# askerlee/segtran

Hardware: AMD Instinct MI355X
Metric: train-step images/sec (cfg2, re-associated op order) (higher is better)
Workload: dtype f32; 1 GPU; REFUGE fundus 2D, segtran eff-b4, translayers 3, layercompress 1,1,2,2, 512x512, bs 6/GPU; global_batch=6, per_gpu_batch=6, parallelism=dp1, step=fwd+BCE/Dice+bwd+allreduce+clip+BertAdam, op_order=re-associated, ranks=1

## Files before the change

include/segx.h:

```cpp
#ifndef SEGX_H
#define SEGX_H
#include <stdint.h>
#ifdef __cplusplus
extern "C" {
#endif

int segx_version(void);
int segx_last_error(char* buf, int buflen);

enum { SEGX_EPI_NONE = 0, SEGX_EPI_GELU = 1 ,
       SEGX_EPI_SWISH = 2 ,
       SEGX_EPI_RELU = 3  };
enum { SEGX_BIAS_NONE = 0, SEGX_BIAS_N = 1 , SEGX_BIAS_M = 2  };
enum { SEGX_ENGINE_F32 = 0, SEGX_ENGINE_BF16X6 = 1 };
enum { SEGX_ENGINE_SEL_DEFAULT = 0, SEGX_ENGINE_SEL_F32 = 1, SEGX_ENGINE_SEL_BF16X6 = 2 };
enum { SEGX_TILE_AUTO = 0, SEGX_TILE_128x128 = 1, SEGX_TILE_64x64 = 2, SEGX_TILE_128x32 = 3, SEGX_TILE_32x128 = 4, SEGX_TILE_64x128 = 5,
       SEGX_TILE_256x128 = 6, SEGX_TILE_WS128x128 = 7, SEGX_TILE_WS128x256 = 8, SEGX_TILE_WS64x256 = 9,
       SEGX_TILE_WS96x256 = 10, SEGX_TILE_WS256x96 = 11,
       SEGX_TILE_SKINNY_NT = 12   };
typedef struct {
    int32_t M, N, K, nb0, nb1;
    int64_t a_b0, a_b1, a_m, a_k;
    int64_t b_b0, b_b1, b_n, b_k;
    int64_t c_b0, c_b1, c_m;
    float alpha;
    int32_t epilogue, bias_mode;
    int64_t bias_b1;
    const float* bias;
    float* aux;
    float* gmax;
    float dropout_p;
    uint64_t seed, offset;
    int32_t splitk;
    float* workspace;
    int32_t tile;
    int64_t bias_b0;
    int32_t batch_reduce;
    int32_t engine;
    const void* b_planes;
    int64_t bp_b0, bp_b1;
    const float* resid;
} segx_gemm_desc;
int segx_gemm_f32(const float* A, const float* B, float* C, const segx_gemm_desc* d, void* stream);
int segx_gemm_plan(const float* A, const float* B, const segx_gemm_desc* d, int* tile, int* splitk);
int segx_gemm_plan_model(const float* A, const float* B, const segx_gemm_desc* d, int* tile, int* splitk);
int segx_gemm_route(const float* A, const float* B, const segx_gemm_desc* d, int32_t* out);
int64_t segx_x6_presplit_elems(int rows, int K, int nb0, int nb1);
int segx_x6_presplit(const float* W, int rows, int K, int64_t s_row, int64_t s_k, int nb0, int nb1, int64_t s_b0, int64_t s_b1, void* planes, void* stream);


int segx_softmax_fwd(const float* S, float* P, float* Pdrop, int64_t rows, int L, float clip, const float* gmax,
                     float p, uint64_t seed, uint64_t offset, void* stream);
int segx_softmax_bwd(const float* P, const float* dPdrop, const float* S , float* dS,
                     int64_t rows, int L, float clip, const float* gmax, float p, uint64_t seed, uint64_t offset, void* stream);
int segx_posbias_fwd(const float* S, float* out, const float* table, int64_t nmat, int N, const int* geom, float weight, float clip,
                     const float* gmax, void* stream);
int segx_posbias_bwd(const float* dOut, const float* S, float* dS, float* dtable, int64_t nmat, int N, const int* geom, float weight,
                     float clip, void* stream);
int segx_layernorm_fwd(const float* X, const float* w, const float* b, float* Y, float* mean, float* rstd,
                       int64_t rows, int C, float eps, void* stream);
int segx_layernorm_bwd(const float* dY, const float* X, const float* w, const float* mean, const float* rstd, float* dX,
                       int64_t rows, int C, void* stream);
int64_t segx_colreduce_ws_floats(int64_t rows, int64_t C, int nout);
int segx_colsum(const float* X, float* out, float* ws, int64_t rows, int64_t C, void* stream);
int segx_ln_param_grad(const float* dY, const float* X, const float* mean, const float* rstd, float* dw, float* db,
                       float* ws, int64_t rows, int C, void* stream);
int segx_sum(const float* x, int64_t n, float* out, float* ws , float scale, void* stream);
int segx_rowsum(const float* X, float* out, int64_t R, int64_t S, void* stream);
int segx_prenorm_fwd(const float* X, const float* w1, const float* b1, const float* pos, int64_t pos_ld, float pos_weight,
                     const float* mask, float* Y, float* stats, int64_t B, int N, int C, float eps,
                     float p, uint64_t seed, uint64_t offset, void* stream);
int segx_prenorm_bwd(const float* dY, const float* X, const float* w1, const float* b1, const float* pos, int64_t pos_ld,
                     float pos_weight, const float* mask, const float* stats, float* dX, float* dU, int64_t B, int N, int C,
                     float p, uint64_t seed, uint64_t offset, void* stream);
int64_t segx_prenorm_bwd_all_ws_floats(int N, int C);
int segx_prenorm_bwd_all(const float* dY, const float* X, const float* w1, const float* b1, const float* pos, int64_t pos_ld, float pos_weight,
                         const float* mask, const float* stats, float* dX, float* dsum, float* dw, float* db, float* ws, int B, int N, int C,
                         float p, uint64_t seed, uint64_t offset, void* stream);
int segx_posembed_fwd(const float* posn, const float* Wp, const float* bp, float* out, float* stats, int64_t N, int C, int pd,
                      float eps, void* stream);
int segx_posembed_bwd(const float* dOut, const float* posn, const float* Wp, const float* bp, const float* stats, float* dZ,
                      int64_t N, int C, int pd, void* stream);
int segx_modes_aggr_fwd(const float* Z, const float* lnw, const float* lnb, const float* wa, const float* ba, float* Y, float* stats,
                        int Mo, int64_t R, int F, float eps, float p, uint64_t seed, uint64_t offset, void* stream);
int segx_modes_aggr_bwd(const float* dY, const float* Z, const float* lnw, const float* lnb, const float* wa, const float* stats,
                        float* dZ, float* dscore, int Mo, int64_t R, int F, float p, uint64_t seed, uint64_t offset, void* stream);
int segx_modes_aggr_param_grad(const float* dY, const float* Z, const float* lnw, const float* lnb, const float* wa,
                               const float* stats, const float* dscore, float* dlnw, float* dlnb, float* dwa, float* ws,
                               int Mo, int64_t R, int F, float p, uint64_t seed, uint64_t offset, void* stream);
int64_t segx_modes_aggr_bwd_all_ws_floats(int Mo, int64_t R, int F);
int segx_modes_aggr_bwd_all(const float* dY, const float* Z, const float* lnw, const float* lnb, const float* wa, const float* stats,
                            float* dZ, float* dscore, float* dlnw, float* dlnb, float* dwa, float* ws, int Mo, int64_t R, int F,
                            float p, uint64_t seed, uint64_t offset, void* stream);
int segx_gelu_bwd(const float* dH, const float* T, float* dT, int64_t n, float p, uint64_t seed, uint64_t offset, void* stream);
int64_t segx_gelu_bwd_colsum_ws_floats(int64_t rows, int N);
int segx_gelu_bwd_colsum(const float* dH, const float* T, float* dT, float* colsum, float* ws, int64_t rows, int N, float p, uint64_t seed, uint64_t offset,
                         void* stream);

int64_t segx_loss_ws_floats(int B, int C);
int segx_seg_loss_fwd(const float* logits, const float* mask, const float* pos_weight, const float* class_w, float* out,
                      float* ws, int B, int C, int64_t S, float dice_w, void* stream);
int segx_seg_loss_bwd(const float* logits, const float* mask, const float* pos_weight, const float* class_w, const float* ws,
                      const float* grad_out, float* dlogits, int B, int C, int64_t S, float dice_w, void* stream);
int segx_mt_bertadam_step(void* const* params, const void* const* grads, void* const* m, void* const* v, const int64_t* sizes,
                          const int* chunk_tensor, const int64_t* chunk_off, const int* chunk_first, const int* active,
                          const float* lr, const float* wd, int ntensors, int nchunks, int chunk,
                          float max_global_norm, float max_tensor_norm, float sched, double b1, double b2, float eps,
                          float* ws, void* stream);

int segx_mt_gather(const void* const* src, void* const* dst, const int64_t* sizes, const int* chunk_tensor, const int64_t* chunk_off,
                   int chunk_begin, int nchunks, int chunk, void* stream);

int64_t segx_bn_ws_floats(int B, int C, int64_t S);
int segx_bn_act_bwd_reduce(const float* dY, const float* X, const float* mean, const float* var, const float* w, const float* b,
                           float* dw, float* db, float* ws, int B, int C, int64_t S, float eps, int act,
                           const float* gate, const float* dpool, float inv_S, float dc_p, uint64_t seed, uint64_t offset, void* stream);
int segx_bn_act_bwd_apply(const float* dY, const float* X, const float* mean, const float* var, const float* w, const float* b,
                          const float* sum_dw, const float* sum_db, float* dX, int B, int C, int64_t S, float eps, int act,
                          float inv_n, const float* gate, const float* dpool, float inv_S, float dc_p, uint64_t seed, uint64_t offset, void* stream);
int64_t segx_plane_chunks(int64_t S);
int64_t segx_bn_pool_chunks(int B, int64_t S, int auto_stats);
int64_t segx_bn_parts_floats(int B, int C, int64_t S);
int segx_bn_stats_local(const float* X, float* part, float* ws, int B, int C, int64_t S, void* stream);
int segx_bn_act_fwd2(const float* X, const float* parts, int nparts, float* mean, float* var, float* run_mean, float* run_var, float momentum,
                     const float* w, const float* b, float* Y, float* psum, const float* resid, float dc_p, uint64_t seed, uint64_t offset,
                     int B, int C, int64_t S, float eps, int act, int64_t parts_floats, int64_t y_bs, void* stream);
int segx_team_status(int clear);
int segx_team_cap(void);
int segx_occupy(int wgs, int heavy, float ms, float* sink, void* stream);
int segx_bn_act_bwd2(const float* dY, const float* X, const float* mean, const float* var, const float* w, const float* b,
                     float* dX, float* dw, float* db, float* ws, int B, int C, int64_t S, float eps, int act, int training,
                     const float* gate, const float* dpool, float inv_S, float dc_p, uint64_t seed, uint64_t offset, int64_t dy_bs, int64_t ws_floats, void* stream);
int segx_se_fwd2(const float* psum, int nch, float inv_S, const float* W1, const float* b1, const float* W2, const float* b2, const float* Wproj,
                 float* p, float* hpre, float* gate, float* Wb, int B, int C, int Cs, int M, void* stream);
int64_t segx_se_ws2_floats(int B, int C, int Cs);
int segx_se_bwd2(const float* dWb, const float* Wproj, const float* dgate, const float* gate, const float* hpre, const float* p, const float* W1,
                 const float* W2, float inv_S, float* dpool, float* dW1, float* db1, float* dW2, float* db2, float* dWproj, float* ws,
                 int B, int C, int Cs, int M, void* stream);
int segx_dwconv2d_fwd(const float* X, const float* W, float* Y, int B, int C, int H, int Wd, int OH, int OW, int k, int stride,
                      int pad_t, int pad_l, void* stream);
int64_t segx_dwconv2d_pool_chunks(int OH, int OW);
int segx_dwconv2d_bias_act_pool(const float* X, const float* W, const float* bias, float* Y, float* psum, int B, int C, int H, int Wd, int OH, int OW,
                                int k, int stride, int pad_t, int pad_l, int act, void* stream);
int segx_dwconv2d_bwd_data(const float* dY, const float* W, float* dX, int B, int C, int H, int Wd, int OH, int OW, int k,
                           int stride, int pad_t, int pad_l, void* stream);
int64_t segx_dwconv2d_wgrad_rows(int OH, int OW);
int64_t segx_dwconv2d_bwd_fused_rows(int H, int Wd, int OH, int OW, int k, int stride, int pad_t, int pad_l);
int segx_dwconv2d_bwd_fused(const float* dY, const float* X, const float* W, float* dX, float* part, int B, int C, int H, int Wd, int OH, int OW,
                            int k, int stride, int pad_t, int pad_l, void* stream);
int segx_mbconv_mid_ok(int B, int C, int H, int W, int k);
int segx_mbconv_mid_fwd(const float* E, const float* w0, const float* b0, float* run_mean0, float* run_var0, const float* Wdw, const float* w1, const float* b1,
                        float* run_mean1, float* run_var1, float* D, float* Y, float* psum, float* mean0, float* var0, float* mean1, float* var1,
                        float momentum0, float eps0, float momentum1, float eps1, int B, int C, int H, int W, int k, void* stream);
int segx_mbconv_mid_bwd(const float* dY, const float* dpool, const float* D, const float* E, const float* mean0, const float* var0, const float* mean1,
                        const float* var1, const float* w0, const float* b0, const float* w1, const float* b1, const float* Wdw,
                        float* dE, float* dw0, float* db0, float* dw1, float* db1, float* dWdw, float inv_S, float eps0, float eps1,
                        int B, int C, int H, int W, int k, void* stream);
int segx_bn_dw_s2_ok(int B, int C, int H, int W, int k, int stride, int pad_t, int pad_l);
int64_t segx_bn_dw_s2_ws_floats(int B, int C, int H, int W, int backward);
int64_t segx_bn_dw_s2_rows(int B, int H, int W);
int segx_bn_dw_s2_fwd(const float* E, const float* w0, const float* b0, float* run_mean, float* run_var, const float* Wdw, float* D, float* mean, float* var,
                      float* ws, float momentum, float eps, int B, int C, int H, int W, int k, int pad_t, int pad_l, int64_t ws_floats, void* stream);
int segx_bn_dw_s2_bwd(const float* dD, const float* E, const float* mean, const float* var, const float* w0, const float* b0, const float* Wdw,
                      float* dE, float* dw0, float* db0, float* part, float* ws, float eps, int B, int C, int H, int W, int k, int pad_t, int pad_l,
                      int64_t part_rows, int64_t ws_floats, void* stream);
int segx_dwconv2d_bwd_weight_direct(const float* dY, const float* X, float* dW, int B, int C, int H, int Wd, int OH, int OW, int k,
                                    int stride, int pad_t, int pad_l, void* stream);
int segx_dwconv2d_bwd_weight(const float* dY, const float* X, float* part, int B, int C, int H, int Wd, int OH, int OW, int k,
                             int stride, int pad_t, int pad_l, void* stream);
int segx_plane_scale(const float* X, const float* gate, float* Y, int64_t planes, int64_t S, void* stream);
int segx_plane_bias_add(const float* X, const float* bias, float* Y, int64_t planes, int C, int64_t S, void* stream);
int segx_plane_dot(const float* A, const float* Bm, float* out, int64_t planes, int64_t S, void* stream);

int segx_add_relu_fwd(const float* Z, const float* R, const float* bias, float* Y, int64_t planes, int C, int64_t S, void* stream);
int segx_add_relu_bwd(const float* dY, const float* Y, float* dZ, int64_t planes, int64_t S, void* stream);

int64_t segx_gn_ws_floats(int B, int C, int G);
int segx_groupnorm_fwd(const float* X, const float* w, const float* b, float* Y, float* mean, float* rstd, float* ws,
                       int B, int C, int G, int64_t S, float eps, void* stream);
int segx_groupnorm_bwd(const float* dY, const float* X, const float* w, const float* mean, const float* rstd, float* dX,
                       float* dw, float* db, float* ws, int B, int C, int G, int64_t S, float* plane_dx_sums, void* stream);
int64_t segx_interp_gn_nparts(int64_t float4_per_plane, int cpg);
int segx_interp_linear_fwd_axis2_gn(const float* in, const float* base, float* out, int64_t outer, int n1_in, int n1_out, int n2_in, int n2_out,
                                    int64_t inner, int cpg, float* parts, int nparts, void* stream);
int segx_groupnorm_fwd_parts(const float* X, const float* parts, int nparts, const float* w, const float* b, float* Y, float* mean, float* rstd,
                             int B, int C, int G, int64_t S, float eps, void* stream);
int segx_groupnorm_stats_parts(const float* parts, int nparts, float* mean, float* rstd, int BG, float eps, void* stream);
int segx_gn_fold_bwd_proj(const float* dOut, const float* Wb, int NC, const float* X, const float* mean, const float* rstd, const float* A, const float* Bc,
                          float* dX, float* plane_sums, float* ws, int B, int C, int G, int64_t S, void* stream);
int segx_gn_fold_bwd(const float* Gd, const float* X, const float* mean, const float* rstd, const float* A, const float* Bc, float* dX, float* plane_sums,
                     float* ws, int B, int C, int G, int64_t S, void* stream);
int segx_avgpool2_fwd(const float* X, float* Y, int64_t planes, int H, int W, void* stream);
int segx_avgpool2_bwd(const float* dY, float* dX, int64_t planes, int H, int W, void* stream);
int segx_transpose(const float* X, float* Y, int64_t batch, int R, int C, void* stream);
int segx_dropout(const float* x, float* y, int64_t n, float p, uint64_t seed, uint64_t offset, void* stream);
int segx_set_rng_base(const uint64_t* base);
int segx_rng_advance(uint64_t* base, uint64_t span, void* stream);

enum {
    SEGX_KNOB_INTERP_VARIANT = 1,
    SEGX_KNOB_CONV_SMALL_POLICY = 2,
    SEGX_KNOB_BN_PATH = 3,
    SEGX_KNOB_ENGINE = 4,
    SEGX_KNOB_X6_LAUNCHES = 5,
    SEGX_KNOB_X6_VARIANT = 6,
    SEGX_KNOB_CONV_X6_WGRAD_ALL = 7,
    SEGX_KNOB_DW_STRIP_OUTPUTS = 8,
    SEGX_KNOB_WS_GRID = 9,
    SEGX_KNOB_TEAM_SPIN = 12,
    SEGX_KNOB_TEAM_DROP = 13,
    SEGX_KNOB_POOL_SLAB = 14,
    SEGX_KNOB_POOL_DSLIDE = 15,
    SEGX_KNOB_CONV_HALO = 16,
    SEGX_KNOB_CONV_HALO_MIN_TILES = 17,
    SEGX_KNOB_SKINNY_NT = 18,
    SEGX_KNOB_TILE_WALK = 19
};
#define SEGX_KNOB_X6_TERMS 20
int segx_tune(int knob, int value);
int segx_tune_get(int knob);
int segx_x3_launches(void);
int segx_interp_linear_fwd_axis2(const float* in, const float* base, float* out, int64_t outer, int n1_in, int n1_out, int n2_in, int n2_out,
                                 int64_t inner, void* stream);
int segx_interp_linear_bwd_axis2(const float* dout, float* din, int64_t outer, int n1_out, int n1_in, int n2_out, int n2_in, int64_t inner, void* stream);
int segx_interp_linear_fwd(const float* in, const float* base, float* out, int64_t planes, int d, int h, int w, int D, int H, int W,
                           void* stream);
int segx_interp_linear_fwd_axis(const float* in, const float* base, float* out, int64_t outer, int n_in, int n_out, int64_t inner,
                                float src_scale, void* stream);
int segx_resized_crop3d(const float* X, float* Y, int64_t planes, const int* geom, void* stream);
int segx_interp_linear_bwd(const float* dout, float* din, int64_t planes, int d, int h, int w, int D, int H, int W, void* stream);
int segx_axis_gather(const float* X, float* Y, int64_t planes, const int* geom, void* stream);
int segx_pixel_shuffle2(const float* X, float* Y, int64_t planes, int h, int w, int inverse, void* stream);
int segx_add_noise(const float* X, const float* noise, float* Y, int64_t n, float mu, float sigma, int nonzero_only, uint64_t seed, uint64_t offset,
                   void* stream);
int segx_resize2d(const float* X, float* Y, int64_t planes, int h, int w, int H, int W, int mode, int quantize, void* stream);
int segx_color_blend(const float* X, float* Y, int B, int64_t HW, int mode, const float* factor, const float* pivot, int quantize, void* stream);
int64_t segx_gray_mean_ws_floats(int B, int64_t HW);
int segx_gray_mean(const float* X, float* mean, float* ws, int B, int64_t HW, int quantize, void* stream);
int segx_normalize(const float* X, float* Y, int B, int C, int64_t HW, float scale, const float* mean, const float* std, void* stream);

int segx_interp_linear_bwd_axis(const float* dout, float* din, int64_t outer, int n_out, int n_in, int64_t inner, float src_scale,
                                void* stream);

int64_t segx_conv3d_splitk(int B, int Cout, const int* geom, int wgrad);
int segx_conv3d_route(int B, int Cout, const int* geom, int wgrad, int splitk, int aligned, int packed, int32_t* out);
int segx_conv3d_fwd_terms(int B, int Cout, const int* geom, int splitk, int aligned, int packed);
int segx_conv3d_fwd(const float* X, const float* W , float* Y, int B, int Cout, const int* geom, int splitk,
                    float* workspace, void* stream);
int segx_conv3d_pack_weights(const float* W, float* Wp, int O, int C, int KV, int mode, void* stream);
int segx_conv3d_fwd_packed(const float* X, const float* Wp, float* Y, int B, int Cout, const int* geom, int splitk, float* workspace,
                           void* stream);
int segx_conv3d_flip_weights(const float* W, float* Wt, int Cout, int Cin, int KV, void* stream);
int segx_conv3d_bwd_weight(const float* dY, const float* X, float* dWb, int B, int Cout, const int* geom, int splitk,
                           float* workspace, void* stream);
int segx_conv3d_bwd_weight_packed(const float* dY, const float* X, float* dWb, int B, int Cout, const int* geom, int splitk,
                                  float* workspace, void* stream);
int segx_conv3d_unpack_wgrad(const float* dWp, float* dW, int Cout, int Cin, int KV, void* stream);
int segx_conv3d_fwd_packed_bs(const float* X, const float* Wp, float* Y, int B, int Cout, const int* geom, int splitk, float* workspace,
                              int64_t x_bstride, int64_t y_bstride, void* stream);
int segx_conv3d_fwd_bias_act(const float* X, const float* W, const float* bias, float* Y, int B, int Cout, const int* geom, int splitk, float* workspace,
                             int packed, int64_t x_bstride, int64_t y_bstride, int act, void* stream);
int segx_bias_map_relu(float* Y, const float* map, int B, int64_t n, void* stream);
int segx_conv3d_bwd_weight_packed_bs(const float* dY, const float* X, float* dWb, int B, int Cout, const int* geom, int splitk, float* workspace,
                                     int64_t dy_bstride, int64_t x_bstride, void* stream);
int segx_conv3d_halo_ok(int B, int Cout, const int* geom);
int64_t segx_conv3d_halo_wq_floats(int O, int C);
int segx_conv3d_halo_pack(const float* W, void* Wq, int O, int C, int mode, void* stream);
int segx_conv3d_halo_fwd(const float* X, const void* Wq, float* Y, int B, int Cout, const int* geom, int64_t x_bstride, int64_t y_bstride, int mtile, void* stream);
int segx_conv3d_halo_bias_act_fwd(const float* X, const void* Wq, const float* bias, float* Y, int B, int Cout, const int* geom, int64_t x_bstride, int64_t y_bstride,
                                  int mtile, int act, void* stream);
int segx_conv3d_halo_wgrad_ok(int B, int Cout, const int* geom);
int64_t segx_conv3d_halo_wgrad_ws_floats(int B, int Cout, const int* geom);
int segx_conv3d_halo_wgrad(const float* dY, const float* X, float* dW, float* ws, int B, int Cout, const int* geom, int64_t dy_bstride, int64_t x_bstride, void* stream);
int segx_conv3d_bwd_data_direct(const float* dY, const float* W, float* dX, float* wt_ws , int B, int Cout,
                                const int* geom, void* stream);
int segx_stem_compose_fwd(const float* Ws, const float* Wb, const float* bb, float* Wc, int O, int C3, int Cb, int Cc, int T, void* stream);
int segx_stem_compose_bwd(const float* dWc, const float* Ws, const float* Wb, const float* bb, float* dWs, float* dWb, float* dbb,
                          int O, int C3, int Cb, int Cc, int T, void* stream);
int segx_bridge_input(const float* X, float* Y, int B, int Cb, int Cc, int H, int W, int D, void* stream);
int segx_stem_s2d_input(const float* X, float* Y, int B, int Cb, int H, int W, int D, int U, void* stream);
int segx_conv2d_stem_fwd(const float* X, const float* W, float* Y, int B, int Cin, int Cout, int H, int Wd, int OH, int OW, int K, int stride, int pt, int pl,
                         void* stream);
int segx_conv2d_stem_bias_act_fwd(const float* X, const float* W, const float* bias, float* Y, int B, int Cin, int Cout, int H, int Wd, int OH, int OW, int K,
                                  int stride, int pt, int pl, int act, void* stream);
int segx_conv2d_stem_im2col(const float* X, float* Xcol, int B, int Cin, int H, int Wd, int OH, int OW, int K, int stride, int pt, int pl, int rows, void* stream);
int segx_bridge_mask(const float* X, const float* Wb, const float* bb, float* out, int B, int Cb, int C3, int H, int W, int D, int kd, int kh, int kw, void* stream);
int segx_nonzero_mask(const float* X, float* out, int B, int C, int D, int H, int W, int kd, int kh, int kw, void* stream);
int segx_label_nhot(const void* labels, float* out, int B, int Cin, int64_t S, int mode, void* stream);
int segx_maxpool3d_fwd(const float* X, float* Y, int* arg, int64_t planes, const int* geom, void* stream);
int segx_maxpool3d_bwd(const float* dY, const int* arg, float* dX, int64_t planes, const int* geom, const float* addend, void* stream);

int segx_window_accum(const float* scores, float* acc, float* cnt, int B, int C, const int* geom, void* stream);
#define SEGX_MAX_CLASSES 16
int segx_harden_segmap(const float* acc, const float* cnt, float* soft, float* hard, int B, int C, int64_t S, int mode, float T,
                       void* stream);
int segx_window_gather(const float* image, const int* origins, const int* origins_host, float* out, int nwin, int B, int C, const int* geom,
                       void* stream);
int segx_window_merge(const float* scores, const int* origins, const int* origins_host, float* soft, float* hard, int nwin, int B, int C,
                      const int* geom, int mode, float T, void* stream);
int64_t segx_dice_ws_floats(int64_t planes, int64_t S);
int segx_dice_sums(const float* pred, const float* gt, float* part, int64_t planes, int64_t S, void* stream);

#define SEGX_EDT_INF 0x40000000
#define SEGX_EDT_MAX_EXTENT 256
int segx_surface_border(const float* mask, uint8_t* border, int64_t planes, int D, int H, int W, int nd, void* stream);
int segx_edt_sq(const uint8_t* border, int32_t* d2, int64_t planes, int D, int H, int W, void* stream);
int segx_surface_hist(const uint8_t* border_from, const int32_t* d2_to, int32_t* hist, int64_t planes, int D, int H, int W, int nbins, void* stream);
#define SEGX_CASE_TAIL_THREADS 256
#define SEGX_CASE_TAIL_MAX_BLOCKS 2048
int segx_brats_case_tail(const float* soft, const float* hard, const int32_t* gt, int32_t* counts, uint8_t* labels, int64_t S, void* stream);

int segx_index_onehot(const void* labels, int label_bytes, float* out, int64_t B, int C, int64_t S, void* stream);
int segx_onehot_colormap(const float* nhot, const uint8_t* colormap, uint8_t* out, int64_t B, int C, int64_t S, void* stream);
int segx_onehot_case_tail(const float* soft, const uint8_t* gt, const uint8_t* colormap, int32_t* counts, uint8_t* labels, uint8_t* rgb, int B, int C, int64_t S,
                          float T, void* stream);
int segx_nhot_case_tail(const float* soft, const void* gt, int gt_map, int gt_channels, const int32_t* values, int32_t* counts, int32_t* ext, uint8_t* labels,
                        float* hard, int B, int C, int h, int w, int H, int W, float T, void* stream);

// ... 14 lines not shown
```

segtran_amd/csrc/backbone.hip:

```cpp
#include "common.h"
#include <mutex>
#include <unordered_map>

namespace segx {


__device__ __forceinline__ float drop_connect_scale(float p, uint64_t seed, uint64_t offset, const uint64_t* __restrict__ rbase, int sample) {
    if (!(p > 0.f)) return 1.0f;
    return dropout_scale(seed, 0, offset + (rbase ? *rbase : 0) + (uint64_t)sample, p, 1.0f / (1.0f - p));
}
__device__ __forceinline__ void bn_fold_sums(const float* __restrict__ ws, int c, int nparts, float& a, float& q) {
    const int lane = threadIdx.x & 63;
    const float2* p = reinterpret_cast<const float2*>(ws) + (int64_t)c * nparts;
    a = 0.f; q = 0.f;
    for (int i = lane; i < nparts; i += 64) { const float2 v = p[i]; a += v.x; q += v.y; }
    a = wave_sum(a); q = wave_sum(q);
}

constexpr int BN_SLABS = 8;
static inline int bn_slabs(int64_t S) { const int64_t n = S / 8192; return (int)(n < 1 ? 1 : n > BN_SLABS ? BN_SLABS : n); }

__global__ __launch_bounds__(256) void bn_act_bwd_stage1(const float* __restrict__ dY, const float* __restrict__ X, const float* __restrict__ mean,
                                                         const float* __restrict__ var, const float* __restrict__ w, const float* __restrict__ b,
                                                         float* __restrict__ ws, int C, int64_t S, float eps, int act,
// ... 471 lines not shown
        g.mean[c] = mean; g.var[c] = var;
        if (g.run_mean && st.n == st.n) {
            g.run_mean[c] = (1.0f - g.momentum) * g.run_mean[c] + g.momentum * mean;
            g.run_var[c] = (1.0f - g.momentum) * g.run_var[c] + g.momentum * (st.m2 / fmaxf(st.n - 1.0f, 1.0f));
        }
    }
    const float sc = rsqrtf(var + g.eps) * g.w[c], sh = g.b[c] - mean * sc;
    const bool resid = RESID < 0 ? g.resid != nullptr : RESID != 0;
    const float dcs = drop_connect_scale(g.dc_p, g.seed, g.offset, g.rbase, b);
    const ws_gptr_w yb = ws_uniform_base_w(g.Y + (int64_t)b * g.y_bs + (int64_t)c * S);
    const ws_gptr rb = ws_uniform_base((resid ? g.resid : g.X) + plane);
    float acc = 0.f;
    constexpr int G = 4;
    int tl2 = tl;
    SEGX_PIN(tl2);
    auto offs = [&](int k) { const int j = j0 + tl2 + 256 * k; return 16u * (unsigned)(j < S4 ? j : S4 - 1); };
#pragma unroll
    for (int k0 = 0; k0 < KP; k0 += G) {
        f32x4 rv[G];
        if (resid) {
#pragma unroll
            for (int e = 0; e < G; ++e) rv[e] = ws_load<f32x4>(rb, offs(k0 + e));
        }
#pragma unroll
        for (int e = 0; e < G; ++e) {
            const int k = k0 + e;
            f32x4 o;
            o.x = act_fwd_c<ACT>(v[k].x * sc + sh, act); o.y = act_fwd_c<ACT>(v[k].y * sc + sh, act);
            o.z = act_fwd_c<ACT>(v[k].z * sc + sh, act); o.w = act_fwd_c<ACT>(v[k].w * sc + sh, act);
            if (resid) { o.x = o.x * dcs + rv[e].x; o.y = o.y * dcs + rv[e].y; o.z = o.z * dcs + rv[e].z; o.w = o.w * dcs + rv[e].w; }
            if (j0 + tl2 + 256 * k < S4) {
                ws_store<f32x4>(yb, offs(k), o);
                if (POOL) acc += (o.x + o.y) + (o.z + o.w);
            }
        }
        __builtin_amdgcn_sched_barrier(0);
    }
    if (POOL) {
        acc = block_sum<4>(acc, red);
        if (tl == 0) g.psum[((int64_t)b * C + c) * t.cpp + ch] = acc;
    }
}
template <int KP, int ACT>
__global__ __launch_bounds__(256) SEGX_MIN_WAVES_PER_SIMD(KP <= 4 ? 4 : KP <= 8 ? 3 : 2) void bn_act_bwd_team_kernel(BnBwdArgs g, BnTeam t) {
    __shared__ float red[4];
    const int TS = t.B * t.cpp, tl = threadIdx.x;
    const int c = blockIdx.x / TS, r = blockIdx.x - c * TS, b = r / t.cpp, ch = r - b * t.cpp;
    const int C = g.C, S4 = (int)(g.S >> 2), j0 = ch * 256 * KP, act = g.act;
    const int64_t S = g.S;
    unsigned off[KP];
#pragma unroll
    for (int k = 0; k < KP; ++k) { const int j = j0 + tl + 256 * k; off[k] = 16u * (unsigned)(j < S4 ? j : S4 - 1); }
    f32x4 h[KP], d[KP];
    const ws_gptr xb = ws_uniform_base(g.X + ((int64_t)b * C + c) * S), gb = ws_uniform_base(g.dY + (int64_t)b * g.dy_bs + (int64_t)c * S);
#pragma unroll
    for (int k = 0; k < KP; ++k) { h[k] = ws_load<f32x4>(xb, off[k]); d[k] = ws_load<f32x4>(gb, off[k]); }
    __builtin_amdgcn_sched_barrier(0);
    const float rstd = rsqrtf(g.var[c] + g.eps), m = g.mean[c], wc = g.w[c], bc_ = g.b[c];
    const int pl = b * C + c;
    const float gt = (g.gate ? g.gate[pl] : 1.0f) * drop_connect_scale(g.dc_p, g.seed, g.offset, g.rbase, b), dp = g.dpool ? g.dpool[pl] * g.inv_S : 0.f;
    float a = 0.f, q = 0.f;
#pragma unroll
    for (int k = 0; k < KP; ++k) {
        const bool ok = j0 + tl + 256 * k < S4;
        const f32x4 xv = h[k], gv = d[k];
        f32x4 hh, dd;
        hh.x = (xv.x - m) * rstd; hh.y = (xv.y - m) * rstd; hh.z = (xv.z - m) * rstd; hh.w = (xv.w - m) * rstd;
        dd.x = (gv.x * gt + dp) * act_grad_c<ACT>(hh.x * wc + bc_, act); dd.y = (gv.y * gt + dp) * act_grad_c<ACT>(hh.y * wc + bc_, act);
        dd.z = (gv.z * gt + dp) * act_grad_c<ACT>(hh.z * wc + bc_, act); dd.w = (gv.w * gt + dp) * act_grad_c<ACT>(hh.w * wc + bc_, act);
        if (!ok) { dd = f32x4{0.f, 0.f, 0.f, 0.f}; hh = dd; }
        h[k] = hh; d[k] = dd;
        a += (dd.x + dd.y) + (dd.z + dd.w); q += (dd.x * hh.x + dd.y * hh.y) + (dd.z * hh.z + dd.w * hh.w);
    }
    a = block_sum<4>(a, red); q = block_sum<4>(q, red);
    const TeamBufs tb{t.slots + (int64_t)c * TS * TEAM_SLOT, t.mbox + (int64_t)c * TS * TEAM_MBOX, t.tag_lo, t.tag_hi, t.err, t.spin};
    if (tl == 0) { float* pp = tb.slots + r * TEAM_SLOT; team_store(pp, a); team_store(pp + 1, q); }
    float res[3];
    team_exchange(tb, r, TS, res, [](const float* parts, int members, float (&o)[3]) {
        const int lane = threadIdx.x & 63;
        const bool h0 = lane < members, h1 = lane + 64 < members;
        const float a0 = team_load(parts + TEAM_SLOT * (h0 ? lane : 0)), q0 = team_load(parts + TEAM_SLOT * (h0 ? lane : 0) + 1);
        const float a1 = team_load(parts + TEAM_SLOT * (h1 ? lane + 64 : 0)), q1 = team_load(parts + TEAM_SLOT * (h1 ? lane + 64 : 0) + 1);
        float A = (h0 ? a0 : 0.f) + (h1 ? a1 : 0.f), Q = (h0 ? q0 : 0.f) + (h1 ? q1 : 0.f);
#pragma unroll
        for (int o2 = 1; o2 < 64; o2 <<= 1) { A += __shfl_xor(A, o2); Q += __shfl_xor(Q, o2); }
        o[0] = A; o[1] = Q; o[2] = 0.f;
    });
    const float A = res[0], Q = res[1];
    if (r == 0 && tl == 0) { g.db[c] = A; g.dw[c] = Q; }
    const float inv_n = 1.0f / ((float)t.B * (float)S), k1 = A * inv_n, k2 = Q * inv_n, sc = wc * rstd;
    const ws_gptr_w ob = ws_uniform_base_w(g.dX + ((int64_t)b * C + c) * S);
#pragma unroll
    for (int k = 0; k < KP; ++k) {
        if (j0 + tl + 256 * k < S4) {
            f32x4 o;
            o.x = sc * (d[k].x - k1 - h[k].x * k2); o.y = sc * (d[k].y - k1 - h[k].y * k2);
            o.z = sc * (d[k].z - k1 - h[k].z * k2); o.w = sc * (d[k].w - k1 - h[k].w * k2);
            ws_store<f32x4>(ob, off[k], o);
        }
    }
}
static inline int bn_res_form(int B, int64_t S, bool backward) {
    if ((S & 3) || B < 1 || B > 8 || S > 8192) return 0;
    const int S4 = (int)(S >> 2);
    const int kw = (S4 + 63) / 64, kb = (S4 + 255) / 256;
    const int capw = backward ? 1 : 2, capb = backward ? 2 : 4;
    if (kw <= capw) return 64 * 16 + (kw <= 1 ? 1 : 2);
    if (kb <= capb) return 256 * 16 + (kb <= 1 ? 1 : kb <= 2 ? 2 : 4);
    return 0;
}
static inline bool bn_bwd_plane_team(int B, int64_t S) { return (S & 3) == 0 && S > 2048 && S <= 4096 && B >= 1 && B <= 6; }

static inline int bn_team_chunks(int64_t S, int kp) { return (int)((S / 4 + 256 * kp - 1) / (256 * kp)); }
static inline int bn_team_kp_small(int64_t S) { return S <= 4096 ? 4 : S <= 8192 ? 8 : 16; }
static inline int bn_team_kp(int B, int64_t S, bool backward) {
    if ((S & 3) || B < 1 || S < 16384) return 0;
    const int cap = team_cap();
    if (backward) return (int64_t)bn_team_chunks(S, 16) * B <= cap ? 16 : 0;
    if ((int64_t)bn_team_chunks(S, 16) * B <= (cap < 32 ? cap : 32)) return 16;
    return (int64_t)bn_team_chunks(S, 32) * B <= (cap < 64 ? cap : 64) ? 32 : 0;
}
static inline int bn_auto_form(int B, int64_t S, bool backward, int* kp = nullptr) {
    const int path = kget(knobs().bn_path);
    int k = 16;
    int form = 0;
    if (path == 2 && (S & 3) == 0 && B <= 128 && S >= 4 && (int64_t)bn_team_chunks(S, 16) * B <= team_cap()) { form = 1; k = bn_team_kp_small(S); }
    else if (bn_res_form(B, S, backward)) form = 2;
    else if (backward && path != 1 && bn_bwd_plane_team(B, S) && B <= team_cap()) { form = 1; k = bn_team_kp_small(S); }
    else if (path != 1 && (k = bn_team_kp(B, S, backward)) != 0) form = 1;
    if (kp) *kp = form == 1 ? k : 0;
    return form;
}
template <int KP>
static int bn_team_launch_fwd(const BnFwdArgs& g, const BnTeam& t, dim3 grid, hipStream_t stream, bool pool) {
    const bool resid = g.resid != nullptr;
#define SEGX_BN_TF(P, A, R) do { if (int rc = team_occupancy_ok((const void*)bn_act_fwd_team_kernel<KP, P, A, R>, "segx_bn_act_fwd2/team")) return rc; \
                                 hipLaunchKernelGGL((bn_act_fwd_team_kernel<KP, P, A, R>), grid, dim3(256), 0, stream, g, t); } while (0)
    if (pool) { if (!resid && g.act == ACT_SWISH) SEGX_BN_TF(true, ACT_SWISH, 0); else SEGX_BN_TF(true, -1, -1); }
    else if (!resid && g.act == ACT_SWISH) SEGX_BN_TF(false, ACT_SWISH, 0);
    else if (g.act == ACT_NONE) { if (resid) SEGX_BN_TF(false, ACT_NONE, 1); else SEGX_BN_TF(false, ACT_NONE, 0); }
    else if (!resid && g.act == ACT_RELU) SEGX_BN_TF(false, ACT_RELU, 0);
    else SEGX_BN_TF(false, -1, -1);
#undef SEGX_BN_TF
    return check_launch("segx_bn_act_fwd2/team");
}
template <int KP>
static int bn_team_launch_bwd(const BnBwdArgs& g, const BnTeam& t, dim3 grid, hipStream_t stream) {
#define SEGX_BN_TB(A) do { if (int rc = team_occupancy_ok((const void*)bn_act_bwd_team_kernel<KP, A>, "segx_bn_act_bwd2/team")) return rc; \
                           hipLaunchKernelGGL((bn_act_bwd_team_kernel<KP, A>), grid, dim3(256), 0, stream, g, t); } while (0)
    if (g.act == ACT_SWISH) SEGX_BN_TB(ACT_SWISH); else if (g.act == ACT_NONE) SEGX_BN_TB(ACT_NONE); else if (g.act == ACT_RELU) SEGX_BN_TB(ACT_RELU); else SEGX_BN_TB(-1);
#undef SEGX_BN_TB
    return check_launch("segx_bn_act_bwd2/team");
}
constexpr int S2_BAND = 4;
constexpr int S2_IMG = 1440;
constexpr int S2_GIMG = 1600;
struct BnDwS2Args {
    const float* E; const float* w; const float* b; const float* Wdw; float* mean; float* var;
    float* D; float* run_mean; float* run_var; float momentum;
    const float* dD; float* dE; float* dw; float* db; float* part;
    float eps; int C, H, W4, pt;
};
template <int KP, int K, int PL>
__global__ __launch_bounds__(256) SEGX_MIN_WAVES_PER_SIMD(KP <= 16 ? 3 : 2) void bn_dw_s2_fwd_team_kernel(BnDwS2Args g, BnTeam t) {
    static_assert(KP % S2_BAND == 0 && PL <= 4 && 4 + 3 * 2 + K - 1 - PL < 16, "window does not fit the four float4 read per row");
    constexpr int NB = KP / S2_BAND;
    __shared__ float red[4];
    __shared__ f32x4 img[NB > 1 ? 2 : 1][S2_IMG];
    const int TS = t.B * t.cpp, tl = threadIdx.x;
    const int c = blockIdx.x / TS, r = blockIdx.x - c * TS, b = r / t.cpp, ch = r - b * t.cpp;
    const int C = g.C, W4 = g.W4, S4 = g.H * W4, j0 = ch * 256 * KP;
    const int64_t S = 4 * (int64_t)S4, plane = ((int64_t)b * C + c) * S;
    auto offk = [&](int k) { const int j = j0 + tl + 256 * k; return 16u * (unsigned)(j < S4 ? j : S4 - 1); };
    f32x4 v[KP];
    const ws_gptr xb = ws_uniform_base(g.E + plane);
#pragma unroll
    for (int k = 0; k < KP; ++k) v[k] = ws_load<f32x4>(xb, offk(k));
    const int rpk = 256 / W4, tr = tl / W4, tc = tl - tr * W4, HT = g.pt, LS = W4 + 1, IR = S2_BAND * rpk + K - 2;
    f32x4 hv[2]; bool hok[2];
#pragma unroll
    for (int q = 0; q < 2; ++q) {
        const int hr = tr + q * rpk;
        const int jh = (hr < HT ? j0 - (HT - hr) * W4 : j0 + 256 * KP + (hr - HT) * W4) + tc;
        hok[q] = hr < K - 2 && jh >= 0 && jh < S4;
        hv[q] = ws_load<f32x4>(xb, 16u * (unsigned)(hok[q] ? jh : 0));
    }
    __builtin_amdgcn_sched_barrier(0);
    for (int i = tl; i <= IR; i += 256) {
        img[0][i * LS] = f32x4{0.f, 0.f, 0.f, 0.f};
        if (NB > 1) img[NB > 1 ? 1 : 0][i * LS] = f32x4{0.f, 0.f, 0.f, 0.f};
    }
    float w[K * K];
#pragma unroll
    for (int i = 0; i < K * K; ++i) w[i] = g.Wdw[(int64_t)c * K * K + i];
    float s = 0.f;
#pragma unroll
    for (int k = 0; k < KP; ++k) {
        if (!(j0 + tl + 256 * k < S4)) v[k] = f32x4{0.f, 0.f, 0.f, 0.f};
        s += (v[k].x + v[k].y) + (v[k].z + v[k].w);
    }
    const int left4 = S4 - j0;
    const float n = 4.0f * (float)(left4 < 256 * KP ? left4 : 256 * KP);
    const float m = block_sum<4>(s, red) / n;
    float q = 0.f;
#pragma unroll
    for (int k = 0; k < KP; ++k) {
        const float d0 = v[k].x - m, d1 = v[k].y - m, d2 = v[k].z - m, d3 = v[k].w - m;
        q += (j0 + tl + 256 * k < S4) ? (d0 * d0 + d1 * d1) + (d2 * d2 + d3 * d3) : 0.f;
    }
    q = block_sum<4>(q, red);
    const TeamBufs tb{t.slots + (int64_t)c * TS * TEAM_SLOT, t.mbox + (int64_t)c * TS * TEAM_MBOX, t.tag_lo, t.tag_hi, t.err, t.spin};
    if (tl == 0) { float* pp = tb.slots + r * TEAM_SLOT; team_store(pp, n); team_store(pp + 1, m); team_store(pp + 2, q); }
    float res[3];
    team_exchange(tb, r, TS, res, [](const float* slots, int members, float (&o)[3]) { const BnPart f = bn_fold_team(slots, members); o[0] = f.n; o[1] = f.mean; o[2] = f.m2; });
    BnPart st; st.n = res[0]; st.mean = res[1]; st.m2 = res[2];
    const float mean = st.mean, var = st.n != st.n ? st.n : st.n > 0.f ? fmaxf(st.m2 / st.n, 0.f) : 0.f;
    if (r == 0 && tl == 0) {
        g.mean[c] = mean; g.var[c] = var;
        if (g.run_mean && st.n == st.n) {
            g.run_mean[c] = (1.0f - g.momentum) * g.run_mean[c] + g.momentum * mean;
            g.run_var[c] = (1.0f - g.momentum) * g.run_var[c] + g.momentum * (st.m2 / fmaxf(st.n - 1.0f, 1.0f));
        }
    }
    const float sc = rsqrtf(var + g.eps) * g.w[c], sh = g.b[c] - mean * sc;
    auto act4 = [&](const f32x4& x, bool ok) {
        f32x4 o;
        o.x = act_fwd_c<ACT_SWISH>(x.x * sc + sh, ACT_SWISH); o.y = act_fwd_c<ACT_SWISH>(x.y * sc + sh, ACT_SWISH);
        o.z = act_fwd_c<ACT_SWISH>(x.z * sc + sh, ACT_SWISH); o.w = act_fwd_c<ACT_SWISH>(x.w * sc + sh, ACT_SWISH);
        return ok ? o : f32x4{0.f, 0.f, 0.f, 0.f};
    };
    const int OW4 = W4 >> 1, orow = tl / OW4, oc = tl - orow * OW4, D4 = S4 >> 2;
    const int rpos = (2 * orow) * LS + 2 * oc + 1;
    const ws_gptr_w db_ = ws_uniform_base_w(g.D + ((int64_t)b * C + c) * (S >> 2));
#pragma unroll
    for (int bd = 0; bd < NB; ++bd) {
        constexpr int KB = S2_BAND;
        const int k0 = bd * KB;
        f32x4* im = img[bd & (NB > 1 ? 1 : 0)];
#pragma unroll
        for (int kk = k0 - 1; kk <= k0 + KB; ++kk) {
            if (kk < 0 || kk >= KP) continue;
            const int ir = tr + (kk - k0) * rpk + HT;
            if (kk < k0 ? ir >= 0 : kk < k0 + KB || ir < IR) im[ir * LS + 1 + tc] = act4(v[kk], j0 + tl + 256 * kk < S4);
        }
        if (bd == 0 || bd == NB - 1) {
#pragma unroll
            for (int q2 = 0; q2 < 2; ++q2) {
                const int hr = tr + q2 * rpk;
                if (hr < K - 2 && (hr < HT ? bd == 0 : bd == NB - 1)) im[(hr < HT ? hr : KB * rpk + hr) * LS + 1 + tc] = act4(hv[q2], hok[q2]);
            }
        }
        __syncthreads();
        float acc[4] = {0.f, 0.f, 0.f, 0.f};
#pragma unroll
        for (int ky = 0; ky < K; ++ky) {
            const f32x4* p = im + rpos + ky * LS;
            const f32x4 e0 = p[-1], e1 = p[0], e2 = p[1], e3 = p[2];
            const float e[16] = {e0.x, e0.y, e0.z, e0.w, e1.x, e1.y, e1.z, e1.w, e2.x, e2.y, e2.z, e2.w, e3.x, e3.y, e3.z, e3.w};
#pragma unroll
            for (int j = 0; j < 4; ++j)
#pragma unroll
                for (int kx = 0; kx < K; ++kx) acc[j] += w[ky * K + kx] * e[4 + j * 2 + kx - PL];
#pragma unroll
            for (int j = 0; j < 4; ++j) SEGX_PIN(acc[j]);
        }
        const int dj = ((j0 + 256 * k0) >> 2) + tl;
        if (dj < D4) ws_store<f32x4>(db_, 16u * (unsigned)dj, f32x4{acc[0], acc[1], acc[2], acc[3]});
        __builtin_amdgcn_sched_barrier(0);
    }
}
template <int KP, int K, int PL>
__global__ __launch_bounds__(256) SEGX_MIN_WAVES_PER_SIMD(2) void bn_dw_s2_bwd_team_kernel(BnDwS2Args g, BnTeam t) {
    constexpr int A = (K + 1) / 2, KK = K * K, NGV = KP / 4 + 1;
    __shared__ float red[4];
    __shared__ double wred[4][KK];
    __shared__ f32x4 gim[S2_GIMG];
    const int TS = t.B * t.cpp, tl = threadIdx.x;
    const int c = blockIdx.x / TS, r = blockIdx.x - c * TS, b = r / t.cpp, ch = r - b * t.cpp;
    const int C = g.C, W4 = g.W4, S4 = g.H * W4, j0 = ch * 256 * KP, pt = g.pt;
    const int64_t S = 4 * (int64_t)S4, plane = ((int64_t)b * C + c) * S;
    auto offk = [&](int k) { const int j = j0 + tl + 256 * k; return 16u * (unsigned)(j < S4 ? j : S4 - 1); };
    f32x4 h[KP], d[KP];
    const ws_gptr xb = ws_uniform_base(g.E + plane);
#pragma unroll
    for (int k = 0; k < KP; ++k) h[k] = ws_load<f32x4>(xb, offk(k));
    const int rpk = 256 / W4, tr = tl / W4, tc = tl - tr * W4, OW4 = W4 >> 1, OH = g.H >> 1, GS = OW4 + 1, NG = KP * (rpk >> 1) + A;
    const int gpr = 256 / OW4, gr = tl / OW4, gc = tl - gr * OW4, oy_lo = ((j0 / W4) >> 1) + (pt >> 1) - (A - 1);
    {
        const ws_gptr gb = ws_uniform_base(g.dD + ((int64_t)b * C + c) * (S >> 2));
        f32x4 gv[NGV];
#pragma unroll
        for (int i = 0; i < NGV; ++i) {
            const int oy = oy_lo + gr + i * gpr;
            gv[i] = ws_load<f32x4>(gb, 16u * (unsigned)(gr + i * gpr < NG && oy >= 0 && oy < OH ? oy * OW4 + gc : 0));
        }
        for (int i = tl; i <= NG; i += 256) gim[i * GS] = f32x4{0.f, 0.f, 0.f, 0.f};
#pragma unroll
        for (int i = 0; i < NGV; ++i) {
            const int gi = gr + i * gpr, oy = oy_lo + gi;
            if (gi < NG) gim[gi * GS + 1 + gc] = oy >= 0 && oy < OH ? gv[i] : f32x4{0.f, 0.f, 0.f, 0.f};
        }
    }
    __syncthreads();
    __builtin_amdgcn_sched_barrier(0);
    const float rstd = rsqrtf(g.var[c] + g.eps), m = g.mean[c], wc = g.w[c], bc_ = g.b[c], sc = rstd * wc, sh = bc_ - m * sc;
    const int py = (tr + pt) & 1;
    float wsel[A][K], dwa[A][K];
#pragma unroll
    for (int a = 0; a < A; ++a)
#pragma unroll
        for (int kx = 0; kx < K; ++kx) {
            const float we = g.Wdw[(int64_t)c * KK + (2 * a) * K + kx], wo = 2 * a + 1 < K ? g.Wdw[(int64_t)c * KK + (2 * a + 1) * K + kx] : 0.f;
            wsel[a][kx] = py ? wo : we; dwa[a][kx] = 0.f;
        }
    const float* gf = reinterpret_cast<const float*>(gim) + (((tr + pt) >> 1) - (pt >> 1) + A - 1) * (4 * GS) + 2 * tc + 2;
    float sa = 0.f, sq = 0.f;
#pragma unroll
    for (int k = 0; k < KP; ++k) {
        const bool ok = j0 + tl + 256 * k < S4;
        const f32x4 xv = h[k];
        const float u[4] = {xv.x * sc + sh, xv.y * sc + sh, xv.z * sc + sh, xv.w * sc + sh};
        float ep[4], de[4] = {0.f, 0.f, 0.f, 0.f};
#pragma unroll
        for (int i = 0; i < 4; ++i) ep[i] = ok ? act_fwd_c<ACT_SWISH>(u[i], ACT_SWISH) : 0.f;
#pragma unroll
        for (int a = A - 1; a >= 0; --a) {
            const float* gp = gf + (k * (rpk >> 1) - a) * (4 * GS);
            const float2 g0 = *reinterpret_cast<const float2*>(gp), g1 = *reinterpret_cast<const float2*>(gp + 2), g2 = *reinterpret_cast<const float2*>(gp + 4);
            const float G[6] = {g0.x, g0.y, g1.x, g1.y, g2.x, g2.y};
#pragma unroll
            for (int i = 0; i < 4; ++i)
#pragma unroll
                for (int kx = 0; kx < K; ++kx) {
                    if ((i + PL - kx) & 1) continue;
                    const int nn = (i + PL - kx + 4) / 2;
                    de[i] = __builtin_fmaf(wsel[a][kx], G[nn], de[i]); dwa[a][kx] = __builtin_fmaf(ep[i], G[nn], dwa[a][kx]);
                    SEGX_PIN(de[i]); SEGX_PIN(dwa[a][kx]);
                }
            __builtin_amdgcn_sched_barrier(0);
        }
        f32x4 hh, dd;
        hh.x = (xv.x - m) * rstd; hh.y = (xv.y - m) * rstd; hh.z = (xv.z - m) * rstd; hh.w = (xv.w - m) * rstd;
        dd.x = de[0] * act_grad_c<ACT_SWISH>(hh.x * wc + bc_, ACT_SWISH); dd.y = de[1] * act_grad_c<ACT_SWISH>(hh.y * wc + bc_, ACT_SWISH);
        dd.z = de[2] * act_grad_c<ACT_SWISH>(hh.z * wc + bc_, ACT_SWISH); dd.w = de[3] * act_grad_c<ACT_SWISH>(hh.w * wc + bc_, ACT_SWISH);
        if (!ok) { dd = f32x4{0.f, 0.f, 0.f, 0.f}; hh = dd; }
        h[k] = hh; d[k] = dd;
        sa += (dd.x + dd.y) + (dd.z + dd.w); sq += (dd.x * hh.x + dd.y * hh.y) + (dd.z * hh.z + dd.w * hh.w);
    }
    sa = block_sum<4>(sa, red); sq = block_sum<4>(sq, red);
    const TeamBufs tb{t.slots + (int64_t)c * TS * TEAM_SLOT, t.mbox + (int64_t)c * TS * TEAM_MBOX, t.tag_lo, t.tag_hi, t.err, t.spin};
    if (tl == 0) { float* pp = tb.slots + r * TEAM_SLOT; team_store(pp, sa); team_store(pp + 1, sq); }
    float res[3];
    team_exchange(tb, r, TS, res, [](const float* parts, int members, float (&o)[3]) {
        const int lane = threadIdx.x & 63;
        const bool h0 = lane < members, h1 = lane + 64 < members;
        const float a0 = team_load(parts + TEAM_SLOT * (h0 ? lane : 0)), q0 = team_load(parts + TEAM_SLOT * (h0 ? lane : 0) + 1);
        const float a1 = team_load(parts + TEAM_SLOT * (h1 ? lane + 64 : 0)), q1 = team_load(parts + TEAM_SLOT * (h1 ? lane + 64 : 0) + 1);
        float As = (h0 ? a0 : 0.f) + (h1 ? a1 : 0.f), Qs = (h0 ? q0 : 0.f) + (h1 ? q1 : 0.f);
#pragma unroll
        for (int o2 = 1; o2 < 64; o2 <<= 1) { As += __shfl_xor(As, o2); Qs += __shfl_xor(Qs, o2); }
        o[0] = As; o[1] = Qs; o[2] = 0.f;
    });
    const float As = res[0], Qs = res[1];
    if (r == 0 && tl == 0) { g.db[c] = As; g.dw[c] = Qs; }
    const float inv_n = 1.0f / ((float)t.B * (float)S), k1 = As * inv_n, k2 = Qs * inv_n;
    const ws_gptr_w ob = ws_uniform_base_w(g.dE + plane);
    int tl2 = tl;
    SEGX_PIN(tl2);
#pragma unroll
    for (int k = 0; k < KP; ++k) {
        const int j = j0 + tl2 + 256 * k;
        if (j < S4) {
            f32x4 o;
            o.x = sc * (d[k].x - k1 - h[k].x * k2); o.y = sc * (d[k].y - k1 - h[k].y * k2);
            o.z = sc * (d[k].z - k1 - h[k].z * k2); o.w = sc * (d[k].w - k1 - h[k].w * k2);
            ws_store<f32x4>(ob, 16u * (unsigned)j, o);
        }
    }
#pragma unroll
    for (int a = 0; a < A; ++a)
#pragma unroll
        for (int p = 0; p < 2; ++p) {
            if (2 * a + p >= K) continue;
#pragma unroll
            for (int kx = 0; kx < K; ++kx) {
                const double sw = wave_sum_d(py == p ? (double)dwa[a][kx] : 0.0);
                if ((tl & 63) == 0) wred[tl >> 6][(2 * a + p) * K + kx] = sw;
            }
        }
    __syncthreads();
    if (tl < KK) g.part[((int64_t)r * C + c) * KK + tl] = (float)((wred[0][tl] + wred[1][tl]) + (wred[2][tl] + wred[3][tl]));
}
static inline bool s2_pow2(int v) { return v > 0 && (v & (v - 1)) == 0; }
static inline int s2_kp(int B, int64_t S, bool backward) {
    int kp = 0;
    if (B < 1 || S < 4 || bn_auto_form(B, S, backward, &kp) != 1) return 0;
    return kp == 4 || kp == 16 || (kp == 32 && !backward) ? kp : 0;
}
static inline bool s2_serves(int B, int C, int H, int W, int k, int stride, int pt, int pl) {
    if (!(stride == 2 && (k == 3 || k == 5) && B >= 1 && C >= 1 && H >= 2 && (H & 1) == 0 && W >= 16 && W <= 512 && s2_pow2(W))) return false;
    if (!(pt == pl && pt >= (k - 2) / 2 && pt <= k / 2)) return false;
    const int64_t S = (int64_t)H * W;
    if (S > (int64_t)1 << 26 || (int64_t)B * C > 65535) return false;
    const int kf = s2_kp(B, S, false), kb = s2_kp(B, S, true);
    if (!kf || !kb || (1024 * kf) % (2 * W) || (1024 * kb) % (2 * W)) return false;
    const int W4 = W / 4, rpk = 256 / W4;
    return (S2_BAND * rpk + k - 2) * (W4 + 1) + 1 <= S2_IMG && (kb * (rpk / 2) + (k + 1) / 2) * (W4 / 2 + 1) + 1 <= S2_GIMG;
}
template <int KP, int K>
static int s2_launch_fwd(const BnDwS2Args& g, const BnTeam& t, dim3 grid, hipStream_t stream, int pl) {
#define SEGX_S2F(P) do { if (int rc = team_occupancy_ok((const void*)bn_dw_s2_fwd_team_kernel<KP, K, P>, "segx_bn_dw_s2_fwd")) return rc; \
                         hipLaunchKernelGGL((bn_dw_s2_fwd_team_kernel<KP, K, P>), grid, dim3(256), 0, stream, g, t); } while (0)
    if (pl == (K - 2) / 2) SEGX_S2F((K - 2) / 2); else SEGX_S2F(K / 2);
#undef SEGX_S2F
    return check_launch("segx_bn_dw_s2_fwd");
}
template <int KP, int K>
static int s2_launch_bwd(const BnDwS2Args& g, const BnTeam& t, dim3 grid, hipStream_t stream, int pl) {
#define SEGX_S2B(P) do { if (int rc = team_occupancy_ok((const void*)bn_dw_s2_bwd_team_kernel<KP, K, P>, "segx_bn_dw_s2_bwd")) return rc; \
                         hipLaunchKernelGGL((bn_dw_s2_bwd_team_kernel<KP, K, P>), grid, dim3(256), 0, stream, g, t); } while (0)
    if (pl == (K - 2) / 2) SEGX_S2B((K - 2) / 2); else SEGX_S2B(K / 2);
#undef SEGX_S2B
    return check_launch("segx_bn_dw_s2_bwd");
}
template <int T, int K, int BM>
static void bn_res_launch_fwd(const BnFwdArgs& g, int B, dim3 grid, hipStream_t stream, bool pool) {
    const bool resid = g.resid != nullptr;
#define SEGX_BN_F(P, A, R) hipLaunchKernelGGL((bn_act_fwd_res_kernel<T, K, BM, P, A, R>), grid, dim3(256), 0, stream, g, B)
    if (pool) { if (!resid && g.act == ACT_SWISH) SEGX_BN_F(true, ACT_SWISH, 0); else SEGX_BN_F(true, -1, -1); }
    else if (!resid && g.act == ACT_SWISH) SEGX_BN_F(false, ACT_SWISH, 0);
    else if (g.act == ACT_NONE) { if (resid) SEGX_BN_F(false, ACT_NONE, 1); else SEGX_BN_F(false, ACT_NONE, 0); }
    else if (!resid && g.act == ACT_RELU) SEGX_BN_F(false, ACT_RELU, 0);
    else SEGX_BN_F(false, -1, -1);
#undef SEGX_BN_F
}
template <int T, int K, int BM>
static void bn_res_launch_bwd(const BnBwdArgs& g, int B, dim3 grid, hipStream_t stream) {
#define SEGX_BN_B(A) hipLaunchKernelGGL((bn_act_bwd_res_kernel<T, K, BM, A>), grid, dim3(256), 0, stream, g, B)
    if (g.act == ACT_SWISH) SEGX_BN_B(ACT_SWISH); else if (g.act == ACT_NONE) SEGX_BN_B(ACT_NONE); else if (g.act == ACT_RELU) SEGX_BN_B(ACT_RELU); else SEGX_BN_B(-1);
#undef SEGX_BN_B
}

constexpr int DW_TY = 8;
struct DwTile { int ox, oy0; bool live; };
__device__ __forceinline__ DwTile dw_tile(int tile, int tiles_x, int txw_log2, int OH, int OW) {
    const int txw = 1 << txw_log2, rg = threadIdx.x >> txw_log2, nrg = 256 >> txw_log2;
    const int tyi = tile / tiles_x, txi = tile - tyi * tiles_x;
    DwTile t;
    t.ox = txi * txw + (threadIdx.x & (txw - 1));
    t.oy0 = (tyi * nrg + rg) * DW_TY;
    t.live = t.ox < OW && t.oy0 < OH;
    return t;
}
template <int K, int ST, bool FLIP>
__global__ __launch_bounds__(256) void dwconv_rows_kernel(const float* __restrict__ X, const float* __restrict__ Wt, float* __restrict__ Y,
                                                          int C, int H, int W, int OH, int OW, int pt, int pl, int tiles_x, int txw_log2) {
    const int bc = blockIdx.y, c = bc % C;
    const DwTile t = dw_tile(blockIdx.x, tiles_x, txw_log2, OH, OW);
    if (!t.live) return;
    const float* x = X + (int64_t)bc * H * W;
    float w[K * K];
#pragma unroll
    for (int i = 0; i < K * K; ++i) w[i] = Wt[(int64_t)c * K * K + (FLIP ? K * K - 1 - i : i)];
    float acc[DW_TY];
#pragma unroll
    for (int i = 0; i < DW_TY; ++i) acc[i] = 0.f;
    const int ix0 = t.ox * ST - pl, iy0 = t.oy0 * ST - pt;
    constexpr int NR = (DW_TY - 1) * ST + K;
#pragma unroll
    for (int r = 0; r < NR; ++r) {
        const int iy = iy0 + r;
        const bool rowok = iy >= 0 && iy < H;
        const float* xr = x + (int64_t)min(max(iy, 0), H - 1) * W;
        float v[K];
#pragma unroll
        for (int kx = 0; kx < K; ++kx) {
            const int ix = ix0 + kx;
            const float q = xr[min(max(ix, 0), W - 1)];
            v[kx] = (rowok && ix >= 0 && ix < W) ? q : 0.f;
        }
#pragma unroll
        for (int ky = 0; ky < K; ++ky) {
            if ((r - ky) < 0 || (r - ky) % ST != 0 || (r - ky) / ST >= DW_TY) continue;
#pragma unroll
            for (int kx = 0; kx < K; ++kx) acc[(r - ky) / ST] += w[ky * K + kx] * v[kx];
            SEGX_PIN(acc[(r - ky) / ST]);
        }
    }
    float* y = Y + (int64_t)bc * OH * OW + t.ox;
#pragma unroll
    for (int i = 0; i < DW_TY; ++i) if (t.oy0 + i < OH) y[(int64_t)(t.oy0 + i) * OW] = acc[i];
}
constexpr int DW4_TY = 8, DW4_AHEAD = 2;
template <int K, int ST> struct Dw4 { static constexpr int NV = ST == 1 ? 3 : 4; };
template <int NV>
__device__ __forceinline__ void dw4_load_row(float (&e)[4 * NV], const float* __restrict__ xr, const int (&xo)[NV], const bool (&okv)[NV], bool rowok) {
#pragma unroll
    for (int i = 0; i < NV; ++i) {
        const float4 q = *reinterpret_cast<const float4*>(xr + xo[i]);
        const bool ok = rowok && okv[i];
        e[4 * i] = ok ? q.x : 0.f; e[4 * i + 1] = ok ? q.y : 0.f; e[4 * i + 2] = ok ? q.z : 0.f; e[4 * i + 3] = ok ? q.w : 0.f;
    }
}
template <int K, int ST, int PL, bool FLIP>
__global__ __launch_bounds__(256) SEGX_MIN_WAVES_PER_SIMD(4) void dwconv_rows4_kernel(const float* __restrict__ X, const float* __restrict__ Wt, float* __restrict__ Y,
                                                           int C, int H, int W, int OH, int OW, int pt, int tiles_x, int tiles_y, int tpr_log2,
                                                           int64_t ngroups) {
    constexpr int NV = Dw4<K, ST>::NV;
    static_assert(PL <= 4 && 4 + 3 * ST + K - 1 - PL < 4 * NV, "window does not fit the loaded float4s");
    const int64_t gid = ((int64_t)xcd_block(blockIdx.x, gridDim.x) * 256 + threadIdx.x) >> tpr_log2;
    if (gid >= ngroups) return;
    const int gpp = tiles_x * tiles_y;
    const int64_t plane = gid / gpp;
    const int rem = (int)(gid - plane * gpp), tyi = rem / tiles_x, txi = rem - tyi * tiles_x;
    const int ox = ((txi << tpr_log2) + (threadIdx.x & ((1 << tpr_log2) - 1))) * 4, oy0 = tyi * DW4_TY;
    if (ox >= OW) return;
    const int c = (int)(plane % C);
    const float* x = X + plane * H * W;
    float w[K * K];
#pragma unroll
    for (int i = 0; i < K * K; ++i) w[i] = Wt[(int64_t)c * K * K + (FLIP ? K * K - 1 - i : i)];
    float acc[DW4_TY][4];
#pragma unroll
    for (int i = 0; i < DW4_TY; ++i) { acc[i][0] = 0.f; acc[i][1] = 0.f; acc[i][2] = 0.f; acc[i][3] = 0.f; }
    int xo[NV]; bool okv[NV];
#pragma unroll
    for (int i = 0; i < NV; ++i) { const int col = ox * ST - 4 + 4 * i; okv[i] = col >= 0 && col < W; xo[i] = min(max(col, 0), W - 4); }
    const int iy0 = oy0 * ST - pt;
    constexpr int NR = (DW4_TY - 1) * ST + K;
    float e[DW4_AHEAD + 1][4 * NV];
#pragma unroll
    for (int r = 0; r < DW4_AHEAD && r < NR; ++r)
        dw4_load_row<NV>(e[r], x + (int64_t)min(max(iy0 + r, 0), H - 1) * W, xo, okv, iy0 + r >= 0 && iy0 + r < H);
#pragma unroll
    for (int r = 0; r < NR; ++r) {
        if (r + DW4_AHEAD < NR) {
            const int iy = iy0 + r + DW4_AHEAD;
            dw4_load_row<NV>(e[(r + DW4_AHEAD) % (DW4_AHEAD + 1)], x + (int64_t)min(max(iy, 0), H - 1) * W, xo, okv, iy >= 0 && iy < H);
        }
        __builtin_amdgcn_sched_barrier(0);
#pragma unroll
        for (int ky = 0; ky < K; ++ky) {
            if ((r - ky) < 0 || (r - ky) % ST != 0 || (r - ky) / ST >= DW4_TY) continue;
#pragma unroll
            for (int j = 0; j < 4; ++j)
#pragma unroll
                for (int kx = 0; kx < K; ++kx)
                    acc[(r - ky) / ST][j] += w[ky * K + kx] * e[r % (DW4_AHEAD + 1)][4 + j * ST + kx - PL];
#pragma unroll
            for (int j = 0; j < 4; ++j) SEGX_PIN(acc[(r - ky) / ST][j]);
        }
        __builtin_amdgcn_sched_barrier(0);
    }
    float* y = Y + plane * OH * OW + ox;
#pragma unroll
    for (int i = 0; i < DW4_TY; ++i)
        if (oy0 + i < OH) *reinterpret_cast<float4*>(y + (int64_t)(oy0 + i) * OW) = make_float4(acc[i][0], acc[i][1], acc[i][2], acc[i][3]);
}
template <int K, int ST, int PL>
__global__ __launch_bounds__(256) SEGX_MIN_WAVES_PER_SIMD(4) void dwconv_rows4_bias_act_pool_kernel(const float* __restrict__ X, const float* __restrict__ Wt, const float* __restrict__ bias,
                                                           float* __restrict__ Y, float* __restrict__ psum, int C, int H, int W, int OH, int OW, int pt, int tiles_x, int tiles_y,
                                                           int tpr_log2, int64_t ngroups, int act) {
    constexpr int NV = Dw4<K, ST>::NV;
    static_assert(PL <= 4 && 4 + 3 * ST + K - 1 - PL < 4 * NV, "window does not fit the loaded float4s");
    const int64_t gid_raw = ((int64_t)xcd_block(blockIdx.x, gridDim.x) * 256 + threadIdx.x) >> tpr_log2;
    const bool glive = gid_raw < ngroups;
    const int64_t gid = glive ? gid_raw : ngroups - 1;
    const int gpp = tiles_x * tiles_y;
    const int64_t plane = gid / gpp;
    const int rem = (int)(gid - plane * gpp), tyi = rem / tiles_x, txi = rem - tyi * tiles_x;
    const int ox_raw = ((txi << tpr_log2) + (threadIdx.x & ((1 << tpr_log2) - 1))) * 4, oy0 = tyi * DW4_TY;
    const bool live = glive && ox_raw < OW;
    const int ox = ox_raw < OW ? ox_raw : OW - 4;
    const int c = (int)(plane % C);
    const float* x = X + plane * H * W;
    float w[K * K];
// ... 818 lines not shown
    const int rows = (64 >> g.tpr_log2) * segx::DWG_TY, ntiles = g.tiles_x * ((OH + rows - 1) / rows);
    const int64_t nwork = (int64_t)B * C * strips;
    const int64_t nblocks = (nwork + 3) / 4;
#define SEGX_DW4(KK, SS, PP)                                                                                                        \
    if (k == KK && stride == SS && pl == PP) {                                                                                       \
        hipLaunchKernelGGL((segx::dwconv_wgrad4_kernel<KK, SS, PP>), dim3((unsigned)nblocks), dim3(256), 0, stream, dY, X, part, C,  \
                           H, Wd, OH, OW, pt, g.tiles_x, ntiles, g.tpr_log2, strips, nwork);                                         \
        return true;                                                                                                                 \
    }
    SEGX_DW4(3, 1, 1) SEGX_DW4(5, 1, 2) SEGX_DW4(3, 2, 0) SEGX_DW4(3, 2, 1) SEGX_DW4(5, 2, 1) SEGX_DW4(5, 2, 2)
#undef SEGX_DW4
    return false;
}
}

extern "C" int segx_dwconv2d_fwd(const float* X, const float* W, float* Y, int B, int C, int H, int Wd, int OH, int OW, int k, int stride,
                                 int pad_t, int pad_l, void* stream_) {
    SEGX_STREAM; SEGX_REQUIRE(X && W && Y && B > 0 && C > 0 && H > 0 && Wd > 0 && OH > 0 && OW > 0 && (int64_t)B * C <= 65535, "segx_dwconv2d_fwd: bad args");
    if (dw4_ok(X, Y, Wd, OW) && dw4_rows_launch<false>(stream, X, W, Y, B * C, C, H, Wd, OH, OW, k, stride, pad_t, pad_l))
        return check_launch("segx_dwconv2d_fwd");
    const DwGrid g = dw_grid(OH, OW);
    dim3 grid(g.tiles_x * g.tiles_y, B * C);
    SEGX_DW_ROWS_DISPATCH(false, X, W, Y, C, H, Wd, OH, OW, pad_t, pad_l, g.tiles_x, g.txw_log2);
    return check_launch("segx_dwconv2d_fwd");
}
extern "C" int64_t segx_dwconv2d_pool_chunks(int OH, int OW) {
    if (OH <= 0 || OW <= 0) return 0;
    return (int64_t)dw4_grid(OW).tiles_x * ((OH + segx::DW4_TY - 1) / segx::DW4_TY);
}
extern "C" int segx_dwconv2d_bias_act_pool(const float* X, const float* W, const float* bias, float* Y, float* psum, int B, int C, int H, int Wd, int OH, int OW,
                                           int k, int stride, int pad_t, int pad_l, int act, void* stream_) {
    SEGX_STREAM; SEGX_REQUIRE(X && W && bias && Y && B > 0 && C > 0 && H > 0 && Wd > 0 && OH > 0 && OW > 0 && (int64_t)B * C <= 65535 && (act == 0 || act == 1) && pad_t >= 0 && pad_l >= 0,
                              "segx_dwconv2d_bias_act_pool: bad args");
    SEGX_REQUIRE((int64_t)(OH - 1) * stride - pad_t < H && (int64_t)(OW - 1) * stride - pad_l < Wd, "segx_dwconv2d_bias_act_pool: output %d x %d does not fit input %d x %d", OH, OW, H, Wd);
    const Dw4Grid g = dw4_grid(OW);
    const int tiles_y = (OH + segx::DW4_TY - 1) / segx::DW4_TY, planes = B * C;
    if (dw4_ok(X, Y, Wd, OW)) {
        const int64_t ngroups = (int64_t)planes * g.tiles_x * tiles_y;
        const int64_t nblocks = ((ngroups << g.tpr_log2) + 255) / 256;
        if (nblocks <= 2147483647LL) {
#define SEGX_DW4P(KK, SS, PP)                                                                                                                          \
            if (k == KK && stride == SS && pad_l == PP) {                                                                                               \
                hipLaunchKernelGGL((segx::dwconv_rows4_bias_act_pool_kernel<KK, SS, PP>), dim3((unsigned)nblocks), dim3(256), 0, stream, X, W, bias, Y, \
                                   psum, C, H, Wd, OH, OW, pad_t, g.tiles_x, tiles_y, g.tpr_log2, ngroups, act);                                        \
                return check_launch("segx_dwconv2d_bias_act_pool");                                                                                     \
            }
            SEGX_DW4P(3, 1, 1) SEGX_DW4P(5, 1, 2) SEGX_DW4P(3, 2, 0) SEGX_DW4P(3, 2, 1) SEGX_DW4P(5, 2, 1) SEGX_DW4P(5, 2, 2)
#undef SEGX_DW4P
        }
    }
    const dim3 grid(g.tiles_x * tiles_y, planes);
    SEGX_DW_DISPATCH(segx::dwconv_bias_act_pool_kernel, X, W, bias, Y, psum, C, H, Wd, OH, OW, pad_t, pad_l, g.tiles_x, g.tpr_log2 + 2, act);
    return check_launch("segx_dwconv2d_bias_act_pool");
}
extern "C" int segx_dwconv2d_bwd_data(const float* dY, const float* W, float* dX, int B, int C, int H, int Wd, int OH, int OW, int k, int stride,
                                      int pad_t, int pad_l, void* stream_) {
    SEGX_STREAM; SEGX_REQUIRE(dY && W && dX && B > 0 && C > 0 && H > 0 && Wd > 0 && OH > 0 && OW > 0 && (int64_t)B * C <= 65535, "segx_dwconv2d_bwd_data: bad args");
    if (stride == 1) {
        if (dw4_ok(dY, dX, OW, Wd) && dw4_rows_launch<true>(stream, dY, W, dX, B * C, C, OH, OW, H, Wd, k, 1, k - 1 - pad_t, k - 1 - pad_l))
            return check_launch("segx_dwconv2d_bwd_data");
        const DwGrid g = dw_grid(H, Wd);
        dim3 grid(g.tiles_x * g.tiles_y, B * C);
        SEGX_DW_ROWS_DISPATCH(true, dY, W, dX, C, OH, OW, H, Wd, k - 1 - pad_t, k - 1 - pad_l, g.tiles_x, g.txw_log2);
        return check_launch("segx_dwconv2d_bwd_data");
    }
    if (stride == 2 && Wd % 8 == 0 && OW % 4 == 0 && pad_t == pad_l && ((reinterpret_cast<uintptr_t>(dY) | reinterpret_cast<uintptr_t>(dX)) & 15) == 0) {
        int l = 3;
        while (l < 6 && (8 << l) < Wd) ++l;
        const int tiles_x = (Wd + (8 << l) - 1) / (8 << l), tiles_y = (H + segx::DWB_TY - 1) / segx::DWB_TY;
        const int64_t ngroups = (int64_t)B * C * tiles_x * tiles_y, nblocks = ((ngroups << l) + 255) / 256;
#define SEGX_DWB(KK, PP)                                                                                                             \
        if (k == KK && pad_l == PP && nblocks <= 2147483647LL) {                                                                      \
            hipLaunchKernelGGL((segx::dwconv_bwd4s2_kernel<KK, PP, PP>), dim3((unsigned)nblocks), dim3(256), 0, stream, dY, W, dX, C, \
                               H, Wd, OH, OW, tiles_x, tiles_y, l, ngroups);                                                          \
            return check_launch("segx_dwconv2d_bwd_data");                                                                            \
        }
        SEGX_DWB(3, 0) SEGX_DWB(3, 1) SEGX_DWB(5, 1) SEGX_DWB(5, 2)
#undef SEGX_DWB
    }
    const int tx = (Wd + 15) / 16, ty = (H + 15) / 16;
    dim3 grid(tx * ty, B * C);
    SEGX_DW_DISPATCH(dwconv_bwd_data_kernel, dY, W, dX, C, H, Wd, OH, OW, pad_t, pad_l, tx);
    return check_launch("segx_dwconv2d_bwd_data");
}
extern "C" int segx_dwconv2d_bwd_weight_direct(const float* dY, const float* X, float* dW, int B, int C, int H, int Wd, int OH, int OW,
                                               int k, int stride, int pad_t, int pad_l, void* stream_) {
    SEGX_STREAM; SEGX_REQUIRE(dY && X && dW && B > 0 && C > 0 && OH > 0 && OW > 0, "segx_dwconv2d_bwd_weight_direct: bad args");
    if (B > 8 || dw_wgrad_strips(OH, OW) != 1 || !dw4_ok(dY, X, Wd, OW)) return 0;
    const Dw4Grid g = dw4_grid(OW);
    const int rows = (64 >> g.tpr_log2) * segx::DWG_TY, ntiles = g.tiles_x * ((OH + rows - 1) / rows);
#define SEGX_DW4C(KK, SS, PP)                                                                                                       \
    if (k == KK && stride == SS && pad_l == PP) {                                                                                    \
        hipLaunchKernelGGL((segx::dwconv_wgrad4c_kernel<KK, SS, PP>), dim3(C), dim3(512), 0, stream, dY, X, dW, B, C, H, Wd, OH, OW,  \
                           pad_t, g.tiles_x, ntiles, g.tpr_log2);                                                                     \
        const int rc = check_launch("segx_dwconv2d_bwd_weight_direct");                                                               \
        return rc ? (rc > 0 ? -rc - 1000 : rc) : 1;                                                                                  \
    }
    SEGX_DW4C(3, 1, 1) SEGX_DW4C(5, 1, 2) SEGX_DW4C(3, 2, 0) SEGX_DW4C(3, 2, 1) SEGX_DW4C(5, 2, 1) SEGX_DW4C(5, 2, 2)
#undef SEGX_DW4C
    return 0;
}
static int dw_fused_strips(int H, int Wd, int OH, int OW, int k, int stride, int pad_t, int pad_l) {
    if (stride != 1 || (k != 3 && k != 5) || pad_t != (k - 1) / 2 || pad_l != (k - 1) / 2 || OH != H || OW != Wd || Wd % 4 != 0 || Wd < 4) return 0;
    const Dw4Grid g = dw4_grid(Wd);
    const int tiles_y = (H + segx::DW4_TY - 1) / segx::DW4_TY, gpp = g.tiles_x * tiles_y, gpw = 64 >> g.tpr_log2;
    return gpp % gpw == 0 ? gpp / gpw : 0;
}
extern "C" int64_t segx_dwconv2d_bwd_fused_rows(int H, int Wd, int OH, int OW, int k, int stride, int pad_t, int pad_l) {
    return dw_fused_strips(H, Wd, OH, OW, k, stride, pad_t, pad_l);
}
extern "C" int segx_dwconv2d_bwd_fused(const float* dY, const float* X, const float* W, float* dX, float* part , int B, int C, int H, int Wd,
                                       int OH, int OW, int k, int stride, int pad_t, int pad_l, void* stream_) {
    SEGX_STREAM; SEGX_REQUIRE(dY && X && W && dX && part && B > 0 && C > 0 && (int64_t)B * C <= 65535, "segx_dwconv2d_bwd_fused: bad args");
    const int strips = dw_fused_strips(H, Wd, OH, OW, k, stride, pad_t, pad_l);
    SEGX_REQUIRE(strips > 0 && ((reinterpret_cast<uintptr_t>(dY) | reinterpret_cast<uintptr_t>(X) | reinterpret_cast<uintptr_t>(dX)) & 15) == 0,
                 "segx_dwconv2d_bwd_fused: shape not served (segx_dwconv2d_bwd_fused_rows == 0) or unaligned tensors");
    const Dw4Grid g = dw4_grid(Wd);
    const int tiles_y = (H + segx::DW4_TY - 1) / segx::DW4_TY;
    const int64_t ngroups = (int64_t)B * C * g.tiles_x * tiles_y, nblocks = ((ngroups << g.tpr_log2) + 255) / 256;
    SEGX_REQUIRE(nblocks <= 2147483647LL, "segx_dwconv2d_bwd_fused: too many workgroups");
    if (k == 3) hipLaunchKernelGGL((segx::dwconv_bwd_s1_fused_kernel<3>), dim3((unsigned)nblocks), dim3(256), 0, stream, dY, X, W, dX, part, C, H, Wd, g.tiles_x, tiles_y, g.tpr_log2, ngroups, strips);
    else hipLaunchKernelGGL((segx::dwconv_bwd_s1_fused_kernel<5>), dim3((unsigned)nblocks), dim3(256), 0, stream, dY, X, W, dX, part, C, H, Wd, g.tiles_x, tiles_y, g.tpr_log2, ngroups, strips);
    return check_launch("segx_dwconv2d_bwd_fused");
}
extern "C" int64_t segx_dwconv2d_wgrad_rows(int OH, int OW) { return OH > 0 && OW > 0 ? dw_wgrad_strips(OH, OW) : 0; }
extern "C" int segx_dwconv2d_bwd_weight(const float* dY, const float* X, float* part , int B, int C, int H, int Wd, int OH, int OW,
                                        int k, int stride, int pad_t, int pad_l, void* stream_) {
    SEGX_STREAM; SEGX_REQUIRE(dY && X && part && B > 0 && C > 0 && OH > 0 && OW > 0 && (int64_t)B * C <= 65535, "segx_dwconv2d_bwd_weight: bad args");
    const int strips = dw_wgrad_strips(OH, OW);
    if (dw4_ok(dY, X, Wd, OW) && dw4_wgrad_launch(stream, dY, X, part, B, C, H, Wd, OH, OW, k, stride, pad_t, pad_l, strips))
        return check_launch("segx_dwconv2d_bwd_weight");
    const DwGrid g = dw_grid(OH, OW);
    dim3 grid(strips, B * C);
    SEGX_DW_DISPATCH(dwconv_wgrad_rows_kernel, dY, X, part, C, H, Wd, OH, OW, pad_t, pad_l, g.tiles_x, g.tiles_x * g.tiles_y, g.txw_log2);
    return check_launch("segx_dwconv2d_bwd_weight");
}
extern "C" int segx_plane_scale(const float* X, const float* gate, float* Y, int64_t planes, int64_t S, void* stream_) {
    SEGX_STREAM; SEGX_REQUIRE(X && gate && Y && planes > 0 && S > 0 && planes <= 65535, "segx_plane_scale: bad args");
    hipLaunchKernelGGL(plane_scale_kernel, dim3(plane_chunks(S, 8), (unsigned)planes), dim3(256), 0, stream, X, gate, Y, S);
    return check_launch("segx_plane_scale");
}
extern "C" int segx_plane_bias_add(const float* X, const float* bias, float* Y, int64_t planes, int C, int64_t S, void* stream_) {
    SEGX_STREAM; SEGX_REQUIRE(X && bias && Y && planes > 0 && C > 0 && S > 0 && planes <= 65535, "segx_plane_bias_add: bad args");
    hipLaunchKernelGGL(plane_bias_add_kernel, dim3(plane_chunks(S, 8), (unsigned)planes), dim3(256), 0, stream, X, bias, Y, C, S);
    return check_launch("segx_plane_bias_add");
}
extern "C" int segx_plane_dot(const float* A, const float* Bm, float* out, int64_t planes, int64_t S, void* stream_) {
    SEGX_STREAM; SEGX_REQUIRE(A && Bm && out && planes > 0 && S > 0 && planes < 2147483647LL, "segx_plane_dot: bad args");
    hipLaunchKernelGGL(plane_dot_kernel, dim3((unsigned)planes), dim3(256), 0, stream, A, Bm, out, S);
    return check_launch("segx_plane_dot");
}
extern "C" int segx_bn_dw_s2_ok(int B, int C, int H, int W, int k, int stride, int pad_t, int pad_l) { return s2_serves(B, C, H, W, k, stride, pad_t, pad_l) ? 1 : 0; }
extern "C" int64_t segx_bn_dw_s2_ws_floats(int B, int C, int H, int W, int backward) {
    const int kp = H > 0 && W > 0 ? s2_kp(B, (int64_t)H * W, backward != 0) : 0;
    return kp ? (int64_t)C * B * bn_team_chunks((int64_t)H * W, kp) * (TEAM_SLOT + TEAM_MBOX) : 0;
}
extern "C" int64_t segx_bn_dw_s2_rows(int B, int H, int W) {
    const int kp = H > 0 && W > 0 ? s2_kp(B, (int64_t)H * W, true) : 0;
    return kp ? (int64_t)B * bn_team_chunks((int64_t)H * W, kp) : 0;
}
static int s2_team(BnTeam& t, float* ws, int64_t ws_floats, int B, int C, int64_t S, int kp, const char* what) {
    t.B = B; t.cpp = bn_team_chunks(S, kp); t.slots = ws; t.mbox = ws + (int64_t)C * B * t.cpp * TEAM_SLOT;
    team_fill(t);
    SEGX_REQUIRE(B * t.cpp <= team_cap() && (int64_t)C * B * t.cpp < 2147483647LL, "%s: team of %d workgroups", what, B * t.cpp);
    const int64_t need = (int64_t)C * B * t.cpp * (TEAM_SLOT + TEAM_MBOX);
    SEGX_REQUIRE(ws_floats >= need, "%s: the scratch holds %lld floats, this call needs %lld (segx_bn_dw_s2_ws_floats under the current knob 3)", what, (long long)ws_floats, (long long)need);
    return 0;
}
extern "C" int segx_bn_dw_s2_fwd(const float* E, const float* w0, const float* b0, float* run_mean, float* run_var, const float* Wdw, float* D, float* mean, float* var,
                                 float* ws, float momentum, float eps, int B, int C, int H, int W, int k, int pad_t, int pad_l, int64_t ws_floats, void* stream_) {
    SEGX_STREAM; SEGX_REQUIRE(E && w0 && b0 && Wdw && D && mean && var && ws && (!run_mean == !run_var), "segx_bn_dw_s2_fwd: bad args");
    SEGX_REQUIRE(s2_serves(B, C, H, W, k, 2, pad_t, pad_l), "segx_bn_dw_s2_fwd: shape not served (segx_bn_dw_s2_ok == 0)");
    SEGX_REQUIRE(((reinterpret_cast<uintptr_t>(E) | reinterpret_cast<uintptr_t>(D)) & 15) == 0, "segx_bn_dw_s2_fwd: tensors must be 16-byte aligned");
    const int64_t S = (int64_t)H * W;
    const int kp = s2_kp(B, S, false);
    BnTeam t;
    if (int rc = s2_team(t, ws, ws_floats, B, C, S, kp, "segx_bn_dw_s2_fwd")) return rc;
    BnDwS2Args g; memset(&g, 0, sizeof(g));
    g.E = E; g.w = w0; g.b = b0; g.Wdw = Wdw; g.mean = mean; g.var = var; g.D = D; g.run_mean = run_mean; g.run_var = run_var; g.momentum = momentum;
    g.eps = eps; g.C = C; g.H = H; g.W4 = W / 4; g.pt = pad_t;
    const dim3 tg = team_grid((int64_t)C * B * t.cpp);
#define SEGX_S2(KP) (k == 3 ? s2_launch_fwd<KP, 3>(g, t, tg, stream, pad_l) : s2_launch_fwd<KP, 5>(g, t, tg, stream, pad_l))
    return kp == 4 ? SEGX_S2(4) : kp == 16 ? SEGX_S2(16) : SEGX_S2(32);
#undef SEGX_S2
}
extern "C" int segx_bn_dw_s2_bwd(const float* dD, const float* E, const float* mean, const float* var, const float* w0, const float* b0, const float* Wdw,
                                 float* dE, float* dw0, float* db0, float* part, float* ws, float eps, int B, int C, int H, int W, int k, int pad_t, int pad_l,
                                 int64_t part_rows, int64_t ws_floats, void* stream_) {
    SEGX_STREAM; SEGX_REQUIRE(dD && E && mean && var && w0 && b0 && Wdw && dE && dw0 && db0 && part && ws, "segx_bn_dw_s2_bwd: bad args");
    SEGX_REQUIRE(s2_serves(B, C, H, W, k, 2, pad_t, pad_l), "segx_bn_dw_s2_bwd: shape not served (segx_bn_dw_s2_ok == 0)");
    SEGX_REQUIRE(((reinterpret_cast<uintptr_t>(E) | reinterpret_cast<uintptr_t>(dD) | reinterpret_cast<uintptr_t>(dE)) & 15) == 0, "segx_bn_dw_s2_bwd: tensors must be 16-byte aligned");
    const int64_t S = (int64_t)H * W;
    const int kp = s2_kp(B, S, true);
    BnTeam t;
    if (int rc = s2_team(t, ws, ws_floats, B, C, S, kp, "segx_bn_dw_s2_bwd")) return rc;
    SEGX_REQUIRE(part_rows >= (int64_t)B * t.cpp, "segx_bn_dw_s2_bwd: the filter-gradient partials hold %lld rows, this call writes %d (segx_bn_dw_s2_rows under the current knob 3)",
                 (long long)part_rows, B * t.cpp);
    BnDwS2Args g; memset(&g, 0, sizeof(g));
    g.E = E; g.w = w0; g.b = b0; g.Wdw = Wdw; g.mean = const_cast<float*>(mean); g.var = const_cast<float*>(var); g.dD = dD; g.dE = dE; g.dw = dw0; g.db = db0; g.part = part;
    g.eps = eps; g.C = C; g.H = H; g.W4 = W / 4; g.pt = pad_t;
    const dim3 tg = team_grid((int64_t)C * B * t.cpp);
#define SEGX_S2(KP) (k == 3 ? s2_launch_bwd<KP, 3>(g, t, tg, stream, pad_l) : s2_launch_bwd<KP, 5>(g, t, tg, stream, pad_l))
    return kp == 4 ? SEGX_S2(4) : SEGX_S2(16);
#undef SEGX_S2
}
```

segtran_amd/efficientnet/model.py:

```python
import math
import torch
from torch import nn
from torch.nn import functional as F

from .. import functional as SF
from ..fold import FoldableBackbone, fold_conv_bn, pair_sources

BN_MOM, BN_EPS = 1 - 0.99, 1e-3

_BASE = [(1, 3, 1, 1, 32, 16, 0.25), (2, 3, 2, 6, 16, 24, 0.25), (2, 5, 2, 6, 24, 40, 0.25), (3, 3, 2, 6, 40, 80, 0.25),
         (3, 5, 1, 6, 80, 112, 0.25), (4, 5, 2, 6, 112, 192, 0.25), (1, 3, 1, 6, 192, 320, 0.25)]
_PARAMS = {'efficientnet-b0': (1.0, 1.0, 224, 0.2), 'efficientnet-b1': (1.0, 1.1, 240, 0.2),
           'efficientnet-b2': (1.1, 1.2, 260, 0.3), 'efficientnet-b3': (1.2, 1.4, 300, 0.3),
           'efficientnet-b4': (1.4, 1.8, 380, 0.4), 'efficientnet-b5': (1.6, 2.2, 456, 0.4),
           'efficientnet-b6': (1.8, 2.6, 528, 0.5), 'efficientnet-b7': (2.0, 3.1, 600, 0.5)}


def round_filters(filters, width, divisor=8):
    filters *= width
    new = max(divisor, int(filters + divisor / 2) // divisor * divisor)
    if new < 0.9 * filters:
        new += divisor
    return int(new)


def round_repeats(repeats, depth):
    return int(math.ceil(depth * repeats))


class Conv2dStaticSamePadding(nn.Conv2d):

    def __init__(self, in_channels, out_channels, kernel_size, stride=1, image_size=None, **kwargs):
        super().__init__(in_channels, out_channels, kernel_size, stride, **kwargs)
        ih = iw = image_size
        kh, kw = self.weight.shape[-2:]
        sh, sw = self.stride
        oh, ow = math.ceil(ih / sh), math.ceil(iw / sw)
        ph = max((oh - 1) * sh + (kh - 1) * self.dilation[0] + 1 - ih, 0)
        pw = max((ow - 1) * sw + (kw - 1) * self.dilation[1] + 1 - iw, 0)
        self.static_pad = (pw // 2, pw - pw // 2, ph // 2, ph - ph // 2)
        self.pointwise = (kh == 1 and kw == 1 and sh == 1 and sw == 1 and self.groups == 1)

    def forward(self, x, pass_input=False):
        if self.pointwise:
            return SF.conv1x1(x, self.weight, self.bias, pass_input=pass_input)
        if self.groups == self.in_channels and self.groups == self.out_channels and self.bias is None:
            return SF.dwconv2d(x, self.weight, self.stride[0], self.static_pad)
        assert self.groups == 1 and self.bias is None and self.dilation == (1, 1)
        return SF.conv2d_dense(x, self.weight, self.stride[0], self.static_pad)


def swish(x):
    return x * torch.sigmoid(x)


def drop_connect(x, p, training):
    if not training:
        return x
    keep = 1 - p
    r = keep + torch.rand([x.shape[0], 1, 1, 1], dtype=x.dtype, device=x.device)
    return x / keep * torch.floor(r)


class MBConvBlock(nn.Module):
    def __init__(self, k, s, e, cin, cout, se_ratio, image_size):
        super().__init__()
        self.stride, self.expand_ratio, self.input_filters, self.output_filters = s, e, cin, cout
        oup = cin * e
        if e != 1:
            self._expand_conv = Conv2dStaticSamePadding(cin, oup, 1, image_size=image_size, bias=False)
            self._bn0 = nn.BatchNorm2d(oup, momentum=BN_MOM, eps=BN_EPS)
        self._depthwise_conv = Conv2dStaticSamePadding(oup, oup, k, stride=s, image_size=image_size, groups=oup, bias=False)
        self._bn1 = nn.BatchNorm2d(oup, momentum=BN_MOM, eps=BN_EPS)
        nsq = max(1, int(cin * se_ratio))
        self._se_reduce = Conv2dStaticSamePadding(oup, nsq, 1, image_size=1)
        self._se_expand = Conv2dStaticSamePadding(nsq, oup, 1, image_size=1)
        self._project_conv = Conv2dStaticSamePadding(oup, cout, 1, image_size=math.ceil(image_size / s), bias=False)
        self._bn2 = nn.BatchNorm2d(cout, momentum=BN_MOM, eps=BN_EPS)

    gate_in_weights = True
    fused_middle = True

    fused_entry = True

    def _takes_fused_entry(self, x):
        if not (MBConvBlock.fused_entry and self.training and SF._bn_stats_sync is None and self.expand_ratio != 1):
            return False
        dw = self._depthwise_conv
        if not (self._bn0.training and dw.stride == (2, 2) and dw.kernel_size[0] == dw.kernel_size[1] and x.dim() == 4 and x.dtype == torch.float32):
            return False
        return SF.bn_dw_s2_ok((x.shape[0], dw.in_channels, x.shape[2], x.shape[3]), dw.kernel_size[0], 2, dw.static_pad)

    def _takes_fused_middle(self, x):
        if not (MBConvBlock.fused_middle and MBConvBlock.gate_in_weights and self.training and SF._bn_stats_sync is None and self.expand_ratio != 1):
            return False
        dw = self._depthwise_conv
        k = dw.kernel_size[0]
        if not (self._bn0.training and self._bn1.training and dw.stride == (1, 1) and dw.kernel_size == (k, k) and tuple(dw.static_pad) == (k // 2,) * 4):
            return False
        return x.dim() == 4 and x.dtype == torch.float32 and SF.mbconv_mid_ok((x.shape[0], dw.in_channels, x.shape[2], x.shape[3]), k)

    def folded_operands(self):
        f0 = fold_conv_bn(self._expand_conv.weight, self._bn0) if self.expand_ratio != 1 else None
        return f0, fold_conv_bn(self._depthwise_conv.weight, self._bn1), fold_conv_bn(self._project_conv.weight, self._bn2)

    def forward_folded(self, inputs, folded):
        f0, (w1, b1), (w2, b2) = folded
        x = inputs
        skip = self.stride == 1 and self.input_filters == self.output_filters
        if f0 is not None:
            x = SF.conv1x1(x, f0[0], f0[1], act=SF.ACT_SWISH)
        dw = self._depthwise_conv
        y, psum, nch = SF.dwconv2d_bias_act_pool(x, w1, b1, dw.stride[0], dw.static_pad, SF.ACT_SWISH)
        Wb = SF.se_gate_weights(y, psum, nch, self._se_reduce.weight, self._se_reduce.bias, self._se_expand.weight, self._se_expand.bias, w2)
        return SF.conv1x1_per_sample_bias(y, Wb, b2, resid=inputs if skip else None)

    def forward(self, inputs, drop_connect_rate=None):
        x = skip_in = inputs
        skip = self.stride == 1 and self.input_filters == self.output_filters
        fused = self._takes_fused_middle(x)
        entry = not fused and self._takes_fused_entry(x)
        if entry:
            dw = self._depthwise_conv
            d = SF.bn_act_dwconv_s2(self._expand_conv(x), self._bn0, dw.weight, dw.stride[0], dw.static_pad)
        elif self.expand_ratio != 1 and not fused:
            x = SF.bn_act(self._expand_conv(x), self._bn0, SF.ACT_SWISH)
        se = (self._se_reduce.weight, self._se_reduce.bias, self._se_expand.weight, self._se_expand.bias)
        rate = float(drop_connect_rate) if (skip and drop_connect_rate and self.training) else 0.0
        if fused:
            y, Wb = SF.mbconv_mid(self._expand_conv(x), self._bn0, self._depthwise_conv.weight, self._bn1, *se, self._project_conv.weight)
            x = SF.conv1x1_per_sample(y, Wb)
        elif MBConvBlock.gate_in_weights:
            y, Wb = SF.bn_act_gate_weights(d if entry else self._depthwise_conv(x), self._bn1, SF.ACT_SWISH, *se, self._project_conv.weight)
            x = SF.conv1x1_per_sample(y, Wb)
        else:
            x = self._project_conv(SF.bn_act_se(d if entry else self._depthwise_conv(x), self._bn1, SF.ACT_SWISH, *se))
        return SF.bn_act(x, self._bn2, SF.ACT_NONE, resid=skip_in if skip else None, drop_connect=rate)


class EfficientNet(FoldableBackbone, nn.Module):
    def __init__(self, model_name='efficientnet-b4', stem_stride=2, drop_connect_rate=0.2, num_classes=1000):
        super().__init__()
        width, depth, res, _ = _PARAMS[model_name]
        self.drop_connect_rate = drop_connect_rate
        self.stem_stride = stem_stride
        c0 = round_filters(32, width)
        self._conv_stem = Conv2dStaticSamePadding(3, c0, 3, stride=stem_stride, image_size=res, bias=False)
        self._bn0 = nn.BatchNorm2d(c0, momentum=BN_MOM, eps=BN_EPS)
        size = math.ceil(res / 2)
        self._blocks = nn.ModuleList([])
        self.endpoint_seg_indices = [0, 1, 2, 4]
        self.endpoint_blk_indices = []
        for i, (r, k, s, e, cin, cout, se) in enumerate(_BASE):
            cin, cout, r = round_filters(cin, width), round_filters(cout, width), round_repeats(r, depth)
            self._blocks.append(MBConvBlock(k, s, e, cin, cout, se, size))
            size = math.ceil(size / s)
            for _ in range(r - 1):
                self._blocks.append(MBConvBlock(k, 1, e, cout, cout, se, size))
            if i in self.endpoint_seg_indices:
                self.endpoint_blk_indices.append(len(self._blocks))
        chead = round_filters(1280, width)
        self._conv_head = Conv2dStaticSamePadding(cout, chead, 1, image_size=size, bias=False)
        self._bn1 = nn.BatchNorm2d(chead, momentum=BN_MOM, eps=BN_EPS)
        self._fc = nn.Linear(chead, num_classes)

    def _fold_build(self):
        pairs = [(self._conv_stem, self._bn0), (self._conv_head, self._bn1)] + \
                [(c, b) for blk in self._blocks for c, b in ((getattr(blk, '_expand_conv', None), getattr(blk, '_bn0', None)), (blk._depthwise_conv, blk._bn1),
                                                            (blk._project_conv, blk._bn2)) if c is not None]
        return (fold_conv_bn(self._conv_stem.weight, self._bn0), [blk.folded_operands() for blk in self._blocks],
                fold_conv_bn(self._conv_head.weight, self._bn1)), pair_sources(pairs)

    def _extract_endpoints_folded(self, inputs):
        (ws, bs), blocks, (wh, bh) = self._folded[:3]
        endpoints = {}
        with torch.no_grad():
            x = SF.conv2d_stem_bias_act(inputs, ws, bs, self._conv_stem.stride[0], self._conv_stem.static_pad, SF.ACT_SWISH)
            prev_x = x
            for idx, block in enumerate(self._blocks):
                x = block.forward_folded(x, blocks[idx])
                if idx in self.endpoint_blk_indices:
                    endpoints['reduction_%d' % (len(endpoints) + 1)] = prev_x
                prev_x = x
            endpoints['reduction_%d' % (len(endpoints) + 1)] = SF.conv1x1(x, wh, bh, act=SF.ACT_SWISH)
        return endpoints

    @classmethod
    def from_name(cls, model_name, stem_stride=2, **kw):
        return cls(model_name, stem_stride=stem_stride, **kw)

    @classmethod
    def from_pretrained(cls, model_name, weights_path=None, advprop=False, ignore_missing_keys=False, stem_stride=2, **kw):
        model = cls.from_name(model_name, stem_stride=stem_stride, **kw)
        load_pretrained_weights(model, model_name, weights_path=weights_path, load_fc=True, advprop=advprop,
                                ignore_missing_keys=ignore_missing_keys)
        return model

    def extract_endpoints(self, inputs):
        if self.batchnorm_folded:
            return self._extract_endpoints_folded(inputs)
        endpoints = {}
        x = SF.bn_act(self._conv_stem(inputs), self._bn0, SF.ACT_SWISH)
        prev_x = x
        nblk = len(self._blocks)
        for idx, block in enumerate(self._blocks):
            rate = self.drop_connect_rate * float(idx) / nblk if self.drop_connect_rate else None
            x = block(x, drop_connect_rate=rate)
            if idx in self.endpoint_blk_indices:
                endpoints['reduction_%d' % (len(endpoints) + 1)] = prev_x
            prev_x = x
        x = SF.bn_act(self._conv_head(x), self._bn1, SF.ACT_SWISH)
        endpoints['reduction_%d' % (len(endpoints) + 1)] = x
        return endpoints


PRETRAINED_FILES = {False: {'efficientnet-b0': 'efficientnet-b0-355c32eb.pth', 'efficientnet-b1': 'efficientnet-b1-f1951068.pth',
                            'efficientnet-b2': 'efficientnet-b2-8bb594d6.pth', 'efficientnet-b3': 'efficientnet-b3-5fb5a3c3.pth',
                            'efficientnet-b4': 'efficientnet-b4-6ed6700e.pth', 'efficientnet-b5': 'efficientnet-b5-b6417697.pth',
                            'efficientnet-b6': 'efficientnet-b6-c76e70fd.pth', 'efficientnet-b7': 'efficientnet-b7-dcc49843.pth'},
                    True: {'efficientnet-b0': 'adv-efficientnet-b0-b64d5a18.pth', 'efficientnet-b1': 'adv-efficientnet-b1-0f3ce85a.pth',
                           'efficientnet-b2': 'adv-efficientnet-b2-6e9d97e5.pth', 'efficientnet-b3': 'adv-efficientnet-b3-cdd7c0f4.pth',
                           'efficientnet-b4': 'adv-efficientnet-b4-44fb3a87.pth', 'efficientnet-b5': 'adv-efficientnet-b5-86493f6b.pth',
                           'efficientnet-b6': 'adv-efficientnet-b6-ac80338e.pth', 'efficientnet-b7': 'adv-efficientnet-b7-4652b6dd.pth',
                           'efficientnet-b8': 'adv-efficientnet-b8-22a8fe65.pth'}}


def pretrained_path(model_name, advprop=False):
    import os
    d = os.environ.get('SEGX_PRETRAINED_DIR')
    if not d:
        raise RuntimeError('pretrained %s weights: no network access here -- download %s and pass weights_path=..., or put it '
                           'under $SEGX_PRETRAINED_DIR (or build with use_pretrained=False)' % (model_name, PRETRAINED_FILES[advprop][model_name]))
    path = os.path.join(d, PRETRAINED_FILES[advprop][model_name])
    if not os.path.exists(path):
        raise RuntimeError('pretrained weights not found: ' + path)
    return path


def load_pretrained_weights(model, model_name, weights_path=None, load_fc=True, advprop=False, ignore_missing_keys=False):
    state_dict = torch.load(weights_path if isinstance(weights_path, str) else pretrained_path(model_name, advprop), map_location='cpu')
    if not load_fc:
        state_dict.pop('_fc.weight'); state_dict.pop('_fc.bias')
    ret = model.load_state_dict(state_dict, strict=False)
    if not ignore_missing_keys:
        expect = set() if load_fc else {'_fc.weight', '_fc.bias'}
        assert set(ret.missing_keys) == expect, 'Missing keys when loading pretrained weights: %s' % ret.missing_keys
    assert not ret.unexpected_keys, 'Unexpected keys when loading pretrained weights: %s' % ret.unexpected_keys
```

segtran_amd/functional.py:

```python
import math
import torch
import torch.nn.functional as F
from . import segx
from .segx import EPI_NONE, EPI_GELU, EPI_SWISH, EPI_RELU, BIAS_NONE, BIAS_N, BIAS_M

LN_EPS = 1e-12


_MRO = torch.autograd.Function.__mro__
_fast_apply = torch._C._FunctionBase in _MRO and not any('apply' in c.__dict__ for c in _MRO[1:_MRO.index(torch._C._FunctionBase)])


class _Fn(torch.autograd.Function):

    @classmethod
    def apply(cls, *args):
        if _fast_apply and not torch._C._are_functorch_transforms_active():
            return super(torch.autograd.Function, cls).apply(*args)
        return super().apply(*args)


def _live(t):
    return t.requires_grad and torch.is_grad_enabled()

# ... 940 lines not shown
        if ctx.needs_input_grad[0]:
            dx = torch.empty_like(x)
            L.dwconv2d_bwd_data(dy, w, dx, B, C, H, W, OH, OW, k, stride, pt, pl)
        if ctx.needs_input_grad[1]:
            dw = _empty(x, C * k * k)
            if not L.dwconv2d_bwd_weight_direct(dy, x, dw, B, C, H, W, OH, OW, k, stride, pt, pl):
                rows = B * L.dwconv2d_wgrad_rows(OH, OW)
                part = _empty(x, rows, C * k * k)
                L.dwconv2d_bwd_weight(dy, x, part, B, C, H, W, OH, OW, k, stride, pt, pl)
                L.colsum(part, dw, _empty(x, L.colreduce_ws(rows, C * k * k, 1)), rows, C * k * k)
            dw = dw.view_as(w)
        return dx, dw, None, None


def dwconv2d(x, w, stride, pad):
    return _DWConv.apply(x, w, int(stride), tuple(int(p) for p in pad))


def _se_excite(L, x, psum, nch, S, w1, b1, w2, b2, Wproj=None):
    B, C = x.shape[0], x.shape[1]
    Cs = w1.shape[0]
    W1, W2 = _c(w1.reshape(Cs, C)), _c(w2.reshape(C, Cs))
    p, hpre, gate = _empty(x, B, C), _empty(x, B, Cs), _empty(x, B, C)
    M = Wproj.shape[0] if Wproj is not None else 0
    Wb = _empty(x, B, M, C) if Wproj is not None else None
    L.se_fwd2(psum, nch, 1.0 / S, W1, b1, W2, b2, Wproj, p, hpre, gate, Wb, B, C, Cs, M)
    return p, hpre, gate, W1, W2, Wb


def _se_excite_backward(L, x, dWb, Wproj, dgate, gate, hpre, p, W1, W2, S):
    B, C = gate.shape
    Cs = hpre.shape[1]
    dpool = _empty(x, B * C)
    dW1, db1, dW2, db2 = _empty(x, Cs, C), _empty(x, Cs), _empty(x, C, Cs), _empty(x, C)
    dWproj = torch.empty_like(Wproj) if Wproj is not None else None
    M = Wproj.shape[0] if Wproj is not None else 0
    L.se_bwd2(dWb, Wproj, dgate, gate, hpre, p, W1, W2, 1.0 / S, dpool, dW1, db1, dW2, db2, dWproj, _empty(x, L.se_ws2(B, C, Cs)), B, C, Cs, M)
    return dpool, dW1, db1, dW2, db2, dWproj


class _BNActSE(_Fn):

    @staticmethod
    def forward(ctx, x, w, b, run_mean, run_var, training, momentum, eps, act, w1, b1, w2, b2):
        L = segx.lib()
        x = _c(x)
        B, C = x.shape[0], x.shape[1]
        S = x.numel() // (B * C)
        y, mean, var, n, psum, nch = _bn_forward(L, x, w, b, run_mean, run_var, training, momentum, eps, act, B, C, S, pool=True)
        p, hpre, gate, W1, W2, _ = _se_excite(L, x, psum, nch, S, w1, b1, w2, b2)
        z = torch.empty_like(x)
        L.plane_scale(y, gate, z, B * C, S)
        ctx.cfg = (B, C, S, eps, act, training, n)
        ctx.shapes = (tuple(w1.shape), tuple(w2.shape))
        ctx.save_for_backward(x, mean, var, w, b, y, p, hpre, gate, W1, W2)
        return z

    @staticmethod
    def backward(ctx, dz):
        L = segx.lib()
        x, mean, var, w, b, y, p, hpre, gate, W1, W2 = ctx.saved_tensors
        B, C, S = ctx.cfg[:3]
        w1s, w2s = ctx.shapes
        dz = _c(dz)
        dgate = _empty(x, B * C)
        L.plane_dot(dz, y, dgate, B * C, S)
        dpool, dW1, db1, dW2, db2, _ = _se_excite_backward(L, x, None, None, dgate, gate, hpre, p, W1, W2, S)
        dx, dw, db = _bn_act_backward(L, dz, x, mean, var, w, b, ctx.cfg, gate.reshape(-1), dpool, 1.0)
        return dx, dw, db, None, None, None, None, None, None, dW1.view(w1s), db1, dW2.view(w2s), db2


class _BNActGateW(_Fn):

    @staticmethod
    def forward(ctx, x, w, b, run_mean, run_var, training, momentum, eps, act, w1, b1, w2, b2, Wproj):
        L = segx.lib()
        x = _c(x)
        B, C = x.shape[0], x.shape[1]
        S = x.numel() // (B * C)
        Wp = _c(Wproj.reshape(Wproj.shape[0], C))
        y, mean, var, n, psum, nch = _bn_forward(L, x, w, b, run_mean, run_var, training, momentum, eps, act, B, C, S, pool=True)
        p, hpre, gate, W1, W2, Wb = _se_excite(L, x, psum, nch, S, w1, b1, w2, b2, Wp)
        ctx.cfg = (B, C, S, eps, act, training, n)
        ctx.shapes = (tuple(w1.shape), tuple(w2.shape), tuple(Wproj.shape))
        ctx.save_for_backward(x, mean, var, w, b, p, hpre, gate, W1, W2, Wp)
        return y, Wb

    @staticmethod
    def backward(ctx, dy, dWb):
        L = segx.lib()
        x, mean, var, w, b, p, hpre, gate, W1, W2, Wp = ctx.saved_tensors
        S = ctx.cfg[2]
        w1s, w2s, wps = ctx.shapes
        dWb = _c(dWb) if dWb is not None else torch.zeros(gate.shape[0], Wp.shape[0], Wp.shape[1], dtype=torch.float32, device=x.device)
        dpool, dW1, db1, dW2, db2, dWp = _se_excite_backward(L, x, dWb, Wp, None, gate, hpre, p, W1, W2, S)
        dx, dw, db = _bn_act_backward(L, _c(dy), x, mean, var, w, b, ctx.cfg, None, dpool, 1.0)
        return dx, dw, db, None, None, None, None, None, None, dW1.view(w1s), db1, dW2.view(w2s), db2, dWp.view(wps)


def bn_act_gate_weights(x, bn, act, w1, b1, w2, b2, proj_weight):
    _bn_tick(bn)
    return _BNActGateW.apply(x, bn.weight, bn.bias, bn.running_mean, bn.running_var, bn.training, float(bn.momentum), float(bn.eps), act, w1, b1, w2, b2,
                             proj_weight)


class _MBConvMid(_Fn):

    @staticmethod
    def forward(ctx, e, w0, b0, rm0, rv0, mom0, eps0, wdw, w1, b1, rm1, rv1, mom1, eps1, sw1, sb1, sw2, sb2, Wproj):
        L = segx.lib()
        e, wdw = _c(e), _c(wdw)
        if e.data_ptr() % 16:
            e = e.clone()
        B, C, H, W = e.shape
        k, S = wdw.shape[-1], H * W
        Wp = _c(Wproj.reshape(Wproj.shape[0], C))
        d, y = torch.empty_like(e), torch.empty_like(e)
        psum, stats = _empty(e, B * C), _empty(e, 4, C)
        L.mbconv_mid_fwd(e, w0, b0, rm0, rv0, wdw, w1, b1, rm1, rv1, d, y, psum, stats[0], stats[1], stats[2], stats[3], mom0, eps0, mom1, eps1, B, C, H, W, k)
        p, hpre, gate, W1, W2, Wb = _se_excite(L, y, psum, 1, S, sw1, sb1, sw2, sb2, Wp)
        ctx.cfg = (B, C, H, W, k, eps0, eps1)
        ctx.shapes = (tuple(sw1.shape), tuple(sw2.shape), tuple(Wproj.shape), tuple(wdw.shape))
        ctx.save_for_backward(e, d, stats, w0, b0, wdw, w1, b1, p, hpre, gate, W1, W2, Wp)
        return y, Wb

    @staticmethod
    def backward(ctx, dy, dWb):
        L = segx.lib()
        e, d, stats, w0, b0, wdw, w1, b1, p, hpre, gate, W1, W2, Wp = ctx.saved_tensors
        B, C, H, W, k, eps0, eps1 = ctx.cfg
        w1s, w2s, wps, wds = ctx.shapes
        dWb = _c(dWb) if dWb is not None else torch.zeros(B, Wp.shape[0], C, dtype=torch.float32, device=e.device)
        dy = _c(dy) if dy is not None else torch.zeros_like(e)
        if dy.data_ptr() % 16:
            dy = dy.clone()
        dpool, dW1, db1, dW2, db2, dWp = _se_excite_backward(L, e, dWb, Wp, None, gate, hpre, p, W1, W2, H * W)
        de, g, dwd = torch.empty_like(e), _empty(e, 4, C), _empty(e, C * k * k)
        L.mbconv_mid_bwd(dy, dpool, d, e, stats[0], stats[1], stats[2], stats[3], w0, b0, w1, b1, wdw, de, g[0], g[1], g[2], g[3], dwd, 1.0, eps0, eps1, B, C, H, W, k)
        return (de, g[0], g[1], None, None, None, None, dwd.view(wds), g[2], g[3], None, None, None, None,
                dW1.view(w1s), db1, dW2.view(w2s), db2, dWp.view(wps))


def mbconv_mid_ok(e_shape, k):
    return len(e_shape) == 4 and segx.lib().mbconv_mid_ok(e_shape[0], e_shape[1], e_shape[2], e_shape[3], int(k))


def mbconv_mid(e, bn0, dw_weight, bn1, w1, b1, w2, b2, proj_weight):
    _bn_tick(bn0)
    _bn_tick(bn1)
    return _MBConvMid.apply(e, bn0.weight, bn0.bias, bn0.running_mean, bn0.running_var, float(bn0.momentum), float(bn0.eps), dw_weight,
                            bn1.weight, bn1.bias, bn1.running_mean, bn1.running_var, float(bn1.momentum), float(bn1.eps), w1, b1, w2, b2, proj_weight)


class _BNActDWConvS2(_Fn):

    @staticmethod
    def forward(ctx, e, w0, b0, rm0, rv0, mom0, eps0, wdw, pt, pl):
        L = segx.lib()
        e, wdw = _c(e), _c(wdw)
        if e.data_ptr() % 16:
            e = e.clone()
        B, C, H, W = e.shape
        k = wdw.shape[-1]
        d, stats = _empty(e, B, C, H // 2, W // 2), _empty(e, 2, C)
        L.bn_dw_s2_fwd(e, w0, b0, rm0, rv0, wdw, d, stats[0], stats[1], _empty(e, L.bn_dw_s2_ws(B, C, H, W, False)), mom0, eps0, B, C, H, W, k, pt, pl)
        ctx.cfg = (B, C, H, W, k, pt, pl, eps0, tuple(wdw.shape))
        ctx.save_for_backward(e, stats, w0, b0, wdw)
        return d

    @staticmethod
    def backward(ctx, dd):
        L = segx.lib()
        e, stats, w0, b0, wdw = ctx.saved_tensors
        B, C, H, W, k, pt, pl, eps0, wds = ctx.cfg
        dd = _c(dd)
        if dd.data_ptr() % 16:
            dd = dd.clone()
        rows = L.bn_dw_s2_rows(B, H, W)
        de, g, part = torch.empty_like(e), _empty(e, 2, C), _empty(e, rows, C * k * k)
        L.bn_dw_s2_bwd(dd, e, stats[0], stats[1], w0, b0, wdw, de, g[0], g[1], part, _empty(e, L.bn_dw_s2_ws(B, C, H, W, True)), eps0, B, C, H, W, k, pt, pl)
        dwd = _empty(e, C * k * k)
        L.colsum(part, dwd, _empty(e, L.colreduce_ws(rows, C * k * k, 1)), rows, C * k * k)
        return de, g[0], g[1], None, None, None, None, dwd.view(wds), None, None


def bn_dw_s2_ok(e_shape, k, stride, pad):
    if len(e_shape) != 4:
        return False
    B, C, H, W = (int(v) for v in e_shape)
    pl, pr, pt, pb = (int(p) for p in pad)
    if int(stride) != 2 or H % 2 or W % 2 or (H + pt + pb - k) // 2 + 1 != H // 2 or (W + pl + pr - k) // 2 + 1 != W // 2:
        return False
    return segx.lib().bn_dw_s2_ok(B, C, H, W, int(k), int(stride), pt, pl)


def bn_act_dwconv_s2(e, bn0, dw_weight, stride, static_pad):
    assert int(stride) == 2
    _bn_tick(bn0)
    return _BNActDWConvS2.apply(e, bn0.weight, bn0.bias, bn0.running_mean, bn0.running_var, float(bn0.momentum), float(bn0.eps), dw_weight,
                                int(static_pad[2]), int(static_pad[0]))


def conv1x1_per_sample(x, Wb, bias=None):
    B, Cin = x.shape[0], x.shape[1]
    S = x.numel() // (B * Cin)
    Cout = Wb.shape[1]
    if bias is None:
        spec = GemmSpec(Cout, S, Cin, (Cout * Cin, 0, Cin, 1), (Cin * S, 0, 1, S), (Cout * S, 0, S), (B, Cout) + tuple(x.shape[2:]), nb=(B, 1))
        return bgemm(Wb, x, spec)
    spec = GemmSpec(Cout, S, Cin, (Cout * Cin, 0, Cin, 1), (Cin * S, 0, 1, S), (Cout * S, 0, S), (B, Cout) + tuple(x.shape[2:]), nb=(B, 1), bias_mode=BIAS_M, bias_b0=Cout)
    return bgemm(Wb, x, spec, bias=_c(bias))


def dwconv2d_bias_act_pool(x, w, bias, stride, pad, act=ACT_SWISH, pool=True):
    if act not in (ACT_NONE, ACT_SWISH):
        raise NotImplementedError('dwconv2d_bias_act_pool: act is ACT_NONE or ACT_SWISH')
    _no_grad_operands('dwconv2d_bias_act_pool', x, w, bias)
    L = segx.lib()
    x, w = _c(x), _c(w)
    B, C, H, W = x.shape
    k, stride = w.shape[-1], int(stride)
    pl, pr, pt, pb = (int(v) for v in pad)
    OH, OW = (H + pt + pb - k) // stride + 1, (W + pl + pr - k) // stride + 1
    y = _empty(x, B, C, OH, OW)
    nch = L.dwconv2d_pool_chunks(OH, OW) if pool else 0
    psum = _empty(x, B * C * nch) if pool else None
    L.dwconv2d_bias_act_pool(x, w, _c(bias), y, psum, B, C, H, W, OH, OW, k, stride, pt, pl, act)
    return y, psum, nch


def se_gate_weights(y, psum, nch, w1, b1, w2, b2, proj_weight):
    _no_grad_operands('se_gate_weights', psum, w1, b1, w2, b2, proj_weight)
    B, C = y.shape[0], y.shape[1]
    S = y.numel() // (B * C)
    return _se_excite(segx.lib(), y, psum, nch, S, w1, b1, w2, b2, _c(proj_weight.reshape(proj_weight.shape[0], C)))[5]


def conv1x1_per_sample_bias(x, Wb, bias, resid=None):
    _no_grad_operands('conv1x1_per_sample_bias', x, Wb, bias, resid)
    B, Cin = x.shape[0], x.shape[1]
    S = x.numel() // (B * Cin)
    Cout = Wb.shape[1]
    x, Wb = _c(x), _c(Wb)
    y = _empty(x, B, Cout, *x.shape[2:])
    kw = dict(resid=_c(resid)) if resid is not None else {}
    assert resid is None or resid.shape == y.shape
    _run_gemm(segx.lib(), Wb, x, y, Cout, S, Cin, (Cout * Cin, 0, Cin, 1), (Cin * S, 0, 1, S), (Cout * S, 0, S), (B, 1), 1.0, bias=_c(bias), bias_mode=BIAS_M, **kw)
    return y


def bn_act_se(x, bn, act, w1, b1, w2, b2):
    _bn_tick(bn)
    return _BNActSE.apply(x, bn.weight, bn.bias, bn.running_mean, bn.running_var, bn.training, float(bn.momentum), float(bn.eps), act, w1, b1, w2, b2)


class _GroupNorm(_Fn):
    @staticmethod
    def forward(ctx, x, w, b, G, eps):
        L = segx.lib()
        x = _c(x)
        B, C = x.shape[:2]
        S = x.numel() // (B * C)
        y = torch.empty_like(x)
        mean, rstd = _empty(x, B * G), _empty(x, B * G)
        L.groupnorm_fwd(x, w, b, y, mean, rstd, _empty(x, L.gn_ws(B, C, G)), B, C, G, S, eps)
        ctx.cfg = (B, C, G, S)
        ctx.save_for_backward(x, w, mean, rstd)
        return y

    @staticmethod
    def backward(ctx, dy):
        L = segx.lib()
        x, w, mean, rstd = ctx.saved_tensors
        B, C, G, S = ctx.cfg
        dx = torch.empty_like(x)
        dw, db = _empty(x, C), _empty(x, C)
        L.groupnorm_bwd(_c(dy), x, w, mean, rstd, dx, dw, db, _empty(x, L.gn_ws(B, C, G)), B, C, G, S)
        return dx, dw, db, None, None


def group_norm(x, gn):
    return _GroupNorm.apply(x, gn.weight, gn.bias, int(gn.num_groups), float(gn.eps))


def _dhw(shape):
    sp = tuple(int(v) for v in shape)
    return (1,) + sp if len(sp) == 2 else sp


def _corner_scale(n_in, n_out):
    return -((n_in - 1) / (n_out - 1)) if n_out > 1 and n_in > 1 else -1e-6


class _InterpAdd(_Fn):
    @staticmethod
    def forward(ctx, x, base, size, align_corners=False):
        L = segx.lib()
        x = _c(x)
        B, C = x.shape[:2]
        d, h, w = _dhw(x.shape[2:])
        D, H, W = _dhw(size)
        base = _c(base) if base is not None else None
        axes = [(ax, n_in, n_out) for ax, (n_in, n_out) in enumerate(((d, D), (h, H), (w, W))) if n_in != n_out]
        ctx.align = bool(align_corners)
        if d != D and h != H and not align_corners and W % 4 == 0:
            cur = x
            if w != W:
                cur = _empty(x, B * C * d * h * W)
                L.interp_fwd_axis(x, None, cur, B * C * d * h, w, W, 1, 0.0)
            out = _empty(x, B, C, *size)
            L.interp_fwd_axis2(cur, base, out, B * C, d, D, h, H, W)
        elif (D > 1 or align_corners) and axes:
            cur, dims = x, [d, h, w]
            for k, (ax, n_in, n_out) in enumerate(sorted(axes, reverse=True)):
                outer = B * C
                for a in range(ax):
                    outer *= dims[a]
                inner = 1
                for a in range(ax + 1, 3):
                    inner *= dims[a]
                last = k == len(axes) - 1
                nxt = _empty(x, B, C, *size) if last else _empty(x, outer * n_out * inner)
                L.interp_fwd_axis(cur, base if last else None, nxt, outer, n_in, n_out, inner, _corner_scale(n_in, n_out) if align_corners else 0.0)
                cur, dims[ax] = nxt, n_out
            out = cur
        elif align_corners:
            out = x.clone() if base is None else x + base
        else:
            out = _empty(x, B, C, *size)
            L.interp_fwd(x, base, out, B * C, d, h, w, D, H, W)
        ctx.cfg = (B * C, d, h, w, D, H, W, tuple(x.shape))
        return out

    @staticmethod
    def backward(ctx, dy):
        L = segx.lib()
        planes, d, h, w, D, H, W, xshape = ctx.cfg
        dy = _c(dy)
        dx = None
        if ctx.needs_input_grad[0] and d != D and h != H and not ctx.align and W % 4 == 0:
            dx = _interp_bwd_yz_x(L, dy, planes, d, h, w, D, H, W).view(xshape)
        if ctx.needs_input_grad[0] and dx is None:
            cur, dims = dy, [D, H, W]
            for ax, n_in in ((0, d), (1, h), (2, w)):
                if dims[ax] == n_in:
                    continue
                outer = planes
                for a in range(ax):
                    outer *= dims[a]
                inner = 1
                for a in range(ax + 1, 3):
                    inner *= dims[a]
                nxt = _empty(dy, outer * n_in * inner)
# ... 1308 lines not shown
```

segtran_amd/segx.py:

```python
import contextlib
import ctypes
import enum
import os
import torch

_HERE = os.path.dirname(os.path.abspath(__file__))
LIB_PATH = os.path.join(_HERE, 'lib', 'libsegx.so')

c_f = ctypes.c_float
c_i = ctypes.c_int32
c_l = ctypes.c_int64
c_u = ctypes.c_uint64
c_p = ctypes.c_void_p


class GemmDesc(ctypes.Structure):
    _fields_ = [('M', c_i), ('N', c_i), ('K', c_i), ('nb0', c_i), ('nb1', c_i),
                ('a_b0', c_l), ('a_b1', c_l), ('a_m', c_l), ('a_k', c_l),
                ('b_b0', c_l), ('b_b1', c_l), ('b_n', c_l), ('b_k', c_l),
                ('c_b0', c_l), ('c_b1', c_l), ('c_m', c_l),
                ('alpha', c_f), ('epilogue', c_i), ('bias_mode', c_i), ('bias_b1', c_l),
                ('bias', c_p), ('aux', c_p), ('gmax', c_p),
                ('dropout_p', c_f), ('seed', c_u), ('offset', c_u),
                ('splitk', c_i), ('workspace', c_p), ('tile', c_i), ('bias_b0', c_l), ('batch_reduce', c_i), ('engine', c_i),
# ... 210 lines not shown
                    raise AssertionError('tensors on different devices')
                assert a.is_contiguous(), name + ': non-contiguous tensor'
                conv.append(a.data_ptr())
            else:
                conv.append(a)
        rc = getattr(self.c, name)(*conv, self.stream(ref))
        if rc:
            self.check(rc, name)

    def colreduce_ws(self, rows, C, nout):
        return int(self.c.segx_colreduce_ws_floats(rows, C, nout))

    def softmax_fwd(self, S, P, Pdrop, rows, L, clip, gmax, p, seed, offset):
        self._call('segx_softmax_fwd', S, S, P, Pdrop, rows, L, clip, gmax, p, seed, offset)

    def softmax_bwd(self, P, dPd, S, dS, rows, L, clip, gmax, p, seed, offset):
        self._call('segx_softmax_bwd', P, P, dPd, S, dS, rows, L, clip, gmax, p, seed, offset)

    def posbias_fwd(self, S, out, table, nmat, N, geom, weight, clip, gmax):
        self._chk_t(S, out, table, gmax)
        rc = self.c.segx_posbias_fwd(_ptr(S), _ptr(out), _ptr(table), nmat, N, self._geom(geom), weight, clip, _ptr(gmax), self.stream(out))
        self.check(rc, 'segx_posbias_fwd')

    def posbias_bwd(self, dOut, S, dS, dtable, nmat, N, geom, weight, clip):
        self._chk_t(dOut, S, dS, dtable)
        rc = self.c.segx_posbias_bwd(_ptr(dOut), _ptr(S), _ptr(dS), _ptr(dtable), nmat, N, self._geom(geom), weight, clip, self.stream(dtable))
        self.check(rc, 'segx_posbias_bwd')

    def layernorm_fwd(self, X, w, b, Y, mean, rstd, rows, C, eps):
        self._call('segx_layernorm_fwd', X, X, w, b, Y, mean, rstd, rows, C, eps)

    def layernorm_bwd(self, dY, X, w, mean, rstd, dX, rows, C):
        self._call('segx_layernorm_bwd', X, dY, X, w, mean, rstd, dX, rows, C)

    def colsum(self, X, out, ws, rows, C):
        self._call('segx_colsum', X, X, out, ws, rows, C)

    def ln_param_grad(self, dY, X, mean, rstd, dw, db, ws, rows, C):
        self._call('segx_ln_param_grad', X, dY, X, mean, rstd, dw, db, ws, rows, C)

    def rowsum(self, X, out, R, S):
        self._call('segx_rowsum', X, X, out, R, S)

    def sum(self, x, n, out, ws, scale=1.0):
        self._call('segx_sum', x, x, n, out, ws, scale)

    def prenorm_fwd(self, X, w1, b1, pos, pos_ld, pw, mask, Y, stats, B, N, C, eps, p, seed, offset):
        self._call('segx_prenorm_fwd', X, X, w1, b1, pos, pos_ld, pw, mask, Y, stats, B, N, C, eps, p, seed, offset)

    def prenorm_bwd(self, dY, X, w1, b1, pos, pos_ld, pw, mask, stats, dX, dU, B, N, C, p, seed, offset):
        self._call('segx_prenorm_bwd', X, dY, X, w1, b1, pos, pos_ld, pw, mask, stats, dX, dU, B, N, C, p, seed, offset)

    def prenorm_bwd_all_ws(self, N, C):
        return int(self.c.segx_prenorm_bwd_all_ws_floats(N, C))

    def prenorm_bwd_all(self, dY, X, w1, b1, pos, pos_ld, pos_weight, mask, stats, dX, dsum, dw, db, ws, B, N, C, p, seed, offset):
        self._call('segx_prenorm_bwd_all', X, dY, X, w1, b1, pos, pos_ld, pos_weight, mask, stats, dX, dsum, dw, db, ws, B, N, C, p, seed, offset)

    def posembed_fwd(self, posn, Wp, bp, out, stats, N, C, pd, eps):
        self._call('segx_posembed_fwd', out, posn, Wp, bp, out, stats, N, C, pd, eps)

    def posembed_bwd(self, dOut, posn, Wp, bp, stats, dZ, N, C, pd):
        self._call('segx_posembed_bwd', dOut, dOut, posn, Wp, bp, stats, dZ, N, C, pd)

    def modes_aggr_fwd(self, Z, lnw, lnb, wa, ba, Y, stats, Mo, R, F, eps, p, seed, offset):
        self._call('segx_modes_aggr_fwd', Z, Z, lnw, lnb, wa, ba, Y, stats, Mo, R, F, eps, p, seed, offset)

    def modes_aggr_bwd(self, dY, Z, lnw, lnb, wa, stats, dZ, dscore, Mo, R, F, p, seed, offset):
        self._call('segx_modes_aggr_bwd', Z, dY, Z, lnw, lnb, wa, stats, dZ, dscore, Mo, R, F, p, seed, offset)

    def modes_aggr_param_grad(self, dY, Z, lnw, lnb, wa, stats, dscore, dlnw, dlnb, dwa, ws, Mo, R, F, p, seed, offset):
        self._call('segx_modes_aggr_param_grad', Z, dY, Z, lnw, lnb, wa, stats, dscore, dlnw, dlnb, dwa, ws, Mo, R, F,
                   p, seed, offset)

    def modes_aggr_bwd_all_ws(self, Mo, R, F):
        return int(self.c.segx_modes_aggr_bwd_all_ws_floats(Mo, R, F))

    def modes_aggr_bwd_all(self, dY, Z, lnw, lnb, wa, stats, dZ, dscore, dlnw, dlnb, dwa, ws, Mo, R, F, p, seed, offset):
        self._call('segx_modes_aggr_bwd_all', Z, dY, Z, lnw, lnb, wa, stats, dZ, dscore, dlnw, dlnb, dwa, ws, Mo, R, F, p, seed, offset)

    def gelu_bwd_colsum_ws(self, rows, N):
        return int(self.c.segx_gelu_bwd_colsum_ws_floats(rows, N))

    def gelu_bwd_colsum(self, dH, T, dT, colsum, ws, rows, N, p, seed, offset):
        self._call('segx_gelu_bwd_colsum', dH, dH, T, dT, colsum, ws, rows, N, p, seed, offset)

    def gelu_bwd(self, dH, T, dT, n, p, seed, offset):
        self._call('segx_gelu_bwd', T, dH, T, dT, n, p, seed, offset)

    def loss_ws(self, B, C):
        return int(self.c.segx_loss_ws_floats(B, C))

    def seg_loss_fwd(self, logits, mask, pw, cw, out, ws, B, C, S, dice_w):
        self._call('segx_seg_loss_fwd', logits, logits, mask, pw, cw, out, ws, B, C, S, dice_w)

    def seg_loss_bwd(self, logits, mask, pw, cw, ws, gout, dlogits, B, C, S, dice_w):
        self._call('segx_seg_loss_bwd', logits, logits, mask, pw, cw, ws, gout, dlogits, B, C, S, dice_w)

    def bn_ws(self, B, C, S=0):
        return int(self.c.segx_bn_ws_floats(B, C, S))

    def plane_chunks(self, S):
        return int(self.c.segx_plane_chunks(S))

    def bn_pool_chunks(self, B, S, auto_stats):
        return int(self.c.segx_bn_pool_chunks(B, S, 1 if auto_stats else 0))

    def bn_parts_floats(self, B, C, S=0):
        return int(self.c.segx_bn_parts_floats(B, C, S))

    def bn_stats_local(self, X, part, ws, B, C, S):
        self._call('segx_bn_stats_local', X, X, part, ws, B, C, S)

    def bn_act_fwd2(self, X, parts, nparts, mean, var, run_mean, run_var, momentum, w, b, Y, psum, resid, dc_p, seed, offset, B, C, S, eps, act, y_bs=0):
        if y_bs:
            self._chk_t(Y)
            assert Y.device == X.device and Y.dtype == torch.float32 and Y.stride(1) == S and Y.stride(0) == y_bs and Y[0].is_contiguous()
            Y = Y.data_ptr()
        self._call('segx_bn_act_fwd2', X, X, parts, nparts, mean, var, run_mean, run_var, momentum, w, b, Y, psum, resid, float(dc_p), seed, offset, B, C, S, eps, act,
                   0 if parts is None else parts.numel(), int(y_bs))

    def bn_act_bwd2(self, dY, X, mean, var, w, b, dX, dw, db, ws, B, C, S, eps, act, training, gate=None, dpool=None, inv_S=0.0, dc_p=0.0, seed=0, offset=0, dy_bs=0):
        self._chk_t(dY, X, mean, var, w, b, dX, dw, db, ws, gate, dpool)
        for t in (X, mean, var, w, b, dX, dw, db, ws):
            assert t.is_contiguous()
        assert dy_bs or dY.is_contiguous()
        rc = self.c.segx_bn_act_bwd2(_ptr(dY), _ptr(X), _ptr(mean), _ptr(var), _ptr(w), _ptr(b), _ptr(dX), _ptr(dw), _ptr(db), _ptr(ws), B, C, S, eps, act, training,
                                     _ptr(gate), _ptr(dpool), float(inv_S), float(dc_p), seed, offset, int(dy_bs), ws.numel(), self.stream(X))
        self.check(rc, 'segx_bn_act_bwd2')

    def se_fwd2(self, psum, nch, inv_S, W1, b1, W2, b2, Wproj, p, hpre, gate, Wb, B, C, Cs, M):
        self._call('segx_se_fwd2', gate, psum, nch, inv_S, W1, b1, W2, b2, Wproj, p, hpre, gate, Wb, B, C, Cs, M)

    def se_ws2(self, B, C, Cs):
        return int(self.c.segx_se_ws2_floats(B, C, Cs))

    def se_bwd2(self, dWb, Wproj, dgate, gate, hpre, p, W1, W2, inv_S, dpool, dW1, db1, dW2, db2, dWproj, ws, B, C, Cs, M):
        self._call('segx_se_bwd2', gate, dWb, Wproj, dgate, gate, hpre, p, W1, W2, inv_S, dpool, dW1, db1, dW2, db2, dWproj, ws, B, C, Cs, M)

    def bn_dw_s2_ok(self, B, C, H, W, k, stride, pt, pl):
        return bool(self.c.segx_bn_dw_s2_ok(B, C, H, W, k, stride, pt, pl))

    def bn_dw_s2_ws(self, B, C, H, W, backward):
        return int(self.c.segx_bn_dw_s2_ws_floats(B, C, H, W, 1 if backward else 0))

    def bn_dw_s2_rows(self, B, H, W):
        return int(self.c.segx_bn_dw_s2_rows(B, H, W))

    def bn_dw_s2_fwd(self, E, w0, b0, rm, rv, Wdw, D, mean, var, ws, mom, eps, B, C, H, W, k, pt, pl):
        self._call('segx_bn_dw_s2_fwd', E, E, w0, b0, rm, rv, Wdw, D, mean, var, ws, float(mom), float(eps), B, C, H, W, k, pt, pl, ws.numel())

    def bn_dw_s2_bwd(self, dD, E, mean, var, w0, b0, Wdw, dE, dw0, db0, part, ws, eps, B, C, H, W, k, pt, pl):
        self._call('segx_bn_dw_s2_bwd', dD, dD, E, mean, var, w0, b0, Wdw, dE, dw0, db0, part, ws, float(eps), B, C, H, W, k, pt, pl, part.shape[0], ws.numel())

    def mbconv_mid_ok(self, B, C, H, W, k):
        return bool(self.c.segx_mbconv_mid_ok(B, C, H, W, k))

    def mbconv_mid_fwd(self, E, w0, b0, rm0, rv0, Wdw, w1, b1, rm1, rv1, D, Y, psum, mean0, var0, mean1, var1, mom0, eps0, mom1, eps1, B, C, H, W, k):
        self._call('segx_mbconv_mid_fwd', E, E, w0, b0, rm0, rv0, Wdw, w1, b1, rm1, rv1, D, Y, psum, mean0, var0, mean1, var1, float(mom0), float(eps0), float(mom1), float(eps1),
                   B, C, H, W, k)

    def mbconv_mid_bwd(self, dY, dpool, D, E, mean0, var0, mean1, var1, w0, b0, w1, b1, Wdw, dE, dw0, db0, dw1, db1, dWdw, inv_S, eps0, eps1, B, C, H, W, k):
        self._call('segx_mbconv_mid_bwd', dY, dY, dpool, D, E, mean0, var0, mean1, var1, w0, b0, w1, b1, Wdw, dE, dw0, db0, dw1, db1, dWdw, float(inv_S), float(eps0), float(eps1),
                   B, C, H, W, k)

    def dwconv2d_fwd(self, X, W, Y, B, C, H, Wd, OH, OW, k, stride, pt, pl):
        self._call('segx_dwconv2d_fwd', X, X, W, Y, B, C, H, Wd, OH, OW, k, stride, pt, pl)

    def dwconv2d_pool_chunks(self, OH, OW):
        return int(self.c.segx_dwconv2d_pool_chunks(OH, OW))

    def dwconv2d_bias_act_pool(self, X, W, bias, Y, psum, B, C, H, Wd, OH, OW, k, stride, pt, pl, act):
        self._call('segx_dwconv2d_bias_act_pool', X, X, W, bias, Y, psum, B, C, H, Wd, OH, OW, k, stride, pt, pl, act)

    def dwconv2d_bwd_data(self, dY, W, dX, B, C, H, Wd, OH, OW, k, stride, pt, pl):
        self._call('segx_dwconv2d_bwd_data', dY, dY, W, dX, B, C, H, Wd, OH, OW, k, stride, pt, pl)

    def dwconv2d_bwd_weight_direct(self, dY, X, dW, B, C, H, Wd, OH, OW, k, stride, pt, pl):
        self._chk_t(dY, X, dW)
        rc = self.c.segx_dwconv2d_bwd_weight_direct(_ptr(dY), _ptr(X), _ptr(dW), B, C, H, Wd, OH, OW, k, stride, pt, pl, self.stream(X))
        if rc < 0:
            self.check(rc, 'segx_dwconv2d_bwd_weight_direct')
        return rc == 1

    def dwconv2d_bwd_fused_rows(self, H, W, OH, OW, k, stride, pad_t, pad_l):
        return int(self.c.segx_dwconv2d_bwd_fused_rows(H, W, OH, OW, k, stride, pad_t, pad_l))

    def dwconv2d_bwd_fused(self, dY, X, W, dX, part, B, C, H, Wd, OH, OW, k, stride, pad_t, pad_l):
        self._call('segx_dwconv2d_bwd_fused', dY, dY, X, W, dX, part, B, C, H, Wd, OH, OW, k, stride, pad_t, pad_l)

    def dwconv2d_wgrad_rows(self, OH, OW):
        return int(self.c.segx_dwconv2d_wgrad_rows(OH, OW))

    def dwconv2d_bwd_weight(self, dY, X, part, B, C, H, Wd, OH, OW, k, stride, pt, pl):
        self._call('segx_dwconv2d_bwd_weight', dY, dY, X, part, B, C, H, Wd, OH, OW, k, stride, pt, pl)

    def plane_scale(self, X, gate, Y, planes, S):
        self._call('segx_plane_scale', X, X, gate, Y, planes, S)

    def bn_act_bwd_reduce(self, dY, X, mean, var, w, b, dw, db, ws, B, C, S, eps, act, gate=None, dpool=None, inv_S=0.0, dc_p=0.0, seed=0, offset=0):
        self._call('segx_bn_act_bwd_reduce', X, dY, X, mean, var, w, b, dw, db, ws, B, C, S, eps, act, gate, dpool, float(inv_S), float(dc_p), seed, offset)

    def bn_act_bwd_apply(self, dY, X, mean, var, w, b, sdw, sdb, dX, B, C, S, eps, act, inv_n, gate=None, dpool=None, inv_S=0.0, dc_p=0.0, seed=0, offset=0):
        self._call('segx_bn_act_bwd_apply', X, dY, X, mean, var, w, b, sdw, sdb, dX, B, C, S, eps, act, inv_n, gate, dpool, float(inv_S), float(dc_p), seed, offset)

    def add_relu_fwd(self, Z, R, bias, Y, planes, C, S):
        self._call('segx_add_relu_fwd', Y, Z, R, bias, Y, planes, C, S)

    def add_relu_bwd(self, dY, Y, dZ, planes, S):
        self._call('segx_add_relu_bwd', dZ, dY, Y, dZ, planes, S)

    def plane_bias_add(self, X, bias, Y, planes, C, S):
        self._call('segx_plane_bias_add', X, X, bias, Y, planes, C, S)

    def plane_dot(self, A, B, out, planes, S):
        self._call('segx_plane_dot', A, A, B, out, planes, S)

    def interp_fwd_axis2(self, inp, base, out, outer, n1_in, n1_out, n2_in, n2_out, inner):
        self._call('segx_interp_linear_fwd_axis2', inp, inp, base, out, outer, n1_in, n1_out, n2_in, n2_out, inner)

    def interp_bwd_axis2(self, dout, din, outer, n1_out, n1_in, n2_out, n2_in, inner):
        self._call('segx_interp_linear_bwd_axis2', dout, dout, din, outer, n1_out, n1_in, n2_out, n2_in, inner)

    def gn_ws(self, B, C, G):
        return int(self.c.segx_gn_ws_floats(B, C, G))

    def groupnorm_fwd(self, X, w, b, Y, mean, rstd, ws, B, C, G, S, eps):
        self._call('segx_groupnorm_fwd', X, X, w, b, Y, mean, rstd, ws, B, C, G, S, eps)

    def groupnorm_bwd(self, dY, X, w, mean, rstd, dX, dw, db, ws, B, C, G, S, plane_dx_sums=None):
        self._call('segx_groupnorm_bwd', X, dY, X, w, mean, rstd, dX, dw, db, ws, B, C, G, S, plane_dx_sums)

    def interp_gn_nparts(self, per4, cpg):
        return int(self.c.segx_interp_gn_nparts(int(per4), int(cpg)))

    def interp_fwd_axis2_gn(self, x, base, out, outer, n1_in, n1_out, n2_in, n2_out, inner, cpg, parts, nparts):
        self._call('segx_interp_linear_fwd_axis2_gn', x, x, base, out, outer, n1_in, n1_out, n2_in, n2_out, inner, cpg, parts, nparts)

    def groupnorm_stats_parts(self, parts, nparts, mean, rstd, BG, eps):
        self._call('segx_groupnorm_stats_parts', parts, parts, nparts, mean, rstd, BG, eps)

    def gn_fold_bwd(self, Gd, X, mean, rstd, A, Bc, dX, plane_sums, ws, B, C, G, S):
        self._call('segx_gn_fold_bwd', X, Gd, X, mean, rstd, A, Bc, dX, plane_sums, ws, B, C, G, S)

    def gn_fold_bwd_proj(self, dOut, Wb, NC, X, mean, rstd, A, Bc, dX, plane_sums, ws, B, C, G, S):
        self._call('segx_gn_fold_bwd_proj', X, dOut, Wb, NC, X, mean, rstd, A, Bc, dX, plane_sums, ws, B, C, G, S)

    def bridge_mask(self, X, Wb, bb, out, B, Cb, C3, H, W, D, kd, kh, kw):
        self._call('segx_bridge_mask', X, X, Wb, bb, out, B, Cb, C3, H, W, D, kd, kh, kw)

    def groupnorm_fwd_parts(self, X, parts, nparts, w, b, Y, mean, rstd, B, C, G, S, eps):
        self._call('segx_groupnorm_fwd_parts', X, X, parts, nparts, w, b, Y, mean, rstd, B, C, G, S, eps)

    def interp_fwd(self, inp, base, out, planes, d, h, w, D, H, W):
        self._call('segx_interp_linear_fwd', inp, inp, base, out, planes, d, h, w, D, H, W)

    def interp_fwd_axis(self, inp, base, out, outer, n_in, n_out, inner, src_scale=0.0):
        self._call('segx_interp_linear_fwd_axis', inp, inp, base, out, outer, n_in, n_out, inner, float(src_scale))

    def resized_crop3d(self, X, Y, planes, geom):
        self._chk_t(X, Y)
        self.check(self.c.segx_resized_crop3d(_ptr(X), _ptr(Y), planes, self._geom(geom), self.stream(Y)), 'segx_resized_crop3d')

    def axis_gather(self, X, Y, planes, geom):
        self._chk_t(X, Y)
        self.check(self.c.segx_axis_gather(_ptr(X), _ptr(Y), planes, self._geom(geom), self.stream(Y)), 'segx_axis_gather')

    def pixel_shuffle2(self, X, Y, planes, h, w, inverse):
        self._call('segx_pixel_shuffle2', X, X, Y, planes, h, w, int(inverse))

    def add_noise(self, X, noise, Y, mu, sigma, nonzero_only, seed, offset):
        self._call('segx_add_noise', X, X, noise, Y, X.numel(), float(mu), float(sigma), int(nonzero_only), seed, offset)

    def resize2d(self, X, Y, planes, h, w, H, W, mode, quantize):
        self._call('segx_resize2d', X, X, Y, planes, h, w, H, W, mode, int(quantize))

    def color_blend(self, X, Y, B, HW, mode, factor, pivot, quantize):
        self._call('segx_color_blend', X, X, Y, B, HW, mode, factor, pivot, int(quantize))

    def gray_mean(self, X, mean, B, HW, quantize):
        ws = torch.empty(int(self.c.segx_gray_mean_ws_floats(B, HW)), dtype=torch.float32, device=X.device)
        self._call('segx_gray_mean', X, X, mean, ws, B, HW, int(quantize))

    def normalize(self, X, Y, B, C, HW, scale, mean, std):
        self._call('segx_normalize', X, X, Y, B, C, HW, float(scale), mean, std)

    def interp_bwd(self, dout, din, planes, d, h, w, D, H, W):
        self._call('segx_interp_linear_bwd', dout, dout, din, planes, d, h, w, D, H, W)

    @staticmethod
    def _geom(vals):
        return (ctypes.c_int32 * len(vals))(*[int(v) for v in vals])

    def _timed(self, ref, flops, tag, fn):
        if self.gemm_prof is not None and ref.is_cuda:
            e0, e1 = torch.cuda.Event(enable_timing=True), torch.cuda.Event(enable_timing=True)
            self.x6_launches()
            e0.record(); rc = fn(); e1.record()
            self.gemm_prof.append((e0, e1, flops, tag, self.x6_launches() > 0))
            return rc
        return fn()

    def avgpool2_fwd(self, X, Y, planes, H, W):
        self._call('segx_avgpool2_fwd', X, X, Y, planes, H, W)

    def avgpool2_bwd(self, dY, dX, planes, H, W):
# ... 131 lines not shown
        return Wq

    def conv3d_halo_fwd(self, X, Wq, Y, B, Cout, geom, x_bs=0, y_bs=0, mtile=0):
        self._chk_t(X, Wq, Y)
        P = geom[4] * geom[5] * geom[6]; K = geom[0] * 27
        call = lambda: self.c.segx_conv3d_halo_fwd(_ptr(X), _ptr(Wq), _ptr(Y), B, Cout, self._geom(geom), int(x_bs), int(y_bs), int(mtile), self.stream(Y))
        rc = self._timed(Y, 2.0 * B * Cout * P * K, ('conv3d_halo_fwd', Cout, P, K, B, 1), call)
        self.check(rc, 'segx_conv3d_halo_fwd')

    def conv3d_halo_bias_act_fwd(self, X, Wq, bias, Y, B, Cout, geom, x_bs=0, y_bs=0, mtile=0, act=2):
        self._chk_t(X, Wq, bias, Y)
        P = geom[4] * geom[5] * geom[6]; K = geom[0] * 27
        call = lambda: self.c.segx_conv3d_halo_bias_act_fwd(_ptr(X), _ptr(Wq), _ptr(bias), _ptr(Y), B, Cout, self._geom(geom), int(x_bs), int(y_bs), int(mtile), int(act), self.stream(Y))
        rc = self._timed(Y, 2.0 * B * Cout * P * K, ('conv3d_halo_fwd', Cout, P, K, B, 1), call)
        self.check(rc, 'segx_conv3d_halo_bias_act_fwd')

    def conv3d_halo_wgrad_ok(self, B, Cout, geom):
        return bool(self.c.segx_conv3d_halo_wgrad_ok(B, Cout, self._geom(geom)))

    def conv3d_halo_wgrad(self, dY, X, dW, B, Cout, geom, dy_bs=0, x_bs=0):
        self._chk_t(dY, X, dW)
        ws = torch.empty(int(self.c.segx_conv3d_halo_wgrad_ws_floats(B, Cout, self._geom(geom))), dtype=torch.float32, device=dW.device)
        P = geom[4] * geom[5] * geom[6]; N = geom[0] * 27
        call = lambda: self.c.segx_conv3d_halo_wgrad(_ptr(dY), _ptr(X), _ptr(dW), _ptr(ws), B, Cout, self._geom(geom), int(dy_bs), int(x_bs), self.stream(dW))
        rc = self._timed(dW, 2.0 * B * Cout * P * N, ('conv3d_halo_wgrad', Cout, N, P, B, 1), call)
        self.check(rc, 'segx_conv3d_halo_wgrad')

    def conv3d_bwd_data_direct(self, dY, W, dX, B, Cout, geom):
        wt = torch.empty(W.numel(), dtype=torch.float32, device=W.device)
        self._chk_t(dY, W, dX)
        rc = self.c.segx_conv3d_bwd_data_direct(_ptr(dY), _ptr(W), _ptr(dX), _ptr(wt), B, Cout, self._geom(geom), self.stream(dX))
        self.check(rc, 'segx_conv3d_bwd_data_direct')

    def stem_compose_fwd(self, Ws, Wb, bb, Wc, O, C3, Cb, Cc, T):
        self._call('segx_stem_compose_fwd', Wc, Ws, Wb, bb, Wc, O, C3, Cb, Cc, T)

    def stem_compose_bwd(self, dWc, Ws, Wb, bb, dWs, dWb, dbb, O, C3, Cb, Cc, T):
        self._call('segx_stem_compose_bwd', dWc, dWc, Ws, Wb, bb, dWs, dWb, dbb, O, C3, Cb, Cc, T)

    def conv2d_stem_fwd(self, X, W, Y, B, Cin, Cout, H, Wd, OH, OW, K, stride, pt, pl):
        self._call('segx_conv2d_stem_fwd', X, X, W, Y, B, Cin, Cout, H, Wd, OH, OW, K, stride, pt, pl)

    def conv2d_stem_bias_act_fwd(self, X, W, bias, Y, B, Cin, Cout, H, Wd, OH, OW, K, stride, pt, pl, act):
        self._call('segx_conv2d_stem_bias_act_fwd', X, X, W, bias, Y, B, Cin, Cout, H, Wd, OH, OW, K, stride, pt, pl, act)

    def conv2d_stem_im2col(self, X, Xcol, B, Cin, H, Wd, OH, OW, K, stride, pt, pl, rows):
        self._call('segx_conv2d_stem_im2col', X, X, Xcol, B, Cin, H, Wd, OH, OW, K, stride, pt, pl, rows)

    def stem_s2d_input(self, X, Y, B, Cb, H, W, D, U):
        self._call('segx_stem_s2d_input', X, X, Y, B, Cb, H, W, D, U)

    def bridge_input(self, X, Y, B, Cb, Cc, H, W, D):
        self._call('segx_bridge_input', X, X, Y, B, Cb, Cc, H, W, D)

    def nonzero_mask(self, X, out, B, C, D, H, W, kd, kh, kw):
        self._call('segx_nonzero_mask', X, X, out, B, C, D, H, W, kd, kh, kw)

    def label_nhot(self, labels, out, B, Cin, S, mode):
        self._call('segx_label_nhot', out, labels, out, B, Cin, S, mode)

    def conv3d_pack_weights(self, W, Wp, O, C, KV, mode):
        self._call('segx_conv3d_pack_weights', W, W, Wp, O, C, KV, mode)

    def conv3d_flip_weights(self, W, Wt, Cout, Cin, KV):
        self._call('segx_conv3d_flip_weights', W, W, Wt, Cout, Cin, KV)

    def conv3d_bwd_weight(self, dY, X, dWb, B, Cout, geom, splitk, ws, packed=False, dy_bs=0, x_bs=0):
        self._chk_t(dY, X, dWb, ws)
        g = [int(v) for v in geom]
        N, P = g[0] * g[7] * g[8] * g[9], g[4] * g[5] * g[6]
        if dy_bs or x_bs:
            assert packed
            call = lambda: self.c.segx_conv3d_bwd_weight_packed_bs(_ptr(dY), _ptr(X), _ptr(dWb), B, Cout, self._geom(geom), splitk, _ptr(ws), int(dy_bs), int(x_bs),
                                                                   self.stream(dWb))
        else:
            fn = self.c.segx_conv3d_bwd_weight_packed if packed else self.c.segx_conv3d_bwd_weight
            call = lambda: fn(_ptr(dY), _ptr(X), _ptr(dWb), B, Cout, self._geom(geom), splitk, _ptr(ws), self.stream(dWb))
        rc = self._timed(dWb, 2.0 * B * Cout * P * N, ('conv3d_wgrad', Cout, N, P, B, splitk), call)
        self.check(rc, 'segx_conv3d_bwd_weight')

    def conv3d_unpack_wgrad(self, dWp, dW, Cout, Cin, KV):
        self._call('segx_conv3d_unpack_wgrad', dWp, dWp, dW, Cout, Cin, KV)

    def maxpool3d_fwd(self, X, Y, arg, planes, geom):
        self._chk_t(X, Y, arg)
        rc = self.c.segx_maxpool3d_fwd(_ptr(X), _ptr(Y), _ptr(arg), planes, self._geom(geom), self.stream(Y))
        self.check(rc, 'segx_maxpool3d_fwd')

    def maxpool3d_bwd(self, dY, arg, dX, planes, geom, addend=None):
        self._chk_t(dY, arg, dX, addend)
        assert addend is None or (addend.is_contiguous() and addend.shape == dX.shape)
        rc = self.c.segx_maxpool3d_bwd(_ptr(dY), _ptr(arg), _ptr(dX), planes, self._geom(geom), _ptr(addend), self.stream(dX))
        self.check(rc, 'segx_maxpool3d_bwd')

    def dropout(self, x, y, n, p, seed, offset):
        self._call('segx_dropout', x, x, y, n, float(p), seed, offset)

    def interp_bwd_axis(self, dout, din, outer, n_out, n_in, inner, src_scale=0.0):
        self._call('segx_interp_linear_bwd_axis', dout, dout, din, outer, n_out, n_in, inner, float(src_scale))

    def mt_bertadam_step(self, tabs, ntensors, nchunks, chunk, max_global, max_tensor, sched, b1, b2, eps, ws):
        t = tabs
        self._call('segx_mt_bertadam_step', ws, t['params'], t['grads'], t['m'], t['v'], t['sizes'], t['chunk_tensor'],
                   t['chunk_off'], t['chunk_first'], t['active'], t['lr'], t['wd'], ntensors, nchunks, chunk,
                   max_global, max_tensor, sched, b1, b2, eps, ws)


    def mt_gather(self, src_tab, tabs, chunk_begin, nchunks, chunk):
        self._call('segx_mt_gather', src_tab, src_tab, tabs['grads'], tabs['sizes'], tabs['chunk_tensor'], tabs['chunk_off'],
                   chunk_begin, nchunks, chunk)


_SIGS = {
    'segx_posbias_fwd': 'ppplipffpp', 'segx_posbias_bwd': 'pppplipffp',
    'segx_softmax_fwd': 'ppplifpfuup', 'segx_softmax_bwd': 'pppplifpfuup',
    'segx_layernorm_fwd': 'pppppplifp', 'segx_layernorm_bwd': 'pppppplip',
    'segx_colreduce_ws_floats': 'lli', 'segx_colsum': 'pppllp', 'segx_ln_param_grad': 'ppppppplip',
    'segx_sum': 'plppfp', 'segx_rowsum': 'ppllp',
    'segx_prenorm_fwd': 'pppplfpppliiffuup',
    'segx_prenorm_bwd': 'ppppplfppppliifuup',
    'segx_prenorm_bwd_all_ws_floats': 'ii', 'segx_prenorm_bwd_all': 'ppppplfpppppppiiifuup',
    'segx_posembed_fwd': 'pppppliifp', 'segx_posembed_bwd': 'ppppppliip',
    'segx_modes_aggr_fwd': 'pppppppiliffuup', 'segx_modes_aggr_bwd': 'ppppppppilifuup',
    'segx_modes_aggr_param_grad': 'pppppppppppilifuup', 'segx_gelu_bwd': 'ppplfuup',
    'segx_gelu_bwd_colsum': 'ppppplifuup', 'segx_gelu_bwd_colsum_ws_floats': 'li', 'segx_modes_aggr_bwd_all_ws_floats': 'ili', 'segx_modes_aggr_bwd_all': 'ppppppppppppilifuup',
    'segx_loss_ws_floats': 'ii', 'segx_seg_loss_fwd': 'ppppppiilfp', 'segx_seg_loss_bwd': 'pppppppiilfp',
    'segx_mt_bertadam_step': 'pppppppppppiiifffddfpp', 'segx_mt_gather': 'pppppiiip',
    'segx_gn_ws_floats': 'iii', 'segx_groupnorm_fwd': 'pppppppiiilfp', 'segx_groupnorm_bwd': 'pppppppppiiilpp',
    'segx_interp_gn_nparts': 'li', 'segx_interp_linear_fwd_axis2_gn': 'pppliiiilipip', 'segx_groupnorm_fwd_parts': 'ppipppppiiilfp',
    'segx_groupnorm_stats_parts': 'pippifp', 'segx_gn_fold_bwd': 'pppppppppiiilp', 'segx_bridge_mask': 'ppppiiiiiiiiip', 'segx_gn_fold_bwd_proj': 'ppippppppppiiilp',
    'segx_interp_linear_fwd': 'pppliiiiiip', 'segx_interp_linear_fwd_axis2': 'pppliiiilp', 'segx_interp_linear_bwd_axis2': 'ppliiiilp', 'segx_interp_linear_bwd': 'ppliiiiiip', 'segx_interp_linear_bwd_axis': 'ppliilfp',
    'segx_axis_gather': 'pplpp', 'segx_pixel_shuffle2': 'ppliiip', 'segx_add_noise': 'ppplffiuup', 'segx_resize2d': 'ppliiiiiip', 'segx_color_blend': 'ppilippip',
    'segx_gray_mean_ws_floats': 'il', 'segx_gray_mean': 'pppilip', 'segx_normalize': 'ppiilfppp',
    'segx_x6_presplit_elems': 'iiii', 'segx_x6_presplit': 'piilliillpp',
    'segx_tune': 'ii', 'segx_tune_get': 'i', 'segx_x3_launches': '', 'segx_gemm_route': 'pppp', 'segx_set_rng_base': 'p', 'segx_rng_advance': 'pup', 'segx_resized_crop3d': 'pplpp', 'segx_stem_compose_fwd': 'ppppiiiiip', 'segx_stem_compose_bwd': 'pppppppiiiiip', 'segx_bridge_input': 'ppiiiiiip', 'segx_stem_s2d_input': 'ppiiiiiip', 'segx_conv2d_stem_fwd': 'pppiiiiiiiiiiip', 'segx_conv2d_stem_im2col': 'ppiiiiiiiiiiip', 'segx_dropout': 'pplfuup', 'segx_avgpool2_fwd': 'ppliip', 'segx_avgpool2_bwd': 'ppliip', 'segx_transpose': 'ppliip', 'segx_interp_linear_fwd_axis': 'pppliilfp', 'segx_window_accum': 'pppiipp', 'segx_harden_segmap': 'ppppiilifp', 'segx_window_gather': 'ppppiiipp', 'segx_window_merge': 'pppppiiipifp', 'segx_dice_ws_floats': 'll', 'segx_dice_sums': 'pppllp',
    'segx_surface_border': 'ppliiiip', 'segx_edt_sq': 'ppliiip', 'segx_surface_hist': 'pppliiiip', 'segx_brats_case_tail': 'ppppplp',
    'segx_index_onehot': 'piplilp', 'segx_onehot_colormap': 'ppplilp', 'segx_onehot_case_tail': 'ppppppiilfp', 'segx_nhot_case_tail': 'ppiipppppiiiiiifp',
    'segx_ccl2d': 'pippliip', 'segx_frag_keep2': 'ppliip', 'segx_frag_apply': 'ppppliiip', 'segx_row_extent': 'ppliifp', 'segx_nhot_to_values': 'ppplilp',
    'segx_conv3d_fwd': 'pppiipipp', 'segx_conv3d_fwd_packed': 'pppiipipp', 'segx_conv3d_fwd_packed_bs': 'pppiipipllp', 'segx_conv3d_bwd_weight_packed_bs': 'pppiipipllp', 'segx_conv3d_pack_weights': 'ppiiiip', 'segx_conv3d_splitk': 'iipi', 'segx_conv3d_route': 'iipiiiip', 'segx_conv3d_fwd_terms': 'iipiii', 'segx_conv3d_flip_weights': 'ppiiip', 'segx_conv3d_bwd_weight': 'pppiipipp', 'segx_conv3d_bwd_weight_packed': 'pppiipipp', 'segx_conv3d_unpack_wgrad': 'ppiiip',
    'segx_conv3d_halo_ok': 'iip', 'segx_conv3d_halo_wq_floats': 'ii', 'segx_conv3d_halo_pack': 'ppiiip', 'segx_conv3d_halo_fwd': 'pppiipllip', 'segx_conv3d_halo_bias_act_fwd': 'ppppiiplliip', 'segx_conv3d_fwd_bias_act': 'ppppiipipillip', 'segx_bias_map_relu': 'ppilp', 'segx_conv3d_halo_wgrad_ok': 'iip', 'segx_conv3d_halo_wgrad_ws_floats': 'iip', 'segx_conv3d_halo_wgrad': 'ppppiipllp',
    'segx_conv3d_bwd_data_direct': 'ppppiipp', 'segx_nonzero_mask': 'ppiiiiiiiip', 'segx_label_nhot': 'ppiilip',
    'segx_maxpool3d_fwd': 'ppplpp', 'segx_maxpool3d_bwd': 'ppplppp',
    'segx_bn_ws_floats': 'iil', 
    'segx_dwconv2d_fwd': 'pppiiiiiiiiiip', 'segx_dwconv2d_bwd_data': 'pppiiiiiiiiiip',
    'segx_dwconv2d_pool_chunks': 'ii', 'segx_dwconv2d_bias_act_pool': 'pppppiiiiiiiiiiip', 'segx_conv2d_stem_bias_act_fwd': 'ppppiiiiiiiiiiiip',
    'segx_dwconv2d_bwd_weight': 'pppiiiiiiiiiip', 'segx_dwconv2d_bwd_weight_direct': 'pppiiiiiiiiiip', 'segx_dwconv2d_wgrad_rows': 'ii', 'segx_dwconv2d_bwd_fused_rows': 'iiiiiiii', 'segx_dwconv2d_bwd_fused': 'pppppiiiiiiiiiip', 'segx_plane_scale': 'pppllp', 'segx_plane_dot': 'pppllp',
     'segx_plane_bias_add': 'ppplilp',
    'segx_add_relu_fwd': 'pppplilp', 'segx_add_relu_bwd': 'pppllp',
    'segx_plane_chunks': 'l', 'segx_bn_pool_chunks': 'ili', 'segx_bn_parts_floats': 'iil', 'segx_bn_stats_local': 'pppiilp',
    'segx_bn_act_fwd2': 'ppippppfpppppfuuiilfillp', 'segx_bn_act_bwd2': 'ppppppppppiilfiippffuullp',
    'segx_team_status': 'i', 'segx_team_cap': '', 'segx_occupy': 'iifpp',
    'segx_bn_dw_s2_ok': 'iiiiiiii', 'segx_bn_dw_s2_ws_floats': 'iiiii', 'segx_bn_dw_s2_rows': 'iii',
    'segx_bn_dw_s2_fwd': 'p' * 10 + 'ff' + 'iiiiiii' + 'l' + 'p', 'segx_bn_dw_s2_bwd': 'p' * 12 + 'f' + 'iiiiiii' + 'll' + 'p',
    'segx_mbconv_mid_ok': 'iiiii', 'segx_mbconv_mid_fwd': 'p' * 17 + 'ffff' + 'iiiii' + 'p', 'segx_mbconv_mid_bwd': 'p' * 19 + 'fff' + 'iiiii' + 'p',
    'segx_se_fwd2': 'pifpppppppppiiiip', 'segx_se_ws2_floats': 'iii', 'segx_se_bwd2': 'ppppppppfpppppppiiiip',
    'segx_bn_act_bwd_reduce': 'pppppppppiilfippffuup', 'segx_bn_act_bwd_apply': 'pppppppppiilfifppffuup',
}

_LIB = None
DEFAULT_ENGINE = 'x6'


def lib():
    global _LIB
    if _LIB is None:
        _LIB = SegxLib(LIB_PATH)
        _LIB.set_engine(os.environ.get('SEGX_ENGINE', DEFAULT_ENGINE))
    return _LIB


def use_library(libobj):
    global _LIB
    _LIB = libobj
```

Before: 98.15 images/s.

## Fuse stem BN+swish into block-0 stride-1 depthwise conv via team kernels

Adds stride-1 fused BN+swish+depthwise-conv forward and backward team kernels, modelled on the existing stride-2 path with shared helpers factored out. The EfficientNet stem now skips materializing the BN+swish output and passes its BN into block 0, whose depthwise conv uses the new fused kernel. The aim is to save a full-resolution activation write and read, plus separate BN kernel launches, at the highest-resolution layer. The cost is extra complexity in team-synchronized kernels and a narrow eligibility check that falls back to the old path when it does not hold.

After: 99.42 images/s (median of 6 runs). +1.3%, better.

```diff
diff --git a/include/segx.h b/include/segx.h
--- a/include/segx.h
+++ b/include/segx.h
@@ -164,6 +164,14 @@
 int segx_bn_dw_s2_bwd(const float* dD, const float* E, const float* mean, const float* var, const float* w0, const float* b0, const float* Wdw,
                       float* dE, float* dw0, float* db0, float* part, float* ws, float eps, int B, int C, int H, int W, int k, int pad_t, int pad_l,
                       int64_t part_rows, int64_t ws_floats, void* stream);
+int segx_bn_dw_s1_ok(int B, int C, int H, int W, int k, int stride, int pad_t, int pad_l);
+int64_t segx_bn_dw_s1_ws_floats(int B, int C, int H, int W, int backward);
+int64_t segx_bn_dw_s1_rows(int B, int H, int W);
+int segx_bn_dw_s1_fwd(const float* E, const float* w0, const float* b0, float* run_mean, float* run_var, const float* Wdw, float* D, float* mean, float* var,
+                      float* ws, float momentum, float eps, int B, int C, int H, int W, int k, int pad_t, int pad_l, int64_t ws_floats, void* stream);
+int segx_bn_dw_s1_bwd(const float* dD, const float* E, const float* mean, const float* var, const float* w0, const float* b0, const float* Wdw,
+                      float* dE, float* dw0, float* db0, float* part, float* ws, float eps, int B, int C, int H, int W, int k, int pad_t, int pad_l,
+                      int64_t part_rows, int64_t ws_floats, void* stream);
 int segx_dwconv2d_bwd_weight_direct(const float* dY, const float* X, float* dW, int B, int C, int H, int Wd, int OH, int OW, int k,
                                     int stride, int pad_t, int pad_l, void* stream);
 int segx_dwconv2d_bwd_weight(const float* dY, const float* X, float* part, int B, int C, int H, int Wd, int OH, int OW, int k,
diff --git a/segtran_amd/csrc/backbone.hip b/segtran_amd/csrc/backbone.hip
--- a/segtran_amd/csrc/backbone.hip
+++ b/segtran_amd/csrc/backbone.hip
@@ -647,7 +647,7 @@
 #undef SEGX_BN_TB
     return check_launch("segx_bn_act_bwd2/team");
 }
-constexpr int S2_BAND = 4;
+constexpr int DW_BAND = 4;
 constexpr int S2_IMG = 1440;
 constexpr int S2_GIMG = 1600;
 struct BnDwS2Args {
@@ -656,38 +656,9 @@
     const float* dD; float* dE; float* dw; float* db; float* part;
     float eps; int C, H, W4, pt;
 };
-template <int KP, int K, int PL>
-__global__ __launch_bounds__(256) SEGX_MIN_WAVES_PER_SIMD(KP <= 16 ? 3 : 2) void bn_dw_s2_fwd_team_kernel(BnDwS2Args g, BnTeam t) {
-    static_assert(KP % S2_BAND == 0 && PL <= 4 && 4 + 3 * 2 + K - 1 - PL < 16, "window does not fit the four float4 read per row");
-    constexpr int NB = KP / S2_BAND;
-    __shared__ float red[4];
-    __shared__ f32x4 img[NB > 1 ? 2 : 1][S2_IMG];
-    const int TS = t.B * t.cpp, tl = threadIdx.x;
-    const int c = blockIdx.x / TS, r = blockIdx.x - c * TS, b = r / t.cpp, ch = r - b * t.cpp;
-    const int C = g.C, W4 = g.W4, S4 = g.H * W4, j0 = ch * 256 * KP;
-    const int64_t S = 4 * (int64_t)S4, plane = ((int64_t)b * C + c) * S;
-    auto offk = [&](int k) { const int j = j0 + tl + 256 * k; return 16u * (unsigned)(j < S4 ? j : S4 - 1); };
-    f32x4 v[KP];
-    const ws_gptr xb = ws_uniform_base(g.E + plane);
-#pragma unroll
-    for (int k = 0; k < KP; ++k) v[k] = ws_load<f32x4>(xb, offk(k));
-    const int rpk = 256 / W4, tr = tl / W4, tc = tl - tr * W4, HT = g.pt, LS = W4 + 1, IR = S2_BAND * rpk + K - 2;
-    f32x4 hv[2]; bool hok[2];
-#pragma unroll
-    for (int q = 0; q < 2; ++q) {
-        const int hr = tr + q * rpk;
-        const int jh = (hr < HT ? j0 - (HT - hr) * W4 : j0 + 256 * KP + (hr - HT) * W4) + tc;
-        hok[q] = hr < K - 2 && jh >= 0 && jh < S4;
-        hv[q] = ws_load<f32x4>(xb, 16u * (unsigned)(hok[q] ? jh : 0));
-    }
-    __builtin_amdgcn_sched_barrier(0);
-    for (int i = tl; i <= IR; i += 256) {
-        img[0][i * LS] = f32x4{0.f, 0.f, 0.f, 0.f};
-        if (NB > 1) img[NB > 1 ? 1 : 0][i * LS] = f32x4{0.f, 0.f, 0.f, 0.f};
-    }
-    float w[K * K];
-#pragma unroll
-    for (int i = 0; i < K * K; ++i) w[i] = g.Wdw[(int64_t)c * K * K + i];
+template <int KP>
+__device__ __forceinline__ void dw_team_stats(f32x4 (&v)[KP], const BnDwS2Args& g, const BnTeam& t, int c, int r, int TS, int j0, int S4, float* red, float& sc, float& sh) {
+    const int tl = threadIdx.x;
     float s = 0.f;
 #pragma unroll
     for (int k = 0; k < KP; ++k) {
@@ -717,19 +688,97 @@
             g.run_var[c] = (1.0f - g.momentum) * g.run_var[c] + g.momentum * (st.m2 / fmaxf(st.n - 1.0f, 1.0f));
         }
     }
-    const float sc = rsqrtf(var + g.eps) * g.w[c], sh = g.b[c] - mean * sc;
-    auto act4 = [&](const f32x4& x, bool ok) {
-        f32x4 o;
-        o.x = act_fwd_c<ACT_SWISH>(x.x * sc + sh, ACT_SWISH); o.y = act_fwd_c<ACT_SWISH>(x.y * sc + sh, ACT_SWISH);
-        o.z = act_fwd_c<ACT_SWISH>(x.z * sc + sh, ACT_SWISH); o.w = act_fwd_c<ACT_SWISH>(x.w * sc + sh, ACT_SWISH);
-        return ok ? o : f32x4{0.f, 0.f, 0.f, 0.f};
-    };
+    sc = rsqrtf(var + g.eps) * g.w[c]; sh = g.b[c] - mean * sc;
+}
+__device__ __forceinline__ f32x4 dw_act4(const f32x4& x, float sc, float sh, bool ok) {
+    f32x4 o;
+    o.x = act_fwd_c<ACT_SWISH>(x.x * sc + sh, ACT_SWISH); o.y = act_fwd_c<ACT_SWISH>(x.y * sc + sh, ACT_SWISH);
+    o.z = act_fwd_c<ACT_SWISH>(x.z * sc + sh, ACT_SWISH); o.w = act_fwd_c<ACT_SWISH>(x.w * sc + sh, ACT_SWISH);
+    return ok ? o : f32x4{0.f, 0.f, 0.f, 0.f};
+}
+__device__ __forceinline__ void dw_slope4(const f32x4& xv, const float (&de)[4], bool ok, float m, float rstd, float wc, float bc_, f32x4& hh, f32x4& dd, float& sa, float& sq) {
+    hh.x = (xv.x - m) * rstd; hh.y = (xv.y - m) * rstd; hh.z = (xv.z - m) * rstd; hh.w = (xv.w - m) * rstd;
+    dd.x = de[0] * act_grad_c<ACT_SWISH>(hh.x * wc + bc_, ACT_SWISH); dd.y = de[1] * act_grad_c<ACT_SWISH>(hh.y * wc + bc_, ACT_SWISH);
+    dd.z = de[2] * act_grad_c<ACT_SWISH>(hh.z * wc + bc_, ACT_SWISH); dd.w = de[3] * act_grad_c<ACT_SWISH>(hh.w * wc + bc_, ACT_SWISH);
+    if (!ok) { dd = f32x4{0.f, 0.f, 0.f, 0.f}; hh = dd; }
+    sa += (dd.x + dd.y) + (dd.z + dd.w); sq += (dd.x * hh.x + dd.y * hh.y) + (dd.z * hh.z + dd.w * hh.w);
+}
+template <int KP>
+__device__ __forceinline__ void dw_team_bwd_finish(const f32x4 (&h)[KP], const f32x4 (&d)[KP], float sa, float sq, const BnDwS2Args& g, const BnTeam& t, int c, int r, int TS,
+                                                   int j0, int S4, int64_t S, int64_t plane, float sc, float* red) {
+    const int tl = threadIdx.x;
+    sa = block_sum<4>(sa, red); sq = block_sum<4>(sq, red);
+    const TeamBufs tb{t.slots + (int64_t)c * TS * TEAM_SLOT, t.mbox + (int64_t)c * TS * TEAM_MBOX, t.tag_lo, t.tag_hi, t.err, t.spin};
+    if (tl == 0) { float* pp = tb.slots + r * TEAM_SLOT; team_store(pp, sa); team_store(pp + 1, sq); }
+    float res[3];
+    team_exchange(tb, r, TS, res, [](const float* parts, int members, float (&o)[3]) {
+        const int lane = threadIdx.x & 63;
+        const bool h0 = lane < members, h1 = lane + 64 < members;
+        const float a0 = team_load(parts + TEAM_SLOT * (h0 ? lane : 0)), q0 = team_load(parts + TEAM_SLOT * (h0 ? lane : 0) + 1);
+        const float a1 = team_load(parts + TEAM_SLOT * (h1 ? lane + 64 : 0)), q1 = team_load(parts + TEAM_SLOT * (h1 ? lane + 64 : 0) + 1);
+        float As = (h0 ? a0 : 0.f) + (h1 ? a1 : 0.f), Qs = (h0 ? q0 : 0.f) + (h1 ? q1 : 0.f);
+#pragma unroll
+        for (int o2 = 1; o2 < 64; o2 <<= 1) { As += __shfl_xor(As, o2); Qs += __shfl_xor(Qs, o2); }
+        o[0] = As; o[1] = Qs; o[2] = 0.f;
+    });
+    const float As = res[0], Qs = res[1];
+    if (r == 0 && tl == 0) { g.db[c] = As; g.dw[c] = Qs; }
+    const float inv_n = 1.0f / ((float)t.B * (float)S), k1 = As * inv_n, k2 = Qs * inv_n;
+    const ws_gptr_w ob = ws_uniform_base_w(g.dE + plane);
+    int tl2 = tl;
+    SEGX_PIN(tl2);
+#pragma unroll
+    for (int k = 0; k < KP; ++k) {
+        const int j = j0 + tl2 + 256 * k;
+        if (j < S4) {
+            f32x4 o;
+            o.x = sc * (d[k].x - k1 - h[k].x * k2); o.y = sc * (d[k].y - k1 - h[k].y * k2);
+            o.z = sc * (d[k].z - k1 - h[k].z * k2); o.w = sc * (d[k].w - k1 - h[k].w * k2);
+            ws_store<f32x4>(ob, 16u * (unsigned)j, o);
+        }
+    }
+}
+template <int KP, int K, int PL>
+__global__ __launch_bounds__(256) SEGX_MIN_WAVES_PER_SIMD(KP <= 16 ? 3 : 2) void bn_dw_s2_fwd_team_kernel(BnDwS2Args g, BnTeam t) {
+    static_assert(KP % DW_BAND == 0 && PL <= 4 && 4 + 3 * 2 + K - 1 - PL < 16, "window does not fit the four float4 read per row");
+    constexpr int NB = KP / DW_BAND;
+    __shared__ float red[4];
+    __shared__ f32x4 img[NB > 1 ? 2 : 1][S2_IMG];
+    const int TS = t.B * t.cpp, tl = threadIdx.x;
+    const int c = blockIdx.x / TS, r = blockIdx.x - c * TS, b = r / t.cpp, ch = r - b * t.cpp;
+    const int C = g.C, W4 = g.W4, S4 = g.H * W4, j0 = ch * 256 * KP;
+    const int64_t S = 4 * (int64_t)S4, plane = ((int64_t)b * C + c) * S;
+    auto offk = [&](int k) { const int j = j0 + tl + 256 * k; return 16u * (unsigned)(j < S4 ? j : S4 - 1); };
+    f32x4 v[KP];
+    const ws_gptr xb = ws_uniform_base(g.E + plane);
+#pragma unroll
+    for (int k = 0; k < KP; ++k) v[k] = ws_load<f32x4>(xb, offk(k));
+    const int rpk = 256 / W4, tr = tl / W4, tc = tl - tr * W4, HT = g.pt, LS = W4 + 1, IR = DW_BAND * rpk + K - 2;
+    f32x4 hv[2]; bool hok[2];
+#pragma unroll
+    for (int q = 0; q < 2; ++q) {
+        const int hr = tr + q * rpk;
+        const int jh = (hr < HT ? j0 - (HT - hr) * W4 : j0 + 256 * KP + (hr - HT) * W4) + tc;
+        hok[q] = hr < K - 2 && jh >= 0 && jh < S4;
+        hv[q] = ws_load<f32x4>(xb, 16u * (unsigned)(hok[q] ? jh : 0));
+    }
+    __builtin_amdgcn_sched_barrier(0);
+    for (int i = tl; i <= IR; i += 256) {
+        img[0][i * LS] = f32x4{0.f, 0.f, 0.f, 0.f};
+        if (NB > 1) img[NB > 1 ? 1 : 0][i * LS] = f32x4{0.f, 0.f, 0.f, 0.f};
+    }
+    float w[K * K];
+#pragma unroll
+    for (int i = 0; i < K * K; ++i) w[i] = g.Wdw[(int64_t)c * K * K + i];
+    float sc, sh;
+    dw_team_stats<KP>(v, g, t, c, r, TS, j0, S4, red, sc, sh);
+    auto act4 = [&](const f32x4& x, bool ok) { return dw_act4(x, sc, sh, ok); };
     const int OW4 = W4 >> 1, orow = tl / OW4, oc = tl - orow * OW4, D4 = S4 >> 2;
     const int rpos = (2 * orow) * LS + 2 * oc + 1;
     const ws_gptr_w db_ = ws_uniform_base_w(g.D + ((int64_t)b * C + c) * (S >> 2));
 #pragma unroll
     for (int bd = 0; bd < NB; ++bd) {
-        constexpr int KB = S2_BAND;
+        constexpr int KB = DW_BAND;
         const int k0 = bd * KB;
         f32x4* im = img[bd & (NB > 1 ? 1 : 0)];
 #pragma unroll
@@ -835,12 +884,8 @@
             __builtin_amdgcn_sched_barrier(0);
         }
         f32x4 hh, dd;
-        hh.x = (xv.x - m) * rstd; hh.y = (xv.y - m) * rstd; hh.z = (xv.z - m) * rstd; hh.w = (xv.w - m) * rstd;
-        dd.x = de[0] * act_grad_c<ACT_SWISH>(hh.x * wc + bc_, ACT_SWISH); dd.y = de[1] * act_grad_c<ACT_SWISH>(hh.y * wc + bc_, ACT_SWISH);
-        dd.z = de[2] * act_grad_c<ACT_SWISH>(hh.z * wc + bc_, ACT_SWISH); dd.w = de[3] * act_grad_c<ACT_SWISH>(hh.w * wc + bc_, ACT_SWISH);
-        if (!ok) { dd = f32x4{0.f, 0.f, 0.f, 0.f}; hh = dd; }
+        dw_slope4(xv, de, ok, m, rstd, wc, bc_, hh, dd, sa, sq);
         h[k] = hh; d[k] = dd;
-        sa += (dd.x + dd.y) + (dd.z + dd.w); sq += (dd.x * hh.x + dd.y * hh.y) + (dd.z * hh.z + dd.w * hh.w);
     }
     sa = block_sum<4>(sa, red); sq = block_sum<4>(sq, red);
     const TeamBufs tb{t.slots + (int64_t)c * TS * TEAM_SLOT, t.mbox + (int64_t)c * TS * TEAM_MBOX, t.tag_lo, t.tag_hi, t.err, t.spin};
@@ -886,21 +931,21 @@
     __syncthreads();
     if (tl < KK) g.part[((int64_t)r * C + c) * KK + tl] = (float)((wred[0][tl] + wred[1][tl]) + (wred[2][tl] + wred[3][tl]));
 }
-static inline bool s2_pow2(int v) { return v > 0 && (v & (v - 1)) == 0; }
-static inline int s2_kp(int B, int64_t S, bool backward) {
+static inline bool dw_pow2(int v) { return v > 0 && (v & (v - 1)) == 0; }
+static inline int dw_kp(int B, int64_t S, bool backward) {
     int kp = 0;
     if (B < 1 || S < 4 || bn_auto_form(B, S, backward, &kp) != 1) return 0;
     return kp == 4 || kp == 16 || (kp == 32 && !backward) ? kp : 0;
 }
 static inline bool s2_serves(int B, int C, int H, int W, int k, int stride, int pt, int pl) {
-    if (!(stride == 2 && (k == 3 || k == 5) && B >= 1 && C >= 1 && H >= 2 && (H & 1) == 0 && W >= 16 && W <= 512 && s2_pow2(W))) return false;
+    if (!(stride == 2 && (k == 3 || k == 5) && B >= 1 && C >= 1 && H >= 2 && (H & 1) == 0 && W >= 16 && W <= 512 && dw_pow2(W))) return false;
     if (!(pt == pl && pt >= (k - 2) / 2 && pt <= k / 2)) return false;
     const int64_t S = (int64_t)H * W;
     if (S > (int64_t)1 << 26 || (int64_t)B * C > 65535) return false;
-    const int kf = s2_kp(B, S, false), kb = s2_kp(B, S, true);
+    const int kf = dw_kp(B, S, false), kb = dw_kp(B, S, true);
     if (!kf || !kb || (1024 * kf) % (2 * W) || (1024 * kb) % (2 * W)) return false;
     const int W4 = W / 4, rpk = 256 / W4;
-    return (S2_BAND * rpk + k - 2) * (W4 + 1) + 1 <= S2_IMG && (kb * (rpk / 2) + (k + 1) / 2) * (W4 / 2 + 1) + 1 <= S2_GIMG;
+    return (DW_BAND * rpk + k - 2) * (W4 + 1) + 1 <= S2_IMG && (kb * (rpk / 2) + (k + 1) / 2) * (W4 / 2 + 1) + 1 <= S2_GIMG;
 }
 template <int KP, int K>
 static int s2_launch_fwd(const BnDwS2Args& g, const BnTeam& t, dim3 grid, hipStream_t stream, int pl) {
@@ -917,6 +962,200 @@
     if (pl == (K - 2) / 2) SEGX_S2B((K - 2) / 2); else SEGX_S2B(K / 2);
 #undef SEGX_S2B
     return check_launch("segx_bn_dw_s2_bwd");
+}
+template <int P>
+__device__ __forceinline__ void dw_s1_row(float (&e)[4 + 2 * P], const float* row) {
+    static_assert(P == 1 || P == 2, "k 3 or 5");
+    const f32x4 cc = *reinterpret_cast<const f32x4*>(row);
+    if constexpr (P == 1) { e[0] = row[-1]; e[5] = row[4]; }
+    else {
+        const float2 l = *reinterpret_cast<const float2*>(row - 2), rr = *reinterpret_cast<const float2*>(row + 4);
+        e[0] = l.x; e[1] = l.y; e[6] = rr.x; e[7] = rr.y;
+    }
+    e[P] = cc.x; e[P + 1] = cc.y; e[P + 2] = cc.z; e[P + 3] = cc.w;
+}
+__device__ __forceinline__ float dw_chain_fma(float a, float b, float c) {
+#if defined(__HIP_DEVICE_COMPILE__)
+    return __builtin_fmaf(a, b, c);
+#else
+    return a * b + c;
+#endif
+}
+constexpr int S1_IMG = 1549;
+template <int KP> struct S1G { static constexpr int IMG = KP <= 4 ? 1549 : 4645; };
+template <int KP, int K>
+__global__ __launch_bounds__(256) SEGX_MIN_WAVES_PER_SIMD(KP <= 16 ? 3 : 2) void bn_dw_s1_fwd_team_kernel(BnDwS2Args g, BnTeam t) {
+    static_assert(KP % DW_BAND == 0 && (K == 3 || K == 5), "bands of DW_BAND k indices; k 3 or 5");
+    constexpr int P = (K - 1) / 2, NB = KP / DW_BAND, KB = DW_BAND;
+    __shared__ float red[4];
+    __shared__ f32x4 img[NB > 1 ? 2 : 1][S1_IMG];
+    const int TS = t.B * t.cpp, tl = threadIdx.x;
+    const int c = blockIdx.x / TS, r = blockIdx.x - c * TS, b = r / t.cpp, ch = r - b * t.cpp;
+    const int C = g.C, W4 = g.W4, S4 = g.H * W4, j0 = ch * 256 * KP;
+    const int64_t S = 4 * (int64_t)S4, plane = ((int64_t)b * C + c) * S;
+    auto offk = [&](int k) { const int j = j0 + tl + 256 * k; return 16u * (unsigned)(j < S4 ? j : S4 - 1); };
+    f32x4 v[KP];
+    const ws_gptr xb = ws_uniform_base(g.E + plane);
+#pragma unroll
+    for (int k = 0; k < KP; ++k) v[k] = ws_load<f32x4>(xb, offk(k));
+    const int rpk = 256 / W4, tr = tl / W4, tc = tl - tr * W4, LS = W4 + 1, IR = KB * rpk + 2 * P;
+    f32x4 hv[2]; bool hok[2];
+#pragma unroll
+    for (int q = 0; q < 2; ++q) {
+        const int hr = tr + q * rpk;
+        const int jh = (hr < P ? j0 - (P - hr) * W4 : j0 + 256 * KP + (hr - P) * W4) + tc;
+        hok[q] = hr < 2 * P && jh >= 0 && jh < S4;
+        hv[q] = ws_load<f32x4>(xb, 16u * (unsigned)(hok[q] ? jh : 0));
+    }
+    __builtin_amdgcn_sched_barrier(0);
+    for (int i = tl; i <= IR; i += 256) {
+        img[0][i * LS] = f32x4{0.f, 0.f, 0.f, 0.f};
+        if (NB > 1) img[NB > 1 ? 1 : 0][i * LS] = f32x4{0.f, 0.f, 0.f, 0.f};
+    }
+    float w[K * K];
+#pragma unroll
+    for (int i = 0; i < K * K; ++i) w[i] = g.Wdw[(int64_t)c * K * K + i];
+    float sc, sh;
+    dw_team_stats<KP>(v, g, t, c, r, TS, j0, S4, red, sc, sh);
+    const ws_gptr_w db_ = ws_uniform_base_w(g.D + plane);
+    int tl2 = tl;
+    SEGX_PIN(tl2);
+#pragma unroll
+    for (int bd = 0; bd < NB; ++bd) {
+        const int k0 = bd * KB;
+        f32x4* im = img[bd & (NB > 1 ? 1 : 0)];
+#pragma unroll
+        for (int kk = k0 - 1; kk <= k0 + KB; ++kk) {
+            if (kk < 0 || kk >= KP) continue;
+            const int ir = tr + (kk - k0) * rpk + P;
+            if (kk < k0 ? ir >= 0 : kk < k0 + KB || ir < IR) im[ir * LS + 1 + tc] = dw_act4(v[kk], sc, sh, j0 + tl + 256 * kk < S4);
+        }
+        if (bd == 0 || bd == NB - 1) {
+#pragma unroll
+            for (int q2 = 0; q2 < 2; ++q2) {
+                const int hr = tr + q2 * rpk;
+                if (hr < 2 * P && (hr < P ? bd == 0 : bd == NB - 1)) im[(hr < P ? hr : KB * rpk + hr) * LS + 1 + tc] = dw_act4(hv[q2], sc, sh, hok[q2]);
+            }
+        }
+        __syncthreads();
+        const float* pf = reinterpret_cast<const float*>(im) + 4 * (tr * LS + 1 + tc);
+#pragma unroll
+        for (int kq = 0; kq < KB; ++kq) {
+            float acc[4] = {0.f, 0.f, 0.f, 0.f};
+#pragma unroll
+            for (int ky = 0; ky < K; ++ky) {
+                float e[4 + 2 * P];
+                dw_s1_row<P>(e, pf + 4 * ((kq * rpk + ky) * LS));
+#pragma unroll
+                for (int j = 0; j < 4; ++j)
+#pragma unroll
+                    for (int kx = 0; kx < K; ++kx) acc[j] += w[ky * K + kx] * e[j + kx];
+#pragma unroll
+                for (int j = 0; j < 4; ++j) SEGX_PIN(acc[j]);
+            }
+            const int dj = j0 + tl2 + 256 * (k0 + kq);
+            if (dj < S4) ws_store<f32x4>(db_, 16u * (unsigned)dj, f32x4{acc[0], acc[1], acc[2], acc[3]});
+        }
+        __builtin_amdgcn_sched_barrier(0);
+    }
+}
+template <int KP, int K>
+__global__ __launch_bounds__(256) SEGX_MIN_WAVES_PER_SIMD(2) void bn_dw_s1_bwd_team_kernel(BnDwS2Args g, BnTeam t) {
+    static_assert(K == 3 || K == 5, "k 3 or 5");
+    constexpr int P = (K - 1) / 2, KK = K * K, NGV = KP + P;
+    __shared__ float red[4];
+    __shared__ double wred[4][KK];
+    __shared__ f32x4 gim[S1G<KP>::IMG];
+    const int TS = t.B * t.cpp, tl = threadIdx.x;
+    const int c = blockIdx.x / TS, r = blockIdx.x - c * TS, b = r / t.cpp, ch = r - b * t.cpp;
+    const int C = g.C, W4 = g.W4, H = g.H, S4 = H * W4, j0 = ch * 256 * KP;
+    const int64_t S = 4 * (int64_t)S4, plane = ((int64_t)b * C + c) * S;
+    auto offk = [&](int k) { const int j = j0 + tl + 256 * k; return 16u * (unsigned)(j < S4 ? j : S4 - 1); };
+    f32x4 h[KP], d[KP];
+    const ws_gptr xb = ws_uniform_base(g.E + plane);
+#pragma unroll
+    for (int k = 0; k < KP; ++k) h[k] = ws_load<f32x4>(xb, offk(k));
+    const int rpk = 256 / W4, tr = tl / W4, tc = tl - tr * W4, LS = W4 + 1, NG = KP * rpk + 2 * P, y_lo = j0 / W4 - P;
+    {
+        const ws_gptr gb = ws_uniform_base(g.dD + plane);
+        f32x4 gv[NGV];
+#pragma unroll
+        for (int i = 0; i < NGV; ++i) {
+            const int gi = tr + i * rpk, y = y_lo + gi;
+            gv[i] = ws_load<f32x4>(gb, 16u * (unsigned)(gi < NG && y >= 0 && y < H ? y * W4 + tc : 0));
+        }
+        for (int i = tl; i <= NG; i += 256) gim[i * LS] = f32x4{0.f, 0.f, 0.f, 0.f};
+#pragma unroll
+        for (int i = 0; i < NGV; ++i) {
+            const int gi = tr + i * rpk, y = y_lo + gi;
+            if (gi < NG) gim[gi * LS + 1 + tc] = y >= 0 && y < H ? gv[i] : f32x4{0.f, 0.f, 0.f, 0.f};
+        }
+    }
+    __syncthreads();
+    __builtin_amdgcn_sched_barrier(0);
+    const float rstd = rsqrtf(g.var[c] + g.eps), m = g.mean[c], wc = g.w[c], bc_ = g.b[c], sc = rstd * wc, sh = bc_ - m * sc;
+    float wr[KK], dwa[KK];
+#pragma unroll
+    for (int i = 0; i < KK; ++i) { wr[i] = g.Wdw[(int64_t)c * KK + (KK - 1 - i)]; dwa[i] = 0.f; }
+    const float* gf = reinterpret_cast<const float*>(gim) + 4 * (tr * LS + 1 + tc);
+    float sa = 0.f, sq = 0.f;
+#pragma unroll
+    for (int k = 0; k < KP; ++k) {
+        const bool ok = j0 + tl + 256 * k < S4;
+        const f32x4 xv = h[k];
+        const f32x4 ev = dw_act4(xv, sc, sh, ok);
+        const float ep[4] = {ev.x, ev.y, ev.z, ev.w};
+        float de[4] = {0.f, 0.f, 0.f, 0.f};
+#pragma unroll
+        for (int ky = 0; ky < K; ++ky) {
+            float G[4 + 2 * P];
+            dw_s1_row<P>(G, gf + 4 * ((k * rpk + ky) * LS));
+#pragma unroll
+            for (int i = 0; i < 4; ++i)
+#pragma unroll
+                for (int kx = 0; kx < K; ++kx) {
+                    de[i] = dw_chain_fma(wr[ky * K + kx], G[i + kx], de[i]); dwa[ky * K + kx] = dw_chain_fma(ep[i], G[i + kx], dwa[ky * K + kx]);
+                }
+#pragma unroll
+            for (int i = 0; i < 4; ++i) SEGX_PIN(de[i]);
+#pragma unroll
+            for (int kx = 0; kx < K; ++kx) SEGX_PIN(dwa[ky * K + kx]);
+            __builtin_amdgcn_sched_barrier(0);
+        }
+        f32x4 hh, dd;
+        dw_slope4(xv, de, ok, m, rstd, wc, bc_, hh, dd, sa, sq);
+        h[k] = hh; d[k] = dd;
+    }
+    dw_team_bwd_finish<KP>(h, d, sa, sq, g, t, c, r, TS, j0, S4, S, plane, sc, red);
+#pragma unroll
+    for (int i = 0; i < KK; ++i) {
+        const double sw = wave_sum_d((double)dwa[i]);
+        if ((tl & 63) == 0) wred[tl >> 6][KK - 1 - i] = sw;
+    }
+    __syncthreads();
+    if (tl < KK) g.part[((int64_t)r * C + c) * KK + tl] = (float)((wred[0][tl] + wred[1][tl]) + (wred[2][tl] + wred[3][tl]));
+}
+static inline bool s1_serves(int B, int C, int H, int W, int k, int stride, int pt, int pl) {
+    if (!(stride == 1 && (k == 3 || k == 5) && B >= 1 && C >= 1 && H >= 1 && W >= 16 && W <= 512 && dw_pow2(W))) return false;
+    if (!(pt == (k - 1) / 2 && pl == (k - 1) / 2)) return false;
+    const int64_t S = (int64_t)H * W;
+    if (S > (int64_t)1 << 26 || (int64_t)B * C > 65535) return false;
+    const int kf = dw_kp(B, S, false), kb = dw_kp(B, S, true);
+    if (!kf || !kb || (1024 * kf) % W || (1024 * kb) % W) return false;
+    const int W4 = W / 4, rpk = 256 / W4;
+    return (DW_BAND * rpk + k - 1) * (W4 + 1) + 1 <= S1_IMG && (kb * rpk + k - 1) * (W4 + 1) + 1 <= (kb <= 4 ? S1G<4>::IMG : S1G<16>::IMG);
+}
+template <int KP, int K>
+static int s1_launch_fwd(const BnDwS2Args& g, const BnTeam& t, dim3 grid, hipStream_t stream) {
+    if (int rc = team_occupancy_ok((const void*)bn_dw_s1_fwd_team_kernel<KP, K>, "segx_bn_dw_s1_fwd")) return rc;
+    hipLaunchKernelGGL((bn_dw_s1_fwd_team_kernel<KP, K>), grid, dim3(256), 0, stream, g, t);
+    return check_launch("segx_bn_dw_s1_fwd");
+}
+template <int KP, int K>
+static int s1_launch_bwd(const BnDwS2Args& g, const BnTeam& t, dim3 grid, hipStream_t stream) {
+    if (int rc = team_occupancy_ok((const void*)bn_dw_s1_bwd_team_kernel<KP, K>, "segx_bn_dw_s1_bwd")) return rc;
+    hipLaunchKernelGGL((bn_dw_s1_bwd_team_kernel<KP, K>), grid, dim3(256), 0, stream, g, t);
+    return check_launch("segx_bn_dw_s1_bwd");
 }
 template <int T, int K, int BM>
 static void bn_res_launch_fwd(const BnFwdArgs& g, int B, dim3 grid, hipStream_t stream, bool pool) {
@@ -2041,55 +2280,78 @@
 }
 extern "C" int segx_bn_dw_s2_ok(int B, int C, int H, int W, int k, int stride, int pad_t, int pad_l) { return s2_serves(B, C, H, W, k, stride, pad_t, pad_l) ? 1 : 0; }
 extern "C" int64_t segx_bn_dw_s2_ws_floats(int B, int C, int H, int W, int backward) {
-    const int kp = H > 0 && W > 0 ? s2_kp(B, (int64_t)H * W, backward != 0) : 0;
+    const int kp = H > 0 && W > 0 ? dw_kp(B, (int64_t)H * W, backward != 0) : 0;
     return kp ? (int64_t)C * B * bn_team_chunks((int64_t)H * W, kp) * (TEAM_SLOT + TEAM_MBOX) : 0;
 }
 extern "C" int64_t segx_bn_dw_s2_rows(int B, int H, int W) {
-    const int kp = H > 0 && W > 0 ? s2_kp(B, (int64_t)H * W, true) : 0;
+    const int kp = H > 0 && W > 0 ? dw_kp(B, (int64_t)H * W, true) : 0;
     return kp ? (int64_t)B * bn_team_chunks((int64_t)H * W, kp) : 0;
 }
-static int s2_team(BnTeam& t, float* ws, int64_t ws_floats, int B, int C, int64_t S, int kp, const char* what) {
+static int dw_team(BnTeam& t, float* ws, int64_t ws_floats, int B, int C, int64_t S, int kp, const char* what, int stride) {
     t.B = B; t.cpp = bn_team_chunks(S, kp); t.slots = ws; t.mbox = ws + (int64_t)C * B * t.cpp * TEAM_SLOT;
     team_fill(t);
     SEGX_REQUIRE(B * t.cpp <= team_cap() && (int64_t)C * B * t.cpp < 2147483647LL, "%s: team of %d workgroups", what, B * t.cpp);
     const int64_t need = (int64_t)C * B * t.cpp * (TEAM_SLOT + TEAM_MBOX);
-    SEGX_REQUIRE(ws_floats >= need, "%s: the scratch holds %lld floats, this call needs %lld (segx_bn_dw_s2_ws_floats under the current knob 3)", what, (long long)ws_floats, (long long)need);
+    SEGX_REQUIRE(ws_floats >= need, "%s: the scratch holds %lld floats, this call needs %lld (segx_bn_dw_s%d_ws_floats under the current knob 3)", what, (long long)ws_floats, (long long)need, stride);
     return 0;
+}
+static int bn_dw_fwd(const char* what, int stride, const float* E, const float* w0, const float* b0, float* run_mean, float* run_var, const float* Wdw, float* D, float* mean,
+                     float* var, float* ws, float momentum, float eps, int B, int C, int H, int W, int k, int pad_t, int pad_l, int64_t ws_floats, void* stream_) {
+    SEGX_STREAM; SEGX_REQUIRE(E && w0 && b0 && Wdw && D && mean && var && ws && (!run_mean == !run_var), "%s: bad args", what);
+    SEGX_REQUIRE(stride == 2 ? s2_serves(B, C, H, W, k, 2, pad_t, pad_l) : s1_serves(B, C, H, W, k, 1, pad_t, pad_l), "%s: shape not served (segx_bn_dw_s%d_ok == 0)", what, stride);
+    SEGX_REQUIRE(((reinterpret_cast<uintptr_t>(E) | reinterpret_cast<uintptr_t>(D)) & 15) == 0, "%s: tensors must be 16-byte aligned", what);
+    const int64_t S = (int64_t)H * W;
+    const int kp = dw_kp(B, S, false);
+    BnTeam t;
+    if (int rc = dw_team(t, ws, ws_floats, B, C, S, kp, what, stride)) return rc;
+    BnDwS2Args g; memset(&g, 0, sizeof(g));
+    g.E = E; g.w = w0; g.b = b0; g.Wdw = Wdw; g.mean = mean; g.var = var; g.D = D; g.run_mean = run_mean; g.run_var = run_var; g.momentum = momentum;
+    g.eps = eps; g.C = C; g.H = H; g.W4 = W / 4; g.pt = stride == 2 ? pad_t : 0;
+    const dim3 tg = team_grid((int64_t)C * B * t.cpp);
+#define SEGX_DW(KP) (stride == 2 ? (k == 3 ? s2_launch_fwd<KP, 3>(g, t, tg, stream, pad_l) : s2_launch_fwd<KP, 5>(g, t, tg, stream, pad_l)) \
+                                 : (k == 3 ? s1_launch_fwd<KP, 3>(g, t, tg, stream) : s1_launch_fwd<KP, 5>(g, t, tg, stream)))
+    return kp == 4 ? SEGX_DW(4) : kp == 16 ? SEGX_DW(16) : SEGX_DW(32);
+#undef SEGX_DW
+}
+static int bn_dw_bwd(const char* what, int stride, const float* dD, const float* E, const float* mean, const float* var, const float* w0, const float* b0, const float* Wdw,
+                     float* dE, float* dw0, float* db0, float* part, float* ws, float eps, int B, int C, int H, int W, int k, int pad_t, int pad_l,
+                     int64_t part_rows, int64_t ws_floats, void* stream_) {
+    SEGX_STREAM; SEGX_REQUIRE(dD && E && mean && var && w0 && b0 && Wdw && dE && dw0 && db0 && part && ws, "%s: bad args", what);
+    SEGX_REQUIRE(stride == 2 ? s2_serves(B, C, H, W, k, 2, pad_t, pad_l) : s1_serves(B, C, H, W, k, 1, pad_t, pad_l), "%s: shape not served (segx_bn_dw_s%d_ok == 0)", what, stride);
+    SEGX_REQUIRE(((reinterpret_cast<uintptr_t>(E) | reinterpret_cast<uintptr_t>(dD) | reinterpret_cast<uintptr_t>(dE)) & 15) == 0, "%s: tensors must be 16-byte aligned", what);
+    const int64_t S = (int64_t)H * W;
+    const int kp = dw_kp(B, S, true);
+    BnTeam t;
+    if (int rc = dw_team(t, ws, ws_floats, B, C, S, kp, what, stride)) return rc;
+    SEGX_REQUIRE(part_rows >= (int64_t)B * t.cpp, "%s: the filter-gradient partials hold %lld rows, this call writes %d (segx_bn_dw_s%d_rows under the current knob 3)",
+                 what, (long long)part_rows, B * t.cpp, stride);
+    BnDwS2Args g; memset(&g, 0, sizeof(g));
+    g.E = E; g.w = w0; g.b = b0; g.Wdw = Wdw; g.mean = const_cast<float*>(mean); g.var = const_cast<float*>(var); g.dD = dD; g.dE = dE; g.dw = dw0; g.db = db0; g.part = part;
+    g.eps = eps; g.C = C; g.H = H; g.W4 = W / 4; g.pt = stride == 2 ? pad_t : 0;
+    const dim3 tg = team_grid((int64_t)C * B * t.cpp);
+#define SEGX_DW(KP) (stride == 2 ? (k == 3 ? s2_launch_bwd<KP, 3>(g, t, tg, stream, pad_l) : s2_launch_bwd<KP, 5>(g, t, tg, stream, pad_l)) \
+                                 : (k == 3 ? s1_launch_bwd<KP, 3>(g, t, tg, stream) : s1_launch_bwd<KP, 5>(g, t, tg, stream)))
+    return kp == 4 ? SEGX_DW(4) : SEGX_DW(16);
+#undef SEGX_DW
 }
 extern "C" int segx_bn_dw_s2_fwd(const float* E, const float* w0, const float* b0, float* run_mean, float* run_var, const float* Wdw, float* D, float* mean, float* var,
                                  float* ws, float momentum, float eps, int B, int C, int H, int W, int k, int pad_t, int pad_l, int64_t ws_floats, void* stream_) {
-    SEGX_STREAM; SEGX_REQUIRE(E && w0 && b0 && Wdw && D && mean && var && ws && (!run_mean == !run_var), "segx_bn_dw_s2_fwd: bad args");
-    SEGX_REQUIRE(s2_serves(B, C, H, W, k, 2, pad_t, pad_l), "segx_bn_dw_s2_fwd: shape not served (segx_bn_dw_s2_ok == 0)");
-    SEGX_REQUIRE(((reinterpret_cast<uintptr_t>(E) | reinterpret_cast<uintptr_t>(D)) & 15) == 0, "segx_bn_dw_s2_fwd: tensors must be 16-byte aligned");
-    const int64_t S = (int64_t)H * W;
-    const int kp = s2_kp(B, S, false);
-    BnTeam t;
-    if (int rc = s2_team(t, ws, ws_floats, B, C, S, kp, "segx_bn_dw_s2_fwd")) return rc;
-    BnDwS2Args g; memset(&g, 0, sizeof(g));
-    g.E = E; g.w = w0; g.b = b0; g.Wdw = Wdw; g.mean = mean; g.var = var; g.D = D; g.run_mean = run_mean; g.run_var = run_var; g.momentum = momentum;
-    g.eps = eps; g.C = C; g.H = H; g.W4 = W / 4; g.pt = pad_t;
-    const dim3 tg = team_grid((int64_t)C * B * t.cpp);
-#define SEGX_S2(KP) (k == 3 ? s2_launch_fwd<KP, 3>(g, t, tg, stream, pad_l) : s2_launch_fwd<KP, 5>(g, t, tg, stream, pad_l))
-    return kp == 4 ? SEGX_S2(4) : kp == 16 ? SEGX_S2(16) : SEGX_S2(32);
-#undef SEGX_S2
+    return bn_dw_fwd("segx_bn_dw_s2_fwd", 2, E, w0, b0, run_mean, run_var, Wdw, D, mean, var, ws, momentum, eps, B, C, H, W, k, pad_t, pad_l, ws_floats, stream_);
 }
 extern "C" int segx_bn_dw_s2_bwd(const float* dD, const float* E, const float* mean, const float* var, const float* w0, const float* b0, const float* Wdw,
                                  float* dE, float* dw0, float* db0, float* part, float* ws, float eps, int B, int C, int H, int W, int k, int pad_t, int pad_l,
                                  int64_t part_rows, int64_t ws_floats, void* stream_) {
-    SEGX_STREAM; SEGX_REQUIRE(dD && E && mean && var && w0 && b0 && Wdw && dE && dw0 && db0 && part && ws, "segx_bn_dw_s2_bwd: bad args");
-    SEGX_REQUIRE(s2_serves(B, C, H, W, k, 2, pad_t, pad_l), "segx_bn_dw_s2_bwd: shape not served (segx_bn_dw_s2_ok == 0)");
-    SEGX_REQUIRE(((reinterpret_cast<uintptr_t>(E) | reinterpret_cast<uintptr_t>(dD) | reinterpret_cast<uintptr_t>(dE)) & 15) == 0, "segx_bn_dw_s2_bwd: tensors must be 16-byte aligned");
-    const int64_t S = (int64_t)H * W;
-    const int kp = s2_kp(B, S, true);
-    BnTeam t;
-    if (int rc = s2_team(t, ws, ws_floats, B, C, S, kp, "segx_bn_dw_s2_bwd")) return rc;
-    SEGX_REQUIRE(part_rows >= (int64_t)B * t.cpp, "segx_bn_dw_s2_bwd: the filter-gradient partials hold %lld rows, this call writes %d (segx_bn_dw_s2_rows under the current knob 3)",
-                 (long long)part_rows, B * t.cpp);
-    BnDwS2Args g; memset(&g, 0, sizeof(g));
-    g.E = E; g.w = w0; g.b = b0; g.Wdw = Wdw; g.mean = const_cast<float*>(mean); g.var = const_cast<float*>(var); g.dD = dD; g.dE = dE; g.dw = dw0; g.db = db0; g.part = part;
-    g.eps = eps; g.C = C; g.H = H; g.W4 = W / 4; g.pt = pad_t;
-    const dim3 tg = team_grid((int64_t)C * B * t.cpp);
-#define SEGX_S2(KP) (k == 3 ? s2_launch_bwd<KP, 3>(g, t, tg, stream, pad_l) : s2_launch_bwd<KP, 5>(g, t, tg, stream, pad_l))
-    return kp == 4 ? SEGX_S2(4) : SEGX_S2(16);
-#undef SEGX_S2
-}
+    return bn_dw_bwd("segx_bn_dw_s2_bwd", 2, dD, E, mean, var, w0, b0, Wdw, dE, dw0, db0, part, ws, eps, B, C, H, W, k, pad_t, pad_l, part_rows, ws_floats, stream_);
+}
+extern "C" int segx_bn_dw_s1_ok(int B, int C, int H, int W, int k, int stride, int pad_t, int pad_l) { return s1_serves(B, C, H, W, k, stride, pad_t, pad_l) ? 1 : 0; }
+extern "C" int64_t segx_bn_dw_s1_ws_floats(int B, int C, int H, int W, int backward) { return segx_bn_dw_s2_ws_floats(B, C, H, W, backward); }
+extern "C" int64_t segx_bn_dw_s1_rows(int B, int H, int W) { return segx_bn_dw_s2_rows(B, H, W); }
+extern "C" int segx_bn_dw_s1_fwd(const float* E, const float* w0, const float* b0, float* run_mean, float* run_var, const float* Wdw, float* D, float* mean, float* var,
+                                 float* ws, float momentum, float eps, int B, int C, int H, int W, int k, int pad_t, int pad_l, int64_t ws_floats, void* stream_) {
+    return bn_dw_fwd("segx_bn_dw_s1_fwd", 1, E, w0, b0, run_mean, run_var, Wdw, D, mean, var, ws, momentum, eps, B, C, H, W, k, pad_t, pad_l, ws_floats, stream_);
+}
+extern "C" int segx_bn_dw_s1_bwd(const float* dD, const float* E, const float* mean, const float* var, const float* w0, const float* b0, const float* Wdw,
+                                 float* dE, float* dw0, float* db0, float* part, float* ws, float eps, int B, int C, int H, int W, int k, int pad_t, int pad_l,
+                                 int64_t part_rows, int64_t ws_floats, void* stream_) {
+    return bn_dw_bwd("segx_bn_dw_s1_bwd", 1, dD, E, mean, var, w0, b0, Wdw, dE, dw0, db0, part, ws, eps, B, C, H, W, k, pad_t, pad_l, part_rows, ws_floats, stream_);
+}
diff --git a/segtran_amd/efficientnet/model.py b/segtran_amd/efficientnet/model.py
--- a/segtran_amd/efficientnet/model.py
+++ b/segtran_amd/efficientnet/model.py
@@ -82,14 +82,18 @@
     fused_middle = True
 
     fused_entry = True
+    fused_entry_s1 = True
 
     def _takes_fused_entry(self, x):
-        if not (MBConvBlock.fused_entry and self.training and SF._bn_stats_sync is None and self.expand_ratio != 1):
-            return False
-        dw = self._depthwise_conv
-        if not (self._bn0.training and dw.stride == (2, 2) and dw.kernel_size[0] == dw.kernel_size[1] and x.dim() == 4 and x.dtype == torch.float32):
-            return False
-        return SF.bn_dw_s2_ok((x.shape[0], dw.in_channels, x.shape[2], x.shape[3]), dw.kernel_size[0], 2, dw.static_pad)
+        dw = self._depthwise_conv
+        if not (self.training and SF._bn_stats_sync is None and self.expand_ratio != 1 and dw.stride in ((1, 1), (2, 2))):
+            return False
+        if not (MBConvBlock.fused_entry if dw.stride == (2, 2) else MBConvBlock.fused_entry_s1):
+            return False
+        if not (self._bn0.training and dw.kernel_size[0] == dw.kernel_size[1] and x.dim() == 4 and x.dtype == torch.float32):
+            return False
+        ok = SF.bn_dw_s2_ok if dw.stride == (2, 2) else SF.bn_dw_s1_ok
+        return ok((x.shape[0], dw.in_channels, x.shape[2], x.shape[3]), dw.kernel_size[0], dw.stride[0], dw.static_pad)
 
     def _takes_fused_middle(self, x):
         if not (MBConvBlock.fused_middle and MBConvBlock.gate_in_weights and self.training and SF._bn_stats_sync is None and self.expand_ratio != 1):
@@ -115,14 +119,17 @@
         Wb = SF.se_gate_weights(y, psum, nch, self._se_reduce.weight, self._se_reduce.bias, self._se_expand.weight, self._se_expand.bias, w2)
         return SF.conv1x1_per_sample_bias(y, Wb, b2, resid=inputs if skip else None)
 
-    def forward(self, inputs, drop_connect_rate=None):
+    def forward(self, inputs, drop_connect_rate=None, entry_bn=None):
         x = skip_in = inputs
         skip = self.stride == 1 and self.input_filters == self.output_filters
-        fused = self._takes_fused_middle(x)
-        entry = not fused and self._takes_fused_entry(x)
-        if entry:
-            dw = self._depthwise_conv
-            d = SF.bn_act_dwconv_s2(self._expand_conv(x), self._bn0, dw.weight, dw.stride[0], dw.static_pad)
+        fused = entry_bn is None and self._takes_fused_middle(x)
+        entry = entry_bn is not None or (not fused and self._takes_fused_entry(x))
+        dw = self._depthwise_conv
+        if entry_bn is not None:
+            assert self.expand_ratio == 1 and not skip
+            d = SF.bn_act_dwconv_s1(x, entry_bn, dw.weight, dw.stride[0], dw.static_pad)
+        elif entry:
+            d = (SF.bn_act_dwconv_s2 if dw.stride == (2, 2) else SF.bn_act_dwconv_s1)(self._expand_conv(x), self._bn0, dw.weight, dw.stride[0], dw.static_pad)
         elif self.expand_ratio != 1 and not fused:
             x = SF.bn_act(self._expand_conv(x), self._bn0, SF.ACT_SWISH)
         se = (self._se_reduce.weight, self._se_reduce.bias, self._se_expand.weight, self._se_expand.bias)
@@ -196,16 +203,33 @@
                                 ignore_missing_keys=ignore_missing_keys)
         return model
 
+    fused_stem_entry = True
+
+    def _stem_into_block0(self, inputs):
+        blk = self._blocks[0]
+        dw, st = blk._depthwise_conv, self._conv_stem
+        if not (EfficientNet.fused_stem_entry and self.training and self._bn0.training and blk.training and SF._bn_stats_sync is None and not self.batchnorm_folded):
+            return False
+        if blk.expand_ratio != 1 or dw.stride != (1, 1) or dw.kernel_size[0] != dw.kernel_size[1] or (blk.stride == 1 and blk.input_filters == blk.output_filters):
+            return False
+        if inputs.dim() != 4 or inputs.dtype != torch.float32 or 0 in self.endpoint_blk_indices:
+            return False
+        pl, pr, pt, pb = st.static_pad
+        H = (inputs.shape[2] + pt + pb - st.kernel_size[0]) // st.stride[0] + 1
+        W = (inputs.shape[3] + pl + pr - st.kernel_size[1]) // st.stride[1] + 1
+        return SF.bn_dw_s1_ok((inputs.shape[0], dw.in_channels, H, W), dw.kernel_size[0], 1, dw.static_pad)
+
     def extract_endpoints(self, inputs):
         if self.batchnorm_folded:
             return self._extract_endpoints_folded(inputs)
         endpoints = {}
-        x = SF.bn_act(self._conv_stem(inputs), self._bn0, SF.ACT_SWISH)
+        stem_bn = self._bn0 if self._stem_into_block0(inputs) else None
+        x = self._conv_stem(inputs) if stem_bn is not None else SF.bn_act(self._conv_stem(inputs), self._bn0, SF.ACT_SWISH)
         prev_x = x
         nblk = len(self._blocks)
         for idx, block in enumerate(self._blocks):
             rate = self.drop_connect_rate * float(idx) / nblk if self.drop_connect_rate else None
-            x = block(x, drop_connect_rate=rate)
+            x = block(x, drop_connect_rate=rate, entry_bn=stem_bn) if idx == 0 and stem_bn is not None else block(x, drop_connect_rate=rate)
             if idx in self.endpoint_blk_indices:
                 endpoints['reduction_%d' % (len(endpoints) + 1)] = prev_x
             prev_x = x
diff --git a/segtran_amd/functional.py b/segtran_amd/functional.py
--- a/segtran_amd/functional.py
+++ b/segtran_amd/functional.py
@@ -1116,19 +1116,22 @@
                             bn1.weight, bn1.bias, bn1.running_mean, bn1.running_var, float(bn1.momentum), float(bn1.eps), w1, b1, w2, b2, proj_weight)
 
 
-class _BNActDWConvS2(_Fn):
-
-    @staticmethod
-    def forward(ctx, e, w0, b0, rm0, rv0, mom0, eps0, wdw, pt, pl):
+class _BNActDWConv(_Fn):
+
+    @staticmethod
+    def forward(ctx, e, w0, b0, rm0, rv0, mom0, eps0, wdw, pt, pl, stride):
         L = segx.lib()
         e, wdw = _c(e), _c(wdw)
         if e.data_ptr() % 16:
             e = e.clone()
         B, C, H, W = e.shape
         k = wdw.shape[-1]
-        d, stats = _empty(e, B, C, H // 2, W // 2), _empty(e, 2, C)
-        L.bn_dw_s2_fwd(e, w0, b0, rm0, rv0, wdw, d, stats[0], stats[1], _empty(e, L.bn_dw_s2_ws(B, C, H, W, False)), mom0, eps0, B, C, H, W, k, pt, pl)
-        ctx.cfg = (B, C, H, W, k, pt, pl, eps0, tuple(wdw.shape))
+        d, stats = _empty(e, B, C, H // stride, W // stride), _empty(e, 2, C)
+        if stride == 2:
+            L.bn_dw_s2_fwd(e, w0, b0, rm0, rv0, wdw, d, stats[0], stats[1], _empty(e, L.bn_dw_s2_ws(B, C, H, W, False)), mom0, eps0, B, C, H, W, k, pt, pl)
+        else:
+            L.bn_dw_s1_fwd(e, w0, b0, rm0, rv0, wdw, d, stats[0], stats[1], _empty(e, L.bn_dw_s1_ws(B, C, H, W, False)), mom0, eps0, B, C, H, W, k, pt, pl)
+        ctx.cfg = (B, C, H, W, k, pt, pl, eps0, tuple(wdw.shape), stride)
         ctx.save_for_backward(e, stats, w0, b0, wdw)
         return d
 
@@ -1136,16 +1139,19 @@
     def backward(ctx, dd):
         L = segx.lib()
         e, stats, w0, b0, wdw = ctx.saved_tensors
-        B, C, H, W, k, pt, pl, eps0, wds = ctx.cfg
+        B, C, H, W, k, pt, pl, eps0, wds, stride = ctx.cfg
         dd = _c(dd)
         if dd.data_ptr() % 16:
             dd = dd.clone()
-        rows = L.bn_dw_s2_rows(B, H, W)
+        rows = L.bn_dw_s2_rows(B, H, W) if stride == 2 else L.bn_dw_s1_rows(B, H, W)
         de, g, part = torch.empty_like(e), _empty(e, 2, C), _empty(e, rows, C * k * k)
-        L.bn_dw_s2_bwd(dd, e, stats[0], stats[1], w0, b0, wdw, de, g[0], g[1], part, _empty(e, L.bn_dw_s2_ws(B, C, H, W, True)), eps0, B, C, H, W, k, pt, pl)
+        if stride == 2:
+            L.bn_dw_s2_bwd(dd, e, stats[0], stats[1], w0, b0, wdw, de, g[0], g[1], part, _empty(e, L.bn_dw_s2_ws(B, C, H, W, True)), eps0, B, C, H, W, k, pt, pl)
+        else:
+            L.bn_dw_s1_bwd(dd, e, stats[0], stats[1], w0, b0, wdw, de, g[0], g[1], part, _empty(e, L.bn_dw_s1_ws(B, C, H, W, True)), eps0, B, C, H, W, k, pt, pl)
         dwd = _empty(e, C * k * k)
         L.colsum(part, dwd, _empty(e, L.colreduce_ws(rows, C * k * k, 1)), rows, C * k * k)
-        return de, g[0], g[1], None, None, None, None, dwd.view(wds), None, None
+        return de, g[0], g[1], None, None, None, None, dwd.view(wds), None, None, None
 
 
 def bn_dw_s2_ok(e_shape, k, stride, pad):
@@ -1161,8 +1167,25 @@
 def bn_act_dwconv_s2(e, bn0, dw_weight, stride, static_pad):
     assert int(stride) == 2
     _bn_tick(bn0)
-    return _BNActDWConvS2.apply(e, bn0.weight, bn0.bias, bn0.running_mean, bn0.running_var, float(bn0.momentum), float(bn0.eps), dw_weight,
-                                int(static_pad[2]), int(static_pad[0]))
+    return _BNActDWConv.apply(e, bn0.weight, bn0.bias, bn0.running_mean, bn0.running_var, float(bn0.momentum), float(bn0.eps), dw_weight,
+                              int(static_pad[2]), int(static_pad[0]), 2)
+
+
+def bn_dw_s1_ok(e_shape, k, stride, pad):
+    if len(e_shape) != 4:
+        return False
+    B, C, H, W = (int(v) for v in e_shape)
+    k = int(k)
+    if int(stride) != 1 or k % 2 != 1 or tuple(int(p) for p in pad) != ((k - 1) // 2,) * 4:
+        return False
+    return segx.lib().bn_dw_s1_ok(B, C, H, W, k, 1, (k - 1) // 2, (k - 1) // 2)
+
+
+def bn_act_dwconv_s1(e, bn0, dw_weight, stride, static_pad):
+    assert int(stride) == 1
+    _bn_tick(bn0)
+    return _BNActDWConv.apply(e, bn0.weight, bn0.bias, bn0.running_mean, bn0.running_var, float(bn0.momentum), float(bn0.eps), dw_weight,
+                              int(static_pad[2]), int(static_pad[0]), 1)
 
 
 def conv1x1_per_sample(x, Wb, bias=None):
diff --git a/segtran_amd/segx.py b/segtran_amd/segx.py
--- a/segtran_amd/segx.py
+++ b/segtran_amd/segx.py
@@ -386,6 +386,21 @@
 
     def bn_dw_s2_bwd(self, dD, E, mean, var, w0, b0, Wdw, dE, dw0, db0, part, ws, eps, B, C, H, W, k, pt, pl):
         self._call('segx_bn_dw_s2_bwd', dD, dD, E, mean, var, w0, b0, Wdw, dE, dw0, db0, part, ws, float(eps), B, C, H, W, k, pt, pl, part.shape[0], ws.numel())
+
+    def bn_dw_s1_ok(self, B, C, H, W, k, stride, pt, pl):
+        return bool(self.c.segx_bn_dw_s1_ok(B, C, H, W, k, stride, pt, pl))
+
+    def bn_dw_s1_ws(self, B, C, H, W, backward):
+        return int(self.c.segx_bn_dw_s1_ws_floats(B, C, H, W, 1 if backward else 0))
+
+    def bn_dw_s1_rows(self, B, H, W):
+        return int(self.c.segx_bn_dw_s1_rows(B, H, W))
+
+    def bn_dw_s1_fwd(self, E, w0, b0, rm, rv, Wdw, D, mean, var, ws, mom, eps, B, C, H, W, k, pt, pl):
+        self._call('segx_bn_dw_s1_fwd', E, E, w0, b0, rm, rv, Wdw, D, mean, var, ws, float(mom), float(eps), B, C, H, W, k, pt, pl, ws.numel())
+
+    def bn_dw_s1_bwd(self, dD, E, mean, var, w0, b0, Wdw, dE, dw0, db0, part, ws, eps, B, C, H, W, k, pt, pl):
+        self._call('segx_bn_dw_s1_bwd', dD, dD, E, mean, var, w0, b0, Wdw, dE, dw0, db0, part, ws, float(eps), B, C, H, W, k, pt, pl, part.shape[0], ws.numel())
 
     def mbconv_mid_ok(self, B, C, H, W, k):
         return bool(self.c.segx_mbconv_mid_ok(B, C, H, W, k))
@@ -823,6 +838,8 @@
     'segx_team_status': 'i', 'segx_team_cap': '', 'segx_occupy': 'iifpp',
     'segx_bn_dw_s2_ok': 'iiiiiiii', 'segx_bn_dw_s2_ws_floats': 'iiiii', 'segx_bn_dw_s2_rows': 'iii',
     'segx_bn_dw_s2_fwd': 'p' * 10 + 'ff' + 'iiiiiii' + 'l' + 'p', 'segx_bn_dw_s2_bwd': 'p' * 12 + 'f' + 'iiiiiii' + 'll' + 'p',
+    'segx_bn_dw_s1_ok': 'iiiiiiii', 'segx_bn_dw_s1_ws_floats': 'iiiii', 'segx_bn_dw_s1_rows': 'iii',
+    'segx_bn_dw_s1_fwd': 'p' * 10 + 'ff' + 'iiiiiii' + 'l' + 'p', 'segx_bn_dw_s1_bwd': 'p' * 12 + 'f' + 'iiiiiii' + 'll' + 'p',
     'segx_mbconv_mid_ok': 'iiiii', 'segx_mbconv_mid_fwd': 'p' * 17 + 'ffff' + 'iiiii' + 'p', 'segx_mbconv_mid_bwd': 'p' * 19 + 'fff' + 'iiiii' + 'p',
     'segx_se_fwd2': 'pifpppppppppiiiip', 'segx_se_ws2_floats': 'iii', 'segx_se_bwd2': 'ppppppppfpppppppiiiip',
     'segx_bn_act_bwd_reduce': 'pppppppppiilfippffuup', 'segx_bn_act_bwd_apply': 'pppppppppiilfifppffuup',
```
